# pansanity666/TransHuman

Measured on AMD Instinct MI355X. Metric: rays/sec (512x512, 64 samples/ray), higher is better.
Workload: dtype f32 (fp16 hi/lo x3 MFMA emulation)

## Files before the change

include/transhuman_hip.h:

```cpp
#ifndef TRANSHUMAN_HIP_H
#define TRANSHUMAN_HIP_H

#include <stddef.h>
#include <stdint.h>

#ifdef __cplusplus
extern "C" {
#endif

#define TH_ABI_VERSION 12

typedef struct th_ctx th_ctx;
typedef void* th_stream;

int         th_abi_version(void);
const char* th_last_error(void);
int         th_ctx_create(int device, th_ctx** out);
void        th_ctx_destroy(th_ctx* ctx);
size_t      th_sizeof(const char* type_name);

enum { TH_PROF_HULL = 0, TH_PROF_DPARF = 1, TH_PROF_GATHER = 2, TH_PROF_MLP = 3, TH_PROF_COMPOSITE = 4,
       TH_PROF_VIT = 5, TH_PROF_FOLD = 6 , TH_PROF_PHASES = 8 };
int th_profile_enable(th_ctx* ctx, int on);
int th_profile_read(th_ctx* ctx, double* ms_out, int64_t* count_out);
// ... 17 lines not shown
    th_linear upsample_color;
} th_mlp_weights;

typedef struct {
    const float *ln1_w, *ln1_b, *ln2_w, *ln2_b;
    th_linear qkv, proj, fc1, fc2;
} th_vit_block;

int th_set_mlp_weights(th_ctx* ctx, const th_mlp_weights* w, th_stream stream);
int th_set_mlp_mode(th_ctx* ctx, int mode);
int th_set_fused_waves(th_ctx* ctx, int waves);
int th_set_tok_gather(th_ctx* ctx, int on);
int th_set_tex_rows(th_ctx* ctx, int on);

#define TH_RANGE_SLOTS 8
#define TH_RANGE_FP16_LIMIT 0x7B53u
#define TH_RANGE_FP16_FLOOR 0x2400u
int th_set_vit_mode(th_ctx* ctx, int mode);
int th_range_snapshot(th_ctx* ctx, th_stream stream);
int th_range_read(th_ctx* ctx, int slot, uint32_t* out );
int th_range_last_slot(th_ctx* ctx);
int th_set_chunk_samples(int n);
int th_set_vit_weights(th_ctx* ctx, int depth, int dim, int heads, const th_vit_block* blocks,
                       const float* norm_w, const float* norm_b, th_stream stream);

size_t th_linear_workspace_bytes(int out_f, int in_f);
int th_linear_forward(th_ctx* ctx, const float* A, int lda, int M, const th_linear* lin, int act,
                      float* C, int ldc, void* workspace, size_t workspace_bytes, th_stream stream);

typedef struct {
    const float* pts;
    const float* ray_o;
    const float* ray_d;
    const float* near;
    const float* far;
    const float* t_vals;
    const float* one_minus_t;
    int R, S;
    const float* z_vals;
    const float* sigma_noise;
} th_points;

size_t th_hull_workspace_bytes(int n_verts);
int th_hull_mask(th_ctx* ctx, const th_points* p, const float* verts_world, int n_verts, float thresh,
                 uint8_t* mask_out, int32_t* ray_hit_out, void* workspace, size_t workspace_bytes,
                 th_stream stream);

int th_paint_group(th_ctx* ctx, const float* holder_map_nchw, int V, int C, int H, int W,
                   const float* verts_world, int n_verts, const float* cams, const float* scale_xy,
                   const uint8_t* vizmap, const int32_t* csr_offsets, const int32_t* csr_members,
                   int n_clusters, float* painted_out , float* tokens_out,
                   th_stream stream);
int th_segment_mean_f32(th_ctx* ctx, const float* src, int width, const int32_t* csr_offsets,
                        const int32_t* csr_members, int n_clusters, float* out, th_stream stream);
int th_segment_mean_rot_f64(th_ctx* ctx, const double* blend, const int32_t* csr_offsets,
                            const int32_t* csr_members, int n_clusters, float* rot_out,
                            th_stream stream);

#define TH_MAP_FULL    384
#define TH_MAP_COMPACT 260
#define TH_MAP_SPLIT   256

int th_upsample_concat_nhwc(th_ctx* ctx, const float* img, const float* lat0, const float* lat1,
                            const float* lat2, const int32_t* dims_host, int V, int H, int W,
                            const float* color_w, const float* color_b, float* out_nhwc, th_stream stream);
int th_upsample_concat_split(th_ctx* ctx, const float* img, const float* lat0, const float* lat1, const float* lat2,
                             const int32_t* dims_host, int V, int H, int W, float* out, th_stream stream);
int th_map_box(th_ctx* ctx, const float* verts_a, int na, const float* verts_b, int nb, const float* cams, int V,
               const float* scale_xy, int H, int W, float reach, int32_t* box_out, th_stream stream);
int th_upsample_concat_split_box(th_ctx* ctx, const float* img, const float* lat0, const float* lat1, const float* lat2,
                                 const int32_t* dims_host, int V, int H, int W, float* out, const int32_t* box,
                                 th_stream stream);
size_t th_map_demand_bytes(int V, int H, int W);
int th_upsample_concat_split_demand(th_ctx* ctx, const float* img, const float* lat0, const float* lat1, const float* lat2,
                                    const int32_t* dims_host, int V, int H, int W, float* out, const int32_t* box,
                                    const void* demand, th_stream stream);
size_t th_paint_group_nhwc_workspace_bytes(int V, int n_verts, int C, int out_f);
int th_paint_group_nhwc(th_ctx* ctx, const float* map_nhwc, int V, int H, int W, int C,
                        const float* verts_world, int n_verts, const float* cams, const float* scale_xy,
                        const uint8_t* vizmap, const th_linear* reduction, const th_linear* color_lift,
                        const int32_t* csr_offsets,
                        const int32_t* csr_members, int n_clusters, float* tokens_out, void* workspace,
                        size_t workspace_bytes, th_stream stream);

size_t th_conv_pack_bytes(int cout, int cin, int ks);
int th_conv_pack(th_ctx* ctx, const float* w, int cout, int cin, int ks, void* packed, size_t packed_bytes,
                 float* inv_scale_out, th_stream stream);
int th_conv2d_supported(int cin, int cout, int ks, int stride);
int th_conv2d(th_ctx* ctx, const float* x, int N, int cin, int H, int W, const void* packed, float inv_scale, int cout,
              int ks, int stride, float* y, th_stream stream);

int th_maxpool3x3s2(th_ctx* ctx, const float* x, int planes, int H, int W, float* y, th_stream stream);

size_t th_bn_workspace_bytes(int N, int C, int HW);
int th_bn_act(th_ctx* ctx, const float* x, const float* residual, int N, int C, int HW, const float* gamma,
              const float* beta, float eps, float momentum, float* running_mean, float* running_var, int relu,
              float* y, void* workspace, size_t workspace_bytes, th_stream stream);
int th_bn_act_eval(th_ctx* ctx, const float* x, const float* residual, int N, int C, int HW, const float* gamma,
                   const float* beta, float eps, const float* running_mean, const float* running_var, int relu,
                   float* y, th_stream stream);
int th_conv2d_stats_partials(int N, int cin, int H, int W, int cout, int ks, int stride);
int th_conv2d_stats(th_ctx* ctx, const float* x, int N, int cin, int H, int W, const void* packed, float inv_scale,
                    int cout, int ks, int stride, float* y, void* stats, size_t stats_bytes, th_stream stream);
int th_bn_act_stats(th_ctx* ctx, const float* x, const float* residual, int N, int C, int HW, const void* stats,
                    int n_partials, const float* gamma, const float* beta, float eps, float momentum,
                    float* running_mean, float* running_var, int relu, float* y, th_stream stream);

size_t th_vit_workspace_bytes(int V, int N, int dim, int heads);
int th_vit_forward(th_ctx* ctx, const float* x, const float* pe, int V, int N, float* out,
                   void* workspace, size_t workspace_bytes, th_stream stream);

int th_dparf_encode(th_ctx* ctx, const float* pts_smpl, const int32_t* sel, int P, const float* centres,
                    const float* rot, const float* tokens, int V, int n_clusters, float* out,
                    th_stream stream);

int th_nchw_to_nhwc(th_ctx* ctx, const float* src, int V, int C, int H, int W, float* dst, th_stream stream);
int th_pixel_gather(th_ctx* ctx, const float* pixel_map_nhwc, int V, int C, int H, int W,
                    const float* pts_world, const int32_t* sel, int P, const float* cams,
                    const float* scale_xy, float* out, int ldo, th_stream stream);
int th_pixel_gather_split(th_ctx* ctx, const float* map_split, int V, int H, int W, const float* pts_world,
                          const int32_t* sel, int P, const float* cams, const float* scale_xy, void* out_rows,
                          int ldo, th_stream stream);

int th_map_fold(th_ctx* ctx, const float* map_split, int V, int H, int W, const int32_t* box, float* fold, th_stream stream);
int th_map_fold_demand(th_ctx* ctx, const float* map_split, int V, int H, int W, const void* demand, float* fold, th_stream stream);

size_t th_pixel_texlist_bytes(int V, int P);
int th_pixel_texlist(th_ctx* ctx, const float* map_split, int V, int H, int W, const float* pts_world, const int32_t* sel,
                     int P, const float* cams, const float* scale_xy, void* out, size_t out_bytes, th_stream stream);

size_t th_network_workspace_bytes(int V, int P);
int th_network_forward(th_ctx* ctx, const float* pixel_feat, const float* viewdir, const float* pts_smpl,
                       const uint8_t* mask, int P, const float* centres, const float* rot,
                       const float* tokens, int V, int n_clusters, float* raw_out, void* workspace,
                       size_t workspace_bytes, th_stream stream);

int th_composite(th_ctx* ctx, const float* raw, const float* z, const th_points* rays, int white_bkgd,
                 float* rgb, float* acc, float* depth, float* weights_out, th_stream stream);

int th_gen_rays(th_ctx* ctx, const float* K_host, const float* R_host, const float* T_host,
                const float* bounds_host, int H, int W, float* ray_o, float* ray_d, float* near_out,
                float* far_out, uint8_t* mask_at_box, th_stream stream);

int th_bound_mask(th_ctx* ctx, const int32_t* corners_xy_host , int H, int W, uint8_t* mask,
                  th_stream stream);

size_t th_marching_cubes_workspace_bytes(int X, int Y, int Z);
int th_marching_cubes_count(th_ctx* ctx, const float* cube, int X, int Y, int Z, float iso, void* workspace,
                            size_t workspace_bytes, int64_t* counts_host , th_stream stream);
int th_marching_cubes_range(th_ctx* ctx, const void* workspace, int X, int Y, int Z, int x,
                            int64_t* prefix_host , th_stream stream);
int th_marching_cubes_emit(th_ctx* ctx, const float* cube, int X, int Y, int Z, float iso, const void* workspace,
                           int x0, int x1, const double* scale_host , const double* origin_host ,
                           double* verts, int32_t* tris, th_stream stream);

size_t th_ssim_workspace_bytes(int h, int w, int c);
int th_ssim(th_ctx* ctx, const float* a, const float* b, int h, int w, int c, int pitch, double* out, void* workspace,
            size_t workspace_bytes, th_stream stream);

size_t th_lpips_pack_bytes(void);
int th_lpips_pack(th_ctx* ctx, const float* const* conv_w , const float* const* conv_b ,
                  const float* const* lin_w , void* packed, size_t bytes, th_stream stream);
size_t th_lpips_workspace_bytes(int n, int h, int w);
int th_lpips(th_ctx* ctx, const float* in0, const float* in1, int n, int h, int w, const void* packed, double* out,
             void* workspace, size_t workspace_bytes, th_stream stream);

typedef struct {
    const double* v_template;
    const double* shapedirs;
    const double* posedirs;
    const double* J_regressor;
    const double* weights;
    const int32_t* parent;
    int n_verts;
} th_smpl_model;
size_t th_smpl_workspace_bytes(int n_verts);
int th_smpl_lbs(th_ctx* ctx, const th_smpl_model* model, const float* pose_aa, const float* rot, const double* beta,
                double* verts, double* joints, double* T, void* workspace, size_t workspace_bytes,
                th_stream stream);

int th_view_embed(th_ctx* ctx, const float* ray_d, int R, int view_res, float* out, th_stream stream);

typedef struct {
    const int32_t* box;
    float          reach;
    const float*   img;
    const float*   lat0;
    const float*   lat1;
    const float*   lat2;
    int32_t        dims[6];
    const void*    demand;
} th_map_source;

typedef struct {
    const float* verts_world;
    int          n_verts;
    const float* Rh;
    const float* Th;
    const float* cams;
    const float* scale_xy;
    const float* pixel_map_nhwc;
    int          V, H, W;
    int          map_channels;
    const float* tokens;
    const float* centres;
    const float* rot;
    int          n_clusters;
    float        hull_thresh;
// ... 35 lines not shown
```

transhuman_amd/csrc/k_encoder.hip:

```cpp
#include "th_internal.h"

struct UpsSrc {
    const float* p;
    int C, h, w;
    int c0;
};

__device__ __forceinline__ void ups_coord(int dst, int in, int out, int& i0, int& i1, float& l0, float& l1) {
    float scale = (out > 1) ? (float)(in - 1) / (float)(out - 1) : 0.f;
    float src = scale * (float)dst;
    i0 = (int)src;
    i1 = i0 + ((i0 < in - 1) ? 1 : 0);
    l1 = src - (float)i0;
    l0 = 1.0f - l1;
}

__global__ __launch_bounds__(256) void upsample_concat_nhwc_kernel(UpsSrc s0, UpsSrc s1, UpsSrc s2,
                                                                   const float* __restrict__ img,
                                                                   const float* __restrict__ wc,
                                                                   const float* __restrict__ bc, int H, int W,
                                                                   int NG, int CO, float* __restrict__ out,
                                                                   float* __restrict__ rgb4,
                                                                   const int32_t* __restrict__ box,
                                                                   const unsigned* __restrict__ need) {
    __shared__ float tile[64][65];
    const int lane = threadIdx.x & 63, wave = threadIdx.x >> 6;
    const int x = blockIdx.x * 64 + lane, y = blockIdx.y;
    const int v = blockIdx.z / NG, grp = blockIdx.z % NG;
    unsigned long long want = ~0ull;
    if (need != nullptr) {
        const unsigned* nw = need + ((((long long)v * H + y) * W + (long long)blockIdx.x * 64) >> 5);
        want = (unsigned long long)nw[0] | ((unsigned long long)nw[1] << 32);
        if (want == 0ull) return;
    }
    if (box != nullptr) {
        const int by0 = box[4 * v + 1], by1 = box[4 * v + 3];
        if (y < by0 || y > by1) return;
        const int32_t* sp = box + 4 * (gridDim.z / NG) + ((long long)v * H + y) * 2;
        if ((int)blockIdx.x * 64 + 63 < sp[0] || (int)blockIdx.x * 64 > sp[1]) return;
    }
    int cout0;
    if (grp == 4 && NG == 5) {
        if (wave == 0 && x < W && ((want >> lane) & 1ull)) {
            long long hw = (long long)H * W;
            const float* ip = img + (long long)v * 3 * hw + (long long)y * W + x;
            float* dst = rgb4 ? rgb4 + (((long long)v * H + y) * W + x) * 4 : out + (((long long)v * H + y) * W + x) * CO + 256;
            *reinterpret_cast<float4*>(dst) = make_float4(ip[0], ip[hw], ip[2 * hw], 0.f);
        }
        return;
    }
    if (grp < 4) {
        UpsSrc s = grp == 0 ? s0 : (grp == 1 ? s1 : s2);
        int cin0 = grp == 3 ? 64 : 0;
        cout0 = s.c0 + cin0;
        int y0, y1, x0, x1;
        float ly0, ly1, lx0, lx1;
        ups_coord(y, s.h, H, y0, y1, ly0, ly1);
        ups_coord(x < W ? x : W - 1, s.w, W, x0, x1, lx0, lx1);
        const float* base = s.p + ((long long)v * s.C + cin0) * s.h * s.w;
        for (int c = wave; c < 64; c += 4) {
            const float* pl = base + (long long)c * s.h * s.w;
            float v00 = pl[y0 * s.w + x0], v01 = pl[y0 * s.w + x1], v10 = pl[y1 * s.w + x0], v11 = pl[y1 * s.w + x1];
            tile[lane][c] = ly0 * (lx0 * v00 + lx1 * v01) + ly1 * (lx0 * v10 + lx1 * v11);
        }
    } else {
        int cin0 = (grp - 4) * 64;
        cout0 = 256 + cin0;
        int xx = x < W ? x : W - 1;
        long long hw = (long long)H * W;
        const float* ip = img + (long long)v * 3 * hw + (long long)y * W + xx;
        float r = ip[0], g = ip[hw], b = ip[2 * hw];
        for (int c = wave; c < 64; c += 4) {
            const float* w = wc + (cin0 + c) * 3;
            tile[lane][c] = fmaf(b, w[2], fmaf(g, w[1], r * w[0])) + bc[cin0 + c];
        }
    }
    __syncthreads();
    float* orow = out + (((long long)v * H + y) * W + (long long)blockIdx.x * 64) * CO + cout0;
    for (int px = wave; px < 64; px += 4)
        if (blockIdx.x * 64 + px < W && ((want >> px) & 1ull)) orow[(long long)px * CO + lane] = tile[px][lane];
}

int th_upsample_concat_launch(const float* img, const float* lat0, const float* lat1, const float* lat2,
                              const int* dims , int V, int H, int W, const float* wc,
                              const float* bc, float* out, hipStream_t s, int split, const int32_t* box, const unsigned* need) {
    UpsSrc s0{lat0, 64, dims[0], dims[1], 0};
    UpsSrc s1{lat1, 64, dims[2], dims[3], 64};
    UpsSrc s2{lat2, 128, dims[4], dims[5], 128};
    const int NG = wc ? 6 : 5, CO = wc ? 384 : (split ? 256 : 260);
    float* rgb4 = (!wc && split) ? out + (long long)V * H * W * 256 : nullptr;
    hipLaunchKernelGGL(upsample_concat_nhwc_kernel, dim3(th_cdiv(W, 64), H, V * NG), dim3(256), 0, s, s0, s1, s2, img, wc,
                       bc, H, W, NG, CO, out, rgb4, box, need);
    TH_LAUNCH_CHECK();
    return 0;
}

#define MAPBOX_NB 8
__global__ void map_box_init_kernel(int V, int H, int W, int32_t* __restrict__ box) {
    const int v = blockIdx.x;
    int32_t* sp = box + 4 * V + (long long)v * H * 2;
    for (int i = threadIdx.x; i < H; i += blockDim.x) { sp[2 * i] = W; sp[2 * i + 1] = -1; }
    if (threadIdx.x == 0) {
        box[4 * v] = 0x7fffffff; box[4 * v + 1] = 0x7fffffff; box[4 * v + 2] = -1; box[4 * v + 3] = -1;
        box[4 * V + (long long)V * H * 2 + v] = 0;
    }
}
__global__ __launch_bounds__(1024) void map_box_kernel(const float* __restrict__ va, int na, const float* __restrict__ vb,
                                                       int nb, const float* __restrict__ cams,
                                                       const float* __restrict__ scale, int H, int W, float reach,
                                                       int32_t* __restrict__ box) {
    const int v = blockIdx.x, V = gridDim.x, tid = threadIdx.x;
    const float* cam = cams + 21 * v;
    bool bad = false;
    extern __shared__ int span_l[];
    __shared__ int bx[4];
    for (int i = tid; i < H; i += 1024) { span_l[2 * i] = W; span_l[2 * i + 1] = -1; }
    if (tid == 0) { bx[0] = 0x7fffffff; bx[1] = 0x7fffffff; bx[2] = -1; bx[3] = -1; }
    __syncthreads();
    for (int i = blockIdx.y * 1024 + tid; i < na + nb; i += 1024 * gridDim.y) {
        const float* p = i < na ? va + 3 * i : vb + 3 * (i - na);
        const float x = p[0], y = p[1], z = p[2];
        float vx0 = 3.0e38f, vx1 = -3.0e38f, vy0 = 3.0e38f, vy1 = -3.0e38f;
        bool vbad = false;
        for (int k = 0; k < 8; ++k) {
            const float qx = x + ((k & 1) ? reach : -reach), qy = y + ((k & 2) ? reach : -reach),
                        qz = z + ((k & 4) ? reach : -reach);
            const float cx = fmaf(cam[2], qz, fmaf(cam[1], qy, cam[0] * qx)) + cam[9];
            const float cy = fmaf(cam[5], qz, fmaf(cam[4], qy, cam[3] * qx)) + cam[10];
            const float cz = fmaf(cam[8], qz, fmaf(cam[7], qy, cam[6] * qx)) + cam[11];
            const float* K = cam + 12;
            const float pz = fmaf(K[8], cz, fmaf(K[7], cy, K[6] * cx));
            float u, w;
            th_project(cam, qx, qy, qz, u, w);
            const float ix = ((u * scale[0] - 1.0f + 1.0f) / 2.0f) * (float)(W - 1);
            const float iy = ((w * scale[1] - 1.0f + 1.0f) / 2.0f) * (float)(H - 1);
            if (!(pz > 1e-6f) || !(fabsf(ix) < 1.0e9f) || !(fabsf(iy) < 1.0e9f)) vbad = true;
            vx0 = fminf(vx0, ix); vx1 = fmaxf(vx1, ix);
            vy0 = fminf(vy0, iy); vy1 = fmaxf(vy1, iy);
        }
        bad = bad || vbad;
        if (!vbad) {
            const int ax0 = (int)fminf(fmaxf(floorf(vx0) - 2.0f, 0.0f), (float)(W - 1));
            const int ax1 = (int)fminf(fmaxf(floorf(vx1) + 3.0f, 0.0f), (float)(W - 1));
            const int ay0 = (int)fminf(fmaxf(floorf(vy0) - 2.0f, 0.0f), (float)(H - 1));
            const int ay1 = (int)fminf(fmaxf(floorf(vy1) + 3.0f, 0.0f), (float)(H - 1));
            atomicMin(&bx[0], ax0); atomicMin(&bx[1], ay0); atomicMax(&bx[2], ax1); atomicMax(&bx[3], ay1);
            for (int yy = ay0; yy <= ay1; ++yy) {
                atomicMin(&span_l[2 * yy], ax0);
                atomicMax(&span_l[2 * yy + 1], ax1);
            }
        }
    }
    if (bad) atomicOr(&box[4 * V + (long long)V * H * 2 + v], 1);
    __syncthreads();
    int32_t* sp = box + 4 * V + (long long)v * H * 2;
    for (int i = tid; i < H; i += 1024)
        if (span_l[2 * i + 1] >= span_l[2 * i]) {
            atomicMin(&sp[2 * i], span_l[2 * i]);
            atomicMax(&sp[2 * i + 1], span_l[2 * i + 1]);
        }
    if (tid == 0 && bx[2] >= 0) {
        atomicMin(&box[4 * v], bx[0]); atomicMin(&box[4 * v + 1], bx[1]);
        atomicMax(&box[4 * v + 2], bx[2]); atomicMax(&box[4 * v + 3], bx[3]);
    }
}
__global__ void map_box_final_kernel(int V, int H, int W, int nverts, int32_t* __restrict__ box) {
    const int v = blockIdx.x;
    const bool full = box[4 * V + (long long)V * H * 2 + v] != 0 || nverts <= 0 || box[4 * v + 2] < 0;
    if (!full) return;
    int32_t* sp = box + 4 * V + (long long)v * H * 2;
    for (int i = threadIdx.x; i < H; i += blockDim.x) { sp[2 * i] = 0; sp[2 * i + 1] = W - 1; }
    if (threadIdx.x == 0) { box[4 * v] = 0; box[4 * v + 1] = 0; box[4 * v + 2] = W - 1; box[4 * v + 3] = H - 1; }
}
int th_map_box_launch(const float* va, int na, const float* vb, int nb, const float* cams, int V, const float* scale, int H,
                      int W, float reach, int32_t* box, hipStream_t s) {
// ... 192 lines not shown
```

transhuman_amd/csrc/k_mlp_fused_host.hip:

```cpp
#include <stdio.h>
#include <stdlib.h>
#include <string.h>

#include "k_mlp_fused_kernel.h"
#include "k_mlp_fused8_kernel.h"

__global__ void pack_fused_kernel(const float* __restrict__ W, int N, int K, int KB, int CT, const int* __restrict__ cols,
                                  float scale, uint4* __restrict__ out) {
    long long total = 4LL * KB * CT * 2 * 64;
    for (long long o = blockIdx.x * (long long)blockDim.x + threadIdx.x; o < total;
         o += (long long)gridDim.x * blockDim.x) {
        int lane = (int)(o & 63);
        long long q = o >> 6;
        int plane = (int)(q & 1); q >>= 1;
        int ct = (int)(q % CT); q /= CT;
        int kb = (int)(q % KB);
        int wave = (int)(q / KB);
        int col = cols[wave * CT + ct] + (lane & 31);
        int k0 = 16 * kb + 8 * (lane >> 5);
        h8 v;
#pragma unroll
        for (int j = 0; j < 8; ++j) {
            int k = k0 + j;
            float x = (col < N && k < K) ? W[(long long)col * K + k] * scale : 0.f;
// ... 73 lines not shown
};

static int pack_layer(const float* w, const float* b, int N, int K, int CT, const int* cols_host, int sl2,
                      PackCursor& cur, FusedLayer* out, hipStream_t s) {
    const int KB = (K + 15) / 16;
    if (b) TH_HIP(hipMemcpyAsync(cur.bias, b, (size_t)N * 4, hipMemcpyDeviceToDevice, s));
    else TH_HIP(hipMemsetAsync(cur.bias, 0, (size_t)N * 4, s));
    TH_HIP(hipMemcpyAsync(cur.cols, cols_host, 4 * CT * sizeof(int), hipMemcpyHostToDevice, s));
    uint4* dst = (uint4*)cur.w;
    long long total = 4LL * KB * CT * 2 * 64;
    hipLaunchKernelGGL(pack_fused_kernel, dim3(256), dim3(256), 0, s, w, N, K, KB, CT, cur.cols, ldexpf(1.f, sl2), dst);
    TH_HIP(hipStreamSynchronize(s));
    out->w = dst;
    out->bias = cur.bias;
    out->inv_scale = ldexpf(1.f, -sl2);
    out->CT = CT;
    out->KB = KB;
    cur.w += th_align((size_t)total * 16);
    cur.bias += (N + 3) & ~3;
    cur.cols += 16;
    return 0;
}

static int pack_layer16(const float* w, int N, int K, int CT, const int* cols_host, const FusedLayer& base, int sl2, PackCursor& cur,
                        FusedLayer* out, hipStream_t s) {
    const int T = (K + 31) / 32;
    Cols24 cols{};
    for (int i = 0; i < 8 * CT; ++i) cols.c[i] = cols_host[i];
    uint4* dst = (uint4*)cur.w;
    const long long total = 8LL * T * CT * 2 * 64;
    hipLaunchKernelGGL(pack_fused16_kernel, dim3(256), dim3(256), 0, s, w, N, K, T, CT, cols, ldexpf(1.f, sl2), K == 256 ? 1 : 0, dst);
    TH_LAUNCH_CHECK();
    *out = base;
    out->w = dst;
    out->CT = CT;
    out->KB = T;
    cur.w += th_align((size_t)total * 16);
    return 0;
}

__global__ void fold_matmul_kernel(const float* __restrict__ F, const float* __restrict__ Vw, float* __restrict__ out) {
    int o = blockIdx.x, k = threadIdx.x;
    double acc = 0.0;
    for (int m = 0; m < 256; ++m) acc += (double)F[o * 256 + m] * (double)Vw[m * 256 + k];
    out[o * 256 + k] = (float)acc;
}
__global__ void fold_bias_kernel(const float* __restrict__ F, const float* __restrict__ bF, const float* __restrict__ b1,
                                 const float* __restrict__ b0, float* __restrict__ out) {
    int o = threadIdx.x;
    double acc = bF ? (double)bF[o] : 0.0;
    for (int m = 0; m < 256; ++m) {
        double bm = (b1 ? (double)b1[m] : 0.0) + (b0 ? (double)b0[m] : 0.0);
        acc += (double)F[o * 256 + m] * bm;
    }
    out[o] = (float)acc;
}

__global__ void fold_mm_kernel(const float* __restrict__ A, int lda, const float* __restrict__ B, int ldb, int K, int N,
                               float* __restrict__ out, int ldo) {
    const int m = blockIdx.x;
    for (int n = threadIdx.x; n < N; n += blockDim.x) {
        double acc = 0.0;
        for (int k = 0; k < K; ++k) acc += (double)A[(long long)m * lda + k] * (double)B[(long long)k * ldb + n];
        out[(long long)m * ldo + n] = (float)acc;
    }
}
__global__ void fold_mv_kernel(const float* __restrict__ A, int lda, int K, const float* __restrict__ b0,
                               const float* __restrict__ b1, const float* __restrict__ b2, float* __restrict__ out) {
    const int m = blockIdx.x * blockDim.x + threadIdx.x;
    double acc = b0 ? (double)b0[m] : 0.0;
    for (int k = 0; k < K; ++k)
        acc += (double)A[(long long)m * lda + k] * ((b1 ? (double)b1[k] : 0.0) + (b2 ? (double)b2[k] : 0.0));
    out[m] = (float)acc;
}
__global__ void scale_rows_kernel(const float* __restrict__ src, int lds_, int rows, int cols, float scale,
                                  float* __restrict__ dst, int ldd) {
    long long n = (long long)rows * cols;
    for (long long i = blockIdx.x * (long long)blockDim.x + threadIdx.x; i < n; i += (long long)gridDim.x * blockDim.x) {
        int r = (int)(i / cols), c = (int)(i % cols);
        dst[(long long)r * ldd + c] = src[(long long)r * lds_ + c] * scale;
    }
}

int th_fused_pack(const th_mlp_weights* w, const th_linear* folded, void* store, FusedParams* out, hipStream_t s) {
    char* tail = (char*)store + th_fused_pack_bytes() - 64 * 1024;
    PackCursor cur{(char*)store, (float*)tail, (int*)(tail + 40 * 1024)};
    unsigned int* amax = (unsigned int*)(tail + 60 * 1024);
    int c256[8], c128[4], ckv[12], cst[8];
    int c256_16[16], c128_16[8], ckv16[24];
    for (int wv = 0; wv < 8; ++wv) {
        c256_16[wv * 2] = wv * 32; c256_16[wv * 2 + 1] = wv * 32 + 16;
        c128_16[wv] = wv * 16;
        ckv16[wv * 3] = wv * 16; ckv16[wv * 3 + 1] = 128 + wv * 32; ckv16[wv * 3 + 2] = 128 + wv * 32 + 16;
    }
    for (int wv = 0; wv < 4; ++wv) {
        c256[wv * 2] = wv * 64; c256[wv * 2 + 1] = wv * 64 + 32;
        c128[wv] = wv * 32;
        ckv[wv * 3] = wv * 32; ckv[wv * 3 + 1] = 128 + wv * 64; ckv[wv * 3 + 2] = 128 + wv * 64 + 32;
        cst[wv * 2] = wv * 32; cst[wv * 2 + 1] = 128 + wv * 32;
    }
    int sl2, sl2b;
#define PACK_SIMPLE(LAYER, L, N_, K_, CT_, COLS)                                       \
    TH_TRY(layer_scale_log2((L).w, (long long)(N_) * (K_), amax, &sl2, s));            \
    TH_TRY(pack_layer((L).w, (L).b, N_, K_, CT_, COLS, sl2, cur, &out->LAYER, s))
    float* scratch = nullptr;
    const size_t n_scratch = 256 * 63 + 128 * 256 + 128 * 384 + 128 * 260 + 256 * 384 + 256 + (384 * 256 + 384);
    TH_HIP(hipMalloc((void**)&scratch, n_scratch * 4));
    struct Free { float* p; ~Free() { (void)hipFree(p); } } free_scratch{scratch};
    float* wpe = scratch;
    float* XF = wpe + 256 * 63;
    float* XR = XF + 128 * 256;
    float* XRc = XR + 128 * 384;
    float* st = XRc + 128 * 260;
    float* stb = st + 256 * 384;
    float* tw = stb + 256;
    {
        TH_HIP(hipMemcpy2DAsync(wpe, 63 * 4, w->fc_0.w + 192, 255 * 4, 63 * 4, 256, hipMemcpyDeviceToDevice, s));
        TH_TRY(layer_scale_log2(wpe, 256LL * 63, amax, &sl2, s));
        TH_TRY(pack_layer(wpe, w->fc_0.b, 256, 63, 2, c256, sl2, cur, &out->fc_0pe, s));
        TH_TRY(pack_layer16(wpe, 256, 63, 2, c256_16, out->fc_0pe, sl2, cur, &out->w16.fc_0pe, s));
    }
    PACK_SIMPLE(ar0, w->alpha_res_0, 256, 384, 2, c256);
    PACK_SIMPLE(fc_2, w->fc_2, 256, 256, 2, c256);
    TH_TRY(pack_layer16(w->fc_2.w, 256, 256, 2, c256_16, out->fc_2, sl2, cur, &out->w16.fc_2, s));
    PACK_SIMPLE(fc_3, w->fc_3, 256, 256, 2, c256);
    TH_TRY(pack_layer16(w->fc_3.w, 256, 256, 2, c256_16, out->fc_3, sl2, cur, &out->w16.fc_3, s));
    PACK_SIMPLE(fc_4, w->fc_4, 128, 128, 1, c128);
    TH_TRY(pack_layer16(w->fc_4.w, 128, 128, 1, c128_16, out->fc_4, sl2, cur, &out->w16.fc_4, s));
#undef PACK_SIMPLE
    out->compact_ready = false;
    if (folded) {
        TH_TRY(layer_scale_log2(folded[0].w, 256LL * 260, amax, &sl2, s));
        TH_TRY(pack_layer(folded[0].w, folded[0].b, 256, 260, 2, c256, sl2, cur, &out->ar0c, s));
    }
    {
        const float* Wvf = w->view_fc.w;
        hipLaunchKernelGGL(fold_mm_kernel, dim3(128), dim3(256), 0, s, Wvf, 283, w->feature_fc.w, 256, 256, 256, XF, 256);
        hipLaunchKernelGGL(fold_mm_kernel, dim3(128), dim3(256), 0, s, Wvf, 283, w->rgb_res_0.w, 384, 256, 384, XR, 384);
        if (folded)
            hipLaunchKernelGGL(fold_mm_kernel, dim3(128), dim3(256), 0, s, Wvf, 283, folded[1].w, 260, 256, 260, XRc, 260);
        TH_LAUNCH_CHECK();
        TH_TRY(layer_scale_log2(XF, 128LL * 256, amax, &sl2, s));
        TH_TRY(layer_scale_log2(XR, 128LL * 384, amax, &sl2b, s));
        if (sl2b < sl2) sl2 = sl2b;
        if (folded) {
            TH_TRY(layer_scale_log2(XRc, 128LL * 260, amax, &sl2b, s));
            if (sl2b < sl2) sl2 = sl2b;
        }
        {
            TH_HIP(hipMemcpy2DAsync(st, 27 * 4, Wvf + 256, 283 * 4, 27 * 4, 128, hipMemcpyDeviceToDevice, s));
            TH_TRY(layer_scale_log2(st, 128LL * 27, amax, &sl2b, s));
            if (sl2b < sl2) sl2 = sl2b;
            TH_TRY(pack_layer(st, nullptr, 128, 27, 1, c128, sl2, cur, &out->vfD, s));
            TH_TRY(pack_layer16(st, 128, 27, 1, c128_16, out->vfD, sl2, cur, &out->w16.vfD, s));
        }
        const int s_vf = sl2;
        TH_TRY(pack_layer(XF, nullptr, 128, 256, 1, c128, s_vf, cur, &out->vfA, s));
        TH_TRY(pack_layer16(XF, 128, 256, 1, c128_16, out->vfA, s_vf, cur, &out->w16.vfA, s));
        for (int variant = 0; variant < (folded ? 2 : 1); ++variant) {
            const int K = variant ? 260 : 384;
            const float* xr = variant ? XRc : XR;
            const th_linear& r0 = variant ? folded[1] : w->rgb_res_0;
            const th_linear& r1 = variant ? folded[2] : w->rgb_res_1;
            int s_r1;
            TH_TRY(layer_scale_log2(r1.w, 128LL * K, amax, &s_r1, s));
            hipLaunchKernelGGL(scale_rows_kernel, dim3(128), dim3(256), 0, s, xr, K, 128, K, ldexpf(1.f, s_vf), st, K);
            hipLaunchKernelGGL(scale_rows_kernel, dim3(128), dim3(256), 0, s, r1.w, K, 128, K, ldexpf(1.f, s_r1),
                               st + 128 * K, K);
            hipLaunchKernelGGL(fold_mv_kernel, dim3(1), dim3(128), 0, s, Wvf, 283, 256, w->view_fc.b, w->feature_fc.b,
                               r0.b, stb);
            if (r1.b) TH_HIP(hipMemcpyAsync(stb + 128, r1.b, 128 * 4, hipMemcpyDeviceToDevice, s));
            else TH_HIP(hipMemsetAsync(stb + 128, 0, 128 * 4, s));
            TH_LAUNCH_CHECK();
            FusedLayer* dst = variant ? &out->rstc : &out->rst;
            TH_TRY(pack_layer(st, stb, 256, K, 2, cst, 0, cur, dst, s));
            dst->inv_scale = ldexpf(1.f, -s_vf);
            dst->inv_scale2 = ldexpf(1.f, -s_r1);
        }
        out->vfA.inv_scale = out->vfD.inv_scale = ldexpf(1.f, -s_vf);
        out->compact_ready = folded != nullptr;
    }
    float* tb = tw + 384 * 256;
    for (int which = 0; which < 2; ++which) {
        const th_linear& k = which == 0 ? w->key1 : w->key0;
        const th_linear& v = which == 0 ? w->val1 : w->val0;
        TH_HIP(hipMemcpyAsync(tw, k.w, 128 * 256 * 4, hipMemcpyDeviceToDevice, s));
        hipLaunchKernelGGL(fold_matmul_kernel, dim3(256), dim3(256), 0, s, w->fc_1.w, v.w, tw + 128 * 256);
        if (k.b) TH_HIP(hipMemcpyAsync(tb, k.b, 128 * 4, hipMemcpyDeviceToDevice, s));
        else TH_HIP(hipMemsetAsync(tb, 0, 128 * 4, s));
        TH_HIP(hipMemsetAsync(tb + 128, 0, 256 * 4, s));
        TH_TRY(layer_scale_log2(tw, 384LL * 256, amax, &sl2, s));
        TH_TRY(pack_layer(tw, tb, 384, 256, 3, ckv, sl2, cur, which == 0 ? &out->kv1 : &out->kv0, s));
        TH_TRY(pack_layer16(tw, 384, 256, 3, ckv16, which == 0 ? out->kv1 : out->kv0, sl2, cur, which == 0 ? &out->w16.kv1 : &out->w16.kv0, s));
    }
    hipLaunchKernelGGL(fold_bias_kernel, dim3(1), dim3(256), 0, s, w->fc_1.w, w->fc_1.b, w->val1.b, w->val0.b, cur.bias);
    out->fc_1 = FusedLayer{};
    out->fc_1.bias = cur.bias;
    cur.bias += 256;
    TH_HIP(hipStreamSynchronize(s));
    TH_REQUIRE(cur.w <= tail, "fused pack overflow");
    TH_REQUIRE((char*)cur.bias <= tail + 40 * 1024 && (char*)cur.cols <= tail + 60 * 1024, "fused pack tail overflow");
    return 0;
}

__global__ __launch_bounds__(256) void tok_split_kernel(float* __restrict__ t, int rows, float* __restrict__ sc,
                                                        unsigned int* __restrict__ range) {
    const unsigned bits = reinterpret_cast<const unsigned*>(sc)[1];
    const int E = (int)((bits >> 23) & 255u);
    int sl2 = 0;
    if (E == 255) { if (range != nullptr && blockIdx.x == 0 && threadIdx.x == 0) atomicMax(range + TH_RANGE_VIT, 0x7c00u); }
    else if (bits != 0u) sl2 = min(139 - E, 100);
    const float scale = __builtin_bit_cast(float, (unsigned)(sl2 + 127) << 23);
    if (blockIdx.x == 0 && threadIdx.x == 0) sc[0] = __builtin_bit_cast(float, (unsigned)(127 - sl2) << 23);
    const int lane = threadIdx.x & 63;
    for (int r = blockIdx.x * 4 + (threadIdx.x >> 6); r < rows; r += gridDim.x * 4) {
        float* row = t + (long long)r * 256;
        const float4 x = reinterpret_cast<const float4*>(row)[lane];
        const float v[4] = {x.x * scale, x.y * scale, x.z * scale, x.w * scale};
        h4 hv, lv;
#pragma unroll
        for (int e = 0; e < 4; ++e) {
            _Float16 hi, lo;
            split_h(v[e], hi, lo);
            hv[e] = hi;
            lv[e] = lo;
        }
        __builtin_amdgcn_s_waitcnt(0);
        _Float16* rh = reinterpret_cast<_Float16*>(row);
        *reinterpret_cast<h4*>(rh + 4 * lane) = hv;
        *reinterpret_cast<h4*>(rh + 256 + 4 * lane) = lv;
    }
}

int th_tok_split(float* tprime, int rows, float* sc, unsigned int* range, hipStream_t s) {
    if (rows <= 0) return 0;
    unsigned int* amax = reinterpret_cast<unsigned int*>(sc) + 1;
    TH_HIP(hipMemsetAsync(amax, 0, 4, s));
    hipLaunchKernelGGL(absmax_kernel, dim3(64), dim3(256), 0, s, tprime, (long long)rows * 256, amax);
    hipLaunchKernelGGL(tok_split_kernel, dim3(th_cdiv(rows, 4) < 1024 ? th_cdiv(rows, 4) : 1024), dim3(256), 0, s, tprime, rows, sc,
                       range);
    TH_LAUNCH_CHECK();
    return 0;
}

int th_map_fold_launch(const FusedParams& base, const float* map_split, int V, int H, int W, const int32_t* box, float* fold,
                       unsigned int* range, hipStream_t s, const unsigned* demand) {
    TH_REQUIRE(base.compact_ready, "the map fold needs the colour-folded layers (th_mlp_weights.upsample_color)");
    TH_REQUIRE(V >= 1 && H >= 1 && W >= 1 && map_split && fold, "bad argument");
    MapFoldParams p;
    p.ar0 = base.ar0c; p.rst = base.rstc;
    p.lat = map_split; p.rgb = map_split + (size_t)V * H * W * 256;
    p.box = box; p.V = V; p.H = H; p.W = W;
    p.out0 = fold; p.out12 = fold + (size_t)V * H * W * 256;
    p.range = range;
    p.list = nullptr; p.count = nullptr;
    static unsigned long long attr_done = 0ull;
    if (th_lds_attr_needed(&attr_done)) {
        TH_HIP(hipFuncSetAttribute((const void*)map_fold_kernel<false>, hipFuncAttributeMaxDynamicSharedMemorySize, 2 * MF_TEX * STR272));
        TH_HIP(hipFuncSetAttribute((const void*)map_fold_kernel<true>, hipFuncAttributeMaxDynamicSharedMemorySize, 2 * MF_TEX * STR272));
    }
    if (demand != nullptr) {
        const size_t NW = (size_t)V * H * W / 32;
        p.count = demand + 2 * NW;
        p.list = reinterpret_cast<const int32_t*>(demand + 2 * NW + 16);
        hipLaunchKernelGGL(map_fold_kernel<true>, dim3(512), dim3(256), 2 * MF_TEX * STR272, s, p);
        TH_LAUNCH_CHECK();
        return 0;
    }
    const int tpr = (W + MF_TEX - 1) / MF_TEX;
    hipLaunchKernelGGL(map_fold_kernel<false>, dim3((unsigned)(V * H * tpr)), dim3(256), 2 * MF_TEX * STR272, s, p);
    TH_LAUNCH_CHECK();
    return 0;
}

int th_mlp_fused_forward(const FusedParams& base, const ThMlpPacked& heads, int V, int P, const float* stok,
                         const void* pe, const void* f, int f_ld, const float* vd, const int32_t* vd_sel, int vd_div, int rgb_all, float* raw_c,
                         unsigned int* range, hipStream_t s, const void* tsplit, const float* t_inv, int t_nc, const float* tex_map,
                         size_t tex_stride) {
    if (P <= 0) return 0;
    TH_REQUIRE(V >= 1 && V <= 3, "fused MLP supports 1..3 reference views");
    TH_REQUIRE(f_ld == 384 || (f_ld == 272 && base.compact_ready),
               "pixel-feature rows must be 384 wide, or 272 wide with upsample_color weights uploaded");
    const bool cf = f_ld == 272;
    FusedParams p = base;
    if (cf) { p.ar0 = base.ar0c; p.rst = base.rstc; }
    p.alpha_w = heads.alpha_w; p.alpha_b = heads.alpha_b; p.rgb_w = heads.rgb_w; p.rgb_b = heads.rgb_b;
    TH_REQUIRE(tsplit == nullptr || (t_inv != nullptr && t_nc >= 7 && t_nc <= 4096), "split token table: scale word and 7 <= N_c <= 4096");
    p.tsplit = (const _Float16*)tsplit; p.t_inv = t_inv; p.t_nc = t_nc;
    const bool tex = tex_map != nullptr;
    TH_REQUIRE(!tex || (cf && f != nullptr), "texel hand-over: compact (272-wide) operand planes only");
    p.tex_hdr = nullptr; p.tex_rec = nullptr; p.tex_map = nullptr; p.tex_map2 = nullptr;
    if (tex) {
        p.tex_hdr = (const unsigned*)f;
        p.tex_rec = p.tex_hdr + (size_t)th_cdiv(P, FM_PTS) * 512;
        p.tex_map = tex_map;
        p.tex_map2 = tex_map + tex_stride;
        f = nullptr;
    }
    p.stok = stok; p.pe = (const _Float16*)pe; p.f = (const _Float16*)f; p.vd = vd; p.vd_sel = vd_sel; p.vd_div = vd_div > 0 ? vd_div : 1; p.raw_c = raw_c; p.P = P; p.rgb_all = rgb_all; p.range = range;
    static unsigned long long attr_done = 0ull;
    if (th_lds_attr_needed(&attr_done)) {
#define FM_ATTR(V_, F_)                                                                                       \
    TH_HIP(hipFuncSetAttribute((const void*)mlp_fused_kernel<V_, F_>, hipFuncAttributeMaxDynamicSharedMemorySize, \
                               FUSED_LDS_BYTES))
        FM_ATTR(1, 0); FM_ATTR(2, 0); FM_ATTR(3, 0); FM_ATTR(1, 1); FM_ATTR(2, 1); FM_ATTR(3, 1);
#undef FM_ATTR
#define FM_ATTR_T(V_)                                                                                              \
    TH_HIP(hipFuncSetAttribute((const void*)mlp_fused_kernel<V_, 1, true>, hipFuncAttributeMaxDynamicSharedMemorySize, \
                               FUSED_LDS_BYTES))
        FM_ATTR_T(1); FM_ATTR_T(2); FM_ATTR_T(3);
#undef FM_ATTR_T
    }
    dim3 grid(tex ? 8 * th_cdiv(th_cdiv(P, FM_PTS), 8) : th_cdiv(P, FM_PTS));
    const bool eight = base.waves == 8 && tex && tsplit != nullptr;
    static unsigned long long attr8_done = 0ull;
    if (eight && th_lds_attr_needed(&attr8_done)) {
        TH_HIP(hipFuncSetAttribute((const void*)mlp_fused8_kernel<1>, hipFuncAttributeMaxDynamicSharedMemorySize, F8_LDS_BYTES));
        TH_HIP(hipFuncSetAttribute((const void*)mlp_fused8_kernel<2>, hipFuncAttributeMaxDynamicSharedMemorySize, F8_LDS_BYTES));
        TH_HIP(hipFuncSetAttribute((const void*)mlp_fused8_kernel<3>, hipFuncAttributeMaxDynamicSharedMemorySize, F8_LDS_BYTES));
    }
    static int dbg_state = getenv("TH_FUSED_DBG") ? 1 : 0;
    static long long* dbg_dev = nullptr;
    p.dbg = base.cycles_buf;
    const bool dbg_now = dbg_state == 1 && P >= 4096 && base.cycles_buf == nullptr;
    hipEvent_t dbg_e0 = nullptr, dbg_e1 = nullptr;
    if (dbg_now) {
        if (!dbg_dev) TH_HIP(hipMalloc((void**)&dbg_dev, 64 * sizeof(long long)));
        TH_HIP(hipMemsetAsync(dbg_dev, 0, 64 * sizeof(long long), s));
        p.dbg = dbg_dev;
        TH_HIP(hipEventCreate(&dbg_e0));
        TH_HIP(hipEventCreate(&dbg_e1));
        TH_HIP(hipStreamSynchronize(s));
        TH_HIP(hipEventRecord(dbg_e0, s));
    }
#define FM_LAUNCH(V_, F_) hipLaunchKernelGGL((mlp_fused_kernel<V_, F_>), grid, dim3(256), FUSED_LDS_BYTES, s, p)
#define FM_LAUNCH_T(V_) hipLaunchKernelGGL((mlp_fused_kernel<V_, 1, true>), grid, dim3(256), FUSED_LDS_BYTES, s, p)
#define FM_LAUNCH_8(V_) hipLaunchKernelGGL((mlp_fused8_kernel<V_>), grid, dim3(F8_THREADS), F8_LDS_BYTES, s, p)
    if (eight) {
        if (V == 1) FM_LAUNCH_8(1); else if (V == 2) FM_LAUNCH_8(2); else FM_LAUNCH_8(3);
    } else if (tex) {
        if (V == 1) FM_LAUNCH_T(1); else if (V == 2) FM_LAUNCH_T(2); else FM_LAUNCH_T(3);
    } else
    switch (V * 2 + (cf ? 1 : 0)) {
        case 2: FM_LAUNCH(1, 0); break;
        case 3: FM_LAUNCH(1, 1); break;
        case 4: FM_LAUNCH(2, 0); break;
        case 5: FM_LAUNCH(2, 1); break;
        case 6: FM_LAUNCH(3, 0); break;
        default: FM_LAUNCH(3, 1); break;
    }
#undef FM_LAUNCH
#undef FM_LAUNCH_T
#undef FM_LAUNCH_8
    TH_LAUNCH_CHECK();
    if (dbg_now) {
// ... 23 lines not shown
```

transhuman_amd/csrc/k_mlp_fused_kernel.h:

```cpp
#pragma once
#include <hip/hip_fp16.h>

#include <utility>

#include "th_internal.h"

typedef float f32x16 __attribute__((ext_vector_type(16)));
typedef _Float16 h8 __attribute__((ext_vector_type(8)));
typedef _Float16 h4 __attribute__((ext_vector_type(4)));
typedef float f32x4v __attribute__((ext_vector_type(4)));
typedef unsigned fm_u4 __attribute__((ext_vector_type(4)));

#define FM_PTS 32
#define STR272 560
#define STR256 528
#define STR192 400
#define STR128 272
#define STR64 144
#define STRVD 80
#define KSTR 132

#define ABUF_BYTES (2 * 96 * STR272)
#define MBUF_BYTES (96 * KSTR * 4)
#define MISC_FLOATS (9 * 32 + 128 + 4 * 32 * 4 + 8)
// ... 1294 lines not shown
    auto texel = [&](int x) __attribute__((always_inline)) -> long long {
        if constexpr (LIST) return (long long)P.list[x];
        else return trow + x;
    };
    for (;;) {
    unsigned rmax = 0u;
    const unsigned seen_f = P.range ? P.range[TH_RANGE_F] : 0u;
    {
        const int wv = __builtin_amdgcn_readfirstlane(wave);
#pragma unroll 4
        for (int k = 0; k < MF_TEX / 4; ++k) {
            const int r = wv + 4 * k;
            const long long t = texel(min(xs + r, x1));
            const float4 q = *reinterpret_cast<const float4*>(P.lat + t * 256 + 4 * lane);
            uint2 h, l;
            split_pair(q.x, q.y, h.x, l.x);
            split_pair(q.z, q.w, h.y, l.y);
            range_acc<false>(rmax, h.x);
            range_acc<false>(rmax, h.y);
            *reinterpret_cast<uint2*>(hi_pl + r * STR272 + lane * 8) = h;
            *reinterpret_cast<uint2*>(lo_pl + r * STR272 + lane * 8) = l;
        }
        if (tid < MF_TEX) {
            const long long t = texel(min(xs + tid, x1));
            const float4 c = *reinterpret_cast<const float4*>(P.rgb + t * 4);
            uint4 th = make_uint4(0u, 0u, 0u, 0u), tl = make_uint4(0u, 0u, 0u, 0u);
            split_pair(c.x, c.y, th.x, tl.x);
            split_pair(c.z, 0.f, th.y, tl.y);
            range_acc<false>(rmax, th.x);
            range_acc<false>(rmax, th.y);
            const uint4 z4 = make_uint4(0u, 0u, 0u, 0u);
            *reinterpret_cast<uint4*>(hi_pl + tid * STR272 + 512) = th;
            *reinterpret_cast<uint4*>(hi_pl + tid * STR272 + 528) = z4;
            *reinterpret_cast<uint4*>(lo_pl + tid * STR272 + 512) = tl;
            *reinterpret_cast<uint4*>(lo_pl + tid * STR272 + 528) = z4;
        }
        range_commit(P.range, TH_RANGE_F, seen_f, rmax);
    }
    __syncthreads();
    const int myrow = lane & 31;
    uint4 wk2[FM_RING_D2][2][2];
    f32x16 acc[2][MF_RT];
    gemm_phase_core<MF_RT, 2, STR272, 32 * STR272, FM_RING_D2, true, 3, false>(hi_pl, lo_pl, wslice(P.ar0, wave, 2, 0), MF_KB, lane, acc, wk2);
    {
        const float sc = P.ar0.inv_scale;
#pragma unroll
        for (int r = 0; r < MF_RT; ++r) {
            const int x = xs + r * 32 + myrow;
            if (MF_STORE(x <= x1)) {
                float* o = P.out0 + texel(x) * 256 + wave * 64 + 4 * (lane >> 5);
#pragma unroll
                for (int c = 0; c < 2; ++c)
#pragma unroll
                    for (int g = 0; g < 4; ++g)
                        *reinterpret_cast<float4*>(o + c * 32 + 8 * g) =
                            make_float4(acc[c][r][4 * g] * sc, acc[c][r][4 * g + 1] * sc, acc[c][r][4 * g + 2] * sc, acc[c][r][4 * g + 3] * sc);
            }
        }
    }
    gemm_phase_core<MF_RT, 2, STR272, 32 * STR272, FM_RING_D2, true, 3, false>(hi_pl, lo_pl, wslice(P.rst, wave, 2, 0), MF_KB, lane, acc, wk2);
    {
        const float s0 = P.rst.inv_scale, s1 = P.rst.inv_scale2;
#pragma unroll
        for (int r = 0; r < MF_RT; ++r) {
            const int x = xs + r * 32 + myrow;
            if (MF_STORE(x <= x1)) {
                float* o = P.out12 + texel(x) * 256 + wave * 32 + 4 * (lane >> 5);
#pragma unroll
                for (int g = 0; g < 4; ++g) {
                    *reinterpret_cast<float4*>(o + 8 * g) =
                        make_float4(acc[0][r][4 * g] * s0, acc[0][r][4 * g + 1] * s0, acc[0][r][4 * g + 2] * s0, acc[0][r][4 * g + 3] * s0);
                    *reinterpret_cast<float4*>(o + 128 + 8 * g) =
                        make_float4(acc[1][r][4 * g] * s1, acc[1][r][4 * g + 1] * s1, acc[1][r][4 * g + 2] * s1, acc[1][r][4 * g + 3] * s1);
                }
            }
        }
    }
    if (!LIST) break;
    xs += (int)gridDim.x * MF_TEX;
    if (xs > x1) break;
    __syncthreads();
    }
}
```

transhuman_amd/csrc/th_api.hip:

```cpp
#include <stdlib.h>
#include <string.h>

#include <vector>

#include "th_internal.h"

static thread_local std::string g_err;
void th_set_error(const std::string& msg) { g_err = msg; }

struct ThProf {
    bool on = false;
    std::vector<hipEvent_t> pool;
    size_t used = 0;
    struct Span { int phase; hipEvent_t a, b; };
    std::vector<Span> spans;
    hipEvent_t get() {
        if (used == pool.size()) {
            hipEvent_t e;
            if (hipEventCreate(&e) != hipSuccess) return nullptr;
            pool.push_back(e);
        }
        return pool[used++];
    }
};
struct ProfScope {
    ThProf* p; int phase; hipStream_t s; hipEvent_t a = nullptr;
    ProfScope(ThProf* p_, int phase_, hipStream_t s_) : p(p_), phase(phase_), s(s_) {
        if (p && p->on) {
            hipStreamCaptureStatus st = hipStreamCaptureStatusNone;
            if (hipStreamIsCapturing(s, &st) != hipSuccess || st != hipStreamCaptureStatusNone) return;
            a = p->get();
            if (a) (void)hipEventRecord(a, s);
        }
    }
    void close() {
        if (a) { hipEvent_t b = p->get(); if (b) { (void)hipEventRecord(b, s); p->spans.push_back({phase, a, b}); } }
        a = nullptr;
    }
    ~ProfScope() { close(); }
};
static ThProf* prof_of(th_ctx* c);
__global__ void clock_probe_kernel(long long* __restrict__ out, int iters) {
    float x = 1.0f + threadIdx.x * 1e-3f;
    const long long t0 = clock64(), w0 = wall_clock64();
    for (int i = 0; i < iters; ++i) x = fmaf(x, 0.999f, 1e-3f);
    const long long t1 = clock64(), w1 = wall_clock64();
    if (threadIdx.x == 0) { out[0] = t1 - t0; out[1] = w1 - w0; }
    if (x == 12345.678f) out[2] = 1;
}


extern "C" {

int th_abi_version(void) { return TH_ABI_VERSION; }
const char* th_last_error(void) { return g_err.c_str(); }
size_t th_sizeof(const char* type_name) {
    if (type_name == nullptr) return 0;
#define TH_SZ(T) if (strcmp(type_name, #T) == 0) return sizeof(T)
    TH_SZ(th_points); TH_SZ(th_frame); TH_SZ(th_map_source); TH_SZ(th_linear); TH_SZ(th_mlp_weights); TH_SZ(th_vit_block); TH_SZ(th_smpl_model);
#undef TH_SZ
    return 0;
}

int th_ctx_create(int device, th_ctx** out) {
    TH_REQUIRE(out != nullptr, "null out");
    int count = 0;
    TH_HIP(hipGetDeviceCount(&count));
    TH_REQUIRE(device >= 0 && device < count, "no such device");
    TH_HIP(hipSetDevice(device));
    hipDeviceProp_t prop;
    TH_HIP(hipGetDeviceProperties(&prop, device));
    TH_REQUIRE(std::string(prop.gcnArchName).rfind("gfx950", 0) == 0,
               std::string("libtranshuman_hip is built for gfx950 only, device is ") + prop.gcnArchName);
    th_ctx* c = new th_ctx();
    c->device = device;
    c->n_cu = prop.multiProcessorCount;
    if (const char* e = getenv("TH_TOK_GATHER")) c->tok_gather = e[0] == '0' ? 0 : 1;
    if (const char* e = getenv("TH_ROWS_TEX")) c->tex_rows = e[0] == '0' ? 0 : 1;
    c->fused.waves = 8;
    if (const char* e = getenv("TH_FUSED_WAVES")) c->fused.waves = e[0] == '4' ? 4 : 8;
    TH_HIP(hipHostMalloc((void**)&c->host_pinned, 64 * sizeof(int32_t), hipHostMallocDefault));
    TH_HIP(hipMalloc((void**)&c->range_dev, TH_RANGE_SLOTS * sizeof(unsigned int)));
    TH_HIP(hipMemset(c->range_dev, 0, TH_RANGE_SLOTS * sizeof(unsigned int)));
    TH_HIP(hipHostMalloc((void**)&c->range_host, th_ctx::kRangeSnaps * TH_RANGE_SLOTS * sizeof(unsigned int),
                         hipHostMallocDefault));
    memset(c->range_host, 0, th_ctx::kRangeSnaps * TH_RANGE_SLOTS * sizeof(unsigned int));
    *out = c;
    return 0;
}

void th_ctx_destroy(th_ctx* c) {
    if (!c) return;
    if (c->mlp_store) (void)hipFree(c->mlp_store);
    if (c->vit_store) (void)hipFree(c->vit_store);
    if (c->fused_store) (void)hipFree(c->fused_store);
    if (c->host_pinned) (void)hipHostFree(c->host_pinned);
    if (c->range_dev) (void)hipFree(c->range_dev);
    if (c->range_host) (void)hipHostFree(c->range_host);
    if (c->aux) (void)hipStreamDestroy(c->aux);
    if (c->aux2) (void)hipStreamDestroy(c->aux2);
    if (c->aux2_join) (void)hipEventDestroy(c->aux2_join);
    if (c->aux_fork) (void)hipEventDestroy(c->aux_fork);
    if (c->aux_join) (void)hipEventDestroy(c->aux_join);
    if (c->after_shade) (void)hipEventDestroy(c->after_shade);
    for (auto& e : c->range_ev)
        if (e) (void)hipEventDestroy(e);
    for (auto& t : c->prepass)
        if (t.ev) (void)hipEventDestroy(t.ev);
    delete[] c->vit.blocks;
    if (c->prof) {
        ThProf* p = (ThProf*)c->prof;
        for (auto e : p->pool) (void)hipEventDestroy(e);
        delete p;
    }
    delete c;
}

int th_profile_enable(th_ctx* c, int on) {
    TH_REQUIRE(c, "null ctx");
    ThProf* p = prof_of(c);
    p->on = on != 0;
    p->used = 0;
    p->spans.clear();
    return 0;
}

int th_clock_probe(th_ctx* c, int64_t* out_dev, th_stream stream) {
    TH_REQUIRE(c && out_dev, "null argument");
    hipLaunchKernelGGL(clock_probe_kernel, dim3(1), dim3(64), 0, (hipStream_t)stream, (long long*)out_dev, 4096);
    TH_LAUNCH_CHECK();
    return 0;
}

int th_fused_cycles(th_ctx* c, int64_t* counters_dev) {
    TH_REQUIRE(c, "null ctx");
    c->fused.cycles_buf = (long long*)counters_dev;
    return 0;
}

int th_host_wait_read(th_ctx* c, double* ms_out) {
    TH_REQUIRE(c && ms_out, "null argument");
    *ms_out = c->host_wait_ms;
    c->host_wait_ms = 0.0;
    return 0;
}

int th_profile_read(th_ctx* c, double* ms_out, int64_t* count_out) {
    TH_REQUIRE(c && ms_out && count_out, "null argument");
    ThProf* p = prof_of(c);
    for (int i = 0; i < TH_PROF_PHASES; ++i) { ms_out[i] = 0.0; count_out[i] = 0; }
    for (auto& sp : p->spans) {
        TH_HIP(hipEventSynchronize(sp.b));
        float ms = 0.f;
        TH_HIP(hipEventElapsedTime(&ms, sp.a, sp.b));
        if (sp.phase >= 0 && sp.phase < TH_PROF_PHASES) { ms_out[sp.phase] += ms; count_out[sp.phase] += 1; }
    }
    p->used = 0;
    p->spans.clear();
    return 0;
}

static bool lin_ok(const th_linear& l, int out_f, int in_f) {
    return l.w != nullptr && l.out_f == out_f && l.in_f == in_f;
}

int th_set_mlp_weights(th_ctx* c, const th_mlp_weights* w, th_stream stream) {
    TH_REQUIRE(c && w, "null argument");
    hipStream_t s = (hipStream_t)stream;
    TH_REQUIRE(lin_ok(w->fc_0, 256, 255) && lin_ok(w->alpha_res_0, 256, 384) && lin_ok(w->key0, 128, 256) &&
                   lin_ok(w->val0, 256, 256) && lin_ok(w->key1, 128, 256) && lin_ok(w->val1, 256, 256) &&
                   lin_ok(w->fc_1, 256, 256) && lin_ok(w->fc_2, 256, 256) && lin_ok(w->fc_3, 256, 256) &&
                   lin_ok(w->alpha_fc, 1, 256) && lin_ok(w->feature_fc, 256, 256) &&
                   lin_ok(w->rgb_res_0, 256, 384) && lin_ok(w->view_fc, 128, 283) &&
                   lin_ok(w->rgb_res_1, 128, 384) && lin_ok(w->fc_4, 128, 128) && lin_ok(w->rgb_fc, 3, 128),
               "unexpected layer shape (expects the reference Network of cross_transformer.py:96-126)");
    struct Item { const th_linear* l; ThPacked* dst; int out_f, in_f; };
    ThMlpPacked& M = c->mlp;
    size_t total = 0;
// ... 214 lines not shown

int th_hull_mask(th_ctx* c, const th_points* p, const float* verts, int nv, float thresh, uint8_t* mask,
                 int32_t* ray_hit, void* ws, size_t ws_bytes, th_stream stream) {
    TH_REQUIRE(c && p && verts && mask && ws, "null argument");
    TH_REQUIRE(p->pts || (p->ray_o && p->ray_d && p->near && p->far && p->t_vals && p->one_minus_t),
               "need explicit pts or a complete ray description");
    ThPointSrc ps = th_src(p);
    long long P = (long long)p->R * p->S;
    return th_hull_mask_launch(ps, P, verts, nv, thresh, mask, ray_hit, ws, ws_bytes, (hipStream_t)stream);
}

int th_paint_group(th_ctx* c, const float* map, int V, int C, int H, int W, const float* verts, int nv,
                   const float* cams, const float* scale, const uint8_t* viz, const int32_t* off, const int32_t* mem,
                   int nc, float* painted, float* tokens, th_stream stream) {
    TH_REQUIRE(c && map && verts && cams && scale && off && mem && tokens, "null argument");
    TH_REQUIRE(painted != nullptr, "painted_out scratch [V,n_verts,C] is required");
    hipStream_t s = (hipStream_t)stream;
    TH_TRY(th_paint_launch(map, V, C, H, W, verts, nv, cams, scale, viz, painted, s));
    return th_segmean_launch(painted, V, (long long)nv * C, C, off, mem, nc, tokens, s);
}

int th_segment_mean_f32(th_ctx* c, const float* src, int width, const int32_t* off, const int32_t* mem, int nc,
                        float* out, th_stream stream) {
    TH_REQUIRE(c && src && off && mem && out, "null argument");
    return th_segmean_launch(src, 1, 0, width, off, mem, nc, out, (hipStream_t)stream);
}

int th_segment_mean_rot_f64(th_ctx* c, const double* blend, const int32_t* off, const int32_t* mem, int nc,
                            float* rot, th_stream stream) {
    TH_REQUIRE(c && blend && off && mem && rot, "null argument");
    return th_segmean_rot_launch(blend, off, mem, nc, rot, (hipStream_t)stream);
}

int th_upsample_concat_split(th_ctx* c, const float* img, const float* lat0, const float* lat1, const float* lat2,
                             const int32_t* dims_host, int V, int H, int W, float* out, th_stream stream) {
    TH_REQUIRE(c && img && lat0 && lat1 && lat2 && dims_host && out, "null argument");
    return th_upsample_concat_launch(img, lat0, lat1, lat2, dims_host, V, H, W, nullptr, nullptr, out, (hipStream_t)stream, 1,
                                     nullptr);
}

int th_upsample_concat_split_box(th_ctx* c, const float* img, const float* lat0, const float* lat1, const float* lat2,
                                 const int32_t* dims_host, int V, int H, int W, float* out, const int32_t* box,
                                 th_stream stream) {
    TH_REQUIRE(c && img && lat0 && lat1 && lat2 && dims_host && out, "null argument");
    return th_upsample_concat_launch(img, lat0, lat1, lat2, dims_host, V, H, W, nullptr, nullptr, out, (hipStream_t)stream, 1,
                                     box);
}

size_t th_map_demand_bytes(int V, int H, int W) { return th_demand_bytes(V, H, W); }

int th_upsample_concat_split_demand(th_ctx* c, const float* img, const float* lat0, const float* lat1, const float* lat2,
                                    const int32_t* dims_host, int V, int H, int W, float* out, const int32_t* box,
                                    const void* demand, th_stream stream) {
    TH_REQUIRE(c && img && lat0 && lat1 && lat2 && dims_host && out && demand, "null argument");
    TH_REQUIRE((W % 64) == 0, "demand-driven map: image width must be a multiple of 64");
    const unsigned* need_map = reinterpret_cast<const unsigned*>(demand) + (size_t)V * H * W / 32;
    return th_upsample_concat_launch(img, lat0, lat1, lat2, dims_host, V, H, W, nullptr, nullptr, out, (hipStream_t)stream, 1,
                                     box, need_map);
}

int th_map_box(th_ctx* c, const float* verts_a, int na, const float* verts_b, int nb, const float* cams, int V,
               const float* scale_xy, int H, int W, float reach, int32_t* box_out, th_stream stream) {
    TH_REQUIRE(c && cams && scale_xy && box_out && (verts_a || na == 0) && (verts_b || nb == 0), "null argument");
    TH_REQUIRE(V > 0 && H > 0 && W > 0 && na >= 0 && nb >= 0 && reach >= 0.f, "bad sizes");
    return th_map_box_launch(verts_a, na, verts_b, nb, cams, V, scale_xy, H, W, reach, box_out, (hipStream_t)stream);
}

int th_upsample_concat_nhwc(th_ctx* c, const float* img, const float* lat0, const float* lat1, const float* lat2,
                            const int32_t* dims_host, int V, int H, int W, const float* color_w, const float* color_b,
                            float* out_nhwc, th_stream stream) {
    TH_REQUIRE(c && img && lat0 && lat1 && lat2 && dims_host && out_nhwc, "null argument");
    TH_REQUIRE(color_w == nullptr || color_b != nullptr, "color_b is required with color_w");
    return th_upsample_concat_launch(img, lat0, lat1, lat2, dims_host, V, H, W, color_w, color_b, out_nhwc,
                                     (hipStream_t)stream, 0, nullptr);
}

size_t th_paint_group_nhwc_workspace_bytes(int V, int n_verts, int C, int out_f) {
    if (C == TH_MAP_SPLIT) C = TH_MAP_COMPACT;
    size_t rows = (size_t)V * n_verts;
    return th_align(rows * C * 4) + th_align(rows * out_f * 4) + ThPacked::bytes(out_f, C) +
           th_align((size_t)(out_f * 260 + out_f) * 4);
}

int th_paint_group_nhwc(th_ctx* c, const float* map_nhwc, int V, int H, int W, int C, const float* verts, int nv,
                        const float* cams, const float* scale, const uint8_t* viz, const th_linear* reduction,
                        const th_linear* color_lift, const int32_t* off, const int32_t* mem, int nc, float* tokens,
                        void* ws, size_t ws_bytes, th_stream stream) {
    TH_REQUIRE(c && map_nhwc && verts && cams && scale && reduction && off && mem && tokens && ws, "null argument");
    const bool compact = C == TH_MAP_COMPACT || C == TH_MAP_SPLIT;
    TH_REQUIRE(reduction->in_f == (compact ? TH_MAP_FULL : C), "reduction layer must take the (full) map's channel count");
    TH_REQUIRE(!compact || (color_lift && color_lift->w && lin_ok(*color_lift, 128, 3)),
               "a compact map needs the upsample_color layer (3 -> 128) to fold into the reduction layer");
    const int out_f = reduction->out_f;
    TH_REQUIRE(ws_bytes >= th_paint_group_nhwc_workspace_bytes(V, nv, C, out_f), "workspace too small");
    hipStream_t s = (hipStream_t)stream;
    ThArena ar(ws, ws_bytes);
    const size_t rows = (size_t)V * nv;
    const int CR = C == TH_MAP_SPLIT ? TH_MAP_COMPACT : C;
    float* g = ar.take<float>(rows * CR);
    float* r = ar.take<float>(rows * out_f);
    void* pk = ar.take<char>(ThPacked::bytes(out_f, CR));
    float* fold = ar.take<float>((size_t)out_f * 260 + out_f);
    TH_REQUIRE(fold != nullptr, "workspace carve failed");
    TH_TRY(th_pixgather_launch(map_nhwc, V, C, H, W, verts, nullptr, nullptr, nv, cams, scale, g, CR, TH_ROWS_F32, s));
    ThPacked P;
    th_linear red = *reduction;
    if (compact) {
        TH_TRY(th_fold_color_launch(reduction->w, reduction->b, color_lift->w, color_lift->b, out_f, fold,
                                    fold + (size_t)out_f * 260, s));
        red.w = fold; red.b = fold + (size_t)out_f * 260; red.in_f = 260;
    }
    TH_TRY(th_pack_linear(red, pk, &P, s));
    TH_TRY(th_gemm(g, CR, (int)rows, P, TH_ACT_NONE, r, out_f, s));
    return th_segmean_masked_launch(r, V, out_f, viz, nv, off, mem, nc, tokens, s);
}

int th_bn_act_eval(th_ctx* c, const float* x, const float* residual, int N, int C, int HW, const float* gamma, const float* beta,
                   float eps, const float* running_mean, const float* running_var, int relu, float* y, th_stream stream) {
    TH_REQUIRE(c && x && y && running_mean && running_var, "null argument");
    return th_bn_act_launch(x, residual, N, C, HW, gamma, beta, eps, 0.f, const_cast<float*>(running_mean),
                            const_cast<float*>(running_var), relu, y, nullptr, 0, (hipStream_t)stream, 1);
}

size_t th_vit_workspace_bytes(int V, int N, int dim, int heads) { return th_vit_ws(V, N, dim, heads); }

size_t th_conv_pack_bytes(int cout, int cin, int ks) { return th_conv_pack_size(cout, cin, ks); }

int th_conv_pack(th_ctx* c, const float* w, int cout, int cin, int ks, void* packed, size_t packed_bytes,
                 float* inv_scale_out, th_stream stream) {
    TH_REQUIRE(c && w && packed && inv_scale_out, "null argument");
    return th_conv_pack_launch(w, cout, cin, ks, packed, packed_bytes, inv_scale_out, (hipStream_t)stream);
}

int th_conv2d_supported(int cin, int cout, int ks, int stride) { return th_conv2d_built(cin, cout, ks, stride) ? 1 : 0; }

int th_conv2d(th_ctx* c, const float* x, int N, int cin, int H, int W, const void* packed, float inv_scale, int cout, int ks,
              int stride, float* y, th_stream stream) {
    TH_REQUIRE(c && x && packed && y, "null argument");
    TH_REQUIRE(N > 0 && H > 0 && W > 0, "empty tensor");
    return th_conv2d_launch(x, N, cin, H, W, packed, inv_scale, cout, ks, stride, y, (hipStream_t)stream, c->range_dev);
}

int th_conv2d_stats_partials(int N, int cin, int H, int W, int cout, int ks, int stride) {
    int np = 0;
    if (!th_conv2d_built(cin, cout, ks, stride) || N <= 0 || H <= 0 || W <= 0) return 0;
    if (th_conv2d_launch(nullptr, N, cin, H, W, nullptr, 0.f, cout, ks, stride, nullptr, nullptr, nullptr, nullptr, &np)) return 0;
    return np;
}

int th_conv2d_stats(th_ctx* c, const float* x, int N, int cin, int H, int W, const void* packed, float inv_scale, int cout,
                    int ks, int stride, float* y, void* stats, size_t stats_bytes, th_stream stream) {
    TH_REQUIRE(c && x && packed && y && stats, "null argument");
    TH_REQUIRE(N > 0 && H > 0 && W > 0, "empty tensor");
    const int np = th_conv2d_stats_partials(N, cin, H, W, cout, ks, stride);
    TH_REQUIRE(np > 0, "th_conv2d_stats: shape not built");
    TH_REQUIRE(stats_bytes >= (size_t)cout * np * sizeof(float2), "statistics buffer too small");
    TH_REQUIRE(((uintptr_t)stats & 7) == 0, "statistics buffer must be 8-byte aligned");
    return th_conv2d_launch(x, N, cin, H, W, packed, inv_scale, cout, ks, stride, y, (hipStream_t)stream, c->range_dev,
                            (float2*)stats, nullptr);
}

int th_bn_act_stats(th_ctx* c, const float* x, const float* residual, int N, int C, int HW, const void* stats, int n_partials,
                    const float* gamma, const float* beta, float eps, float momentum, float* running_mean,
                    float* running_var, int relu, float* y, th_stream stream) {
    TH_REQUIRE(c && x && y && stats && n_partials > 0, "null argument");
    TH_REQUIRE((running_mean == nullptr) == (running_var == nullptr), "running_mean / running_var go together");
    return th_bn_act_launch(x, residual, N, C, HW, gamma, beta, eps, momentum, running_mean, running_var, relu, y, nullptr, 0,
                            (hipStream_t)stream, 0, stats, n_partials);
}

int th_maxpool3x3s2(th_ctx* c, const float* x, int planes, int H, int W, float* y, th_stream stream) {
    TH_REQUIRE(c && x && y && planes > 0 && H > 0 && W > 0, "bad argument");
    return th_maxpool3x3s2_launch(x, planes, H, W, y, (hipStream_t)stream);
}

size_t th_bn_workspace_bytes(int N, int C, int HW) { return th_bn_ws(N, C, HW); }

int th_bn_act(th_ctx* c, const float* x, const float* residual, int N, int C, int HW, const float* gamma, const float* beta,
              float eps, float momentum, float* running_mean, float* running_var, int relu, float* y, void* ws,
              size_t ws_bytes, th_stream stream) {
    TH_REQUIRE(c && x && y && ws, "null argument");
    TH_REQUIRE((running_mean == nullptr) == (running_var == nullptr), "running_mean / running_var go together");
    return th_bn_act_launch(x, residual, N, C, HW, gamma, beta, eps, momentum, running_mean, running_var, relu, y, ws,
                            ws_bytes, (hipStream_t)stream);
}

int th_vit_forward(th_ctx* c, const float* x, const float* pe, int V, int N, float* out, void* ws, size_t ws_bytes,
                   th_stream stream) {
    TH_REQUIRE(c && x && pe && out && ws, "null argument");
    ProfScope sc(prof_of(c), TH_PROF_VIT, (hipStream_t)stream);
    return th_vit_launch(c->vit, x, pe, V, N, out, ws, ws_bytes, (hipStream_t)stream, c->vit_mode >= 1 ? c->range_dev : nullptr,
                         c->vit_mode >= 1);
}

int th_dparf_encode(th_ctx* c, const float* pts, const int32_t* sel, int P, const float* centres, const float* rot,
                    const float* tokens, int V, int nc, float* out, th_stream stream) {
    TH_REQUIRE(c && pts && centres && rot && tokens && out, "null argument");
    return th_dparf_launch(pts, nullptr, nullptr, nullptr, sel, P, centres, rot, tokens, V, nc, 0.5f, out, nullptr,
                           TH_ROWS_F32, nullptr, (hipStream_t)stream);
}

int th_nchw_to_nhwc(th_ctx* c, const float* src, int V, int C, int H, int W, float* dst, th_stream stream) {
    TH_REQUIRE(c && src && dst, "null argument");
    return th_nchw_to_nhwc_launch(src, V, C, H, W, dst, (hipStream_t)stream);
}

int th_pixel_gather(th_ctx* c, const float* map, int V, int C, int H, int W, const float* pts, const int32_t* sel,
                    int P, const float* cams, const float* scale, float* out, int ldo, th_stream stream) {
    TH_REQUIRE(c && map && pts && cams && scale && out, "null argument");
    return th_pixgather_launch(map, V, C, H, W, pts, nullptr, sel, P, cams, scale, out, ldo, TH_ROWS_F32,
                               (hipStream_t)stream);
}

int th_pixel_gather_split(th_ctx* c, const float* map_split, int V, int H, int W, const float* pts, const int32_t* sel, int P,
                          const float* cams, const float* scale, void* out_rows, int ldo, th_stream stream) {
    TH_REQUIRE(c && map_split && pts && cams && scale && out_rows, "null argument");
    TH_REQUIRE(ldo == 272, "split rows of the compact map are 272 wide (256 latents | r g b 0 | zeros)");
    return th_pixgather_launch(map_split, V, TH_MAP_SPLIT, H, W, pts, nullptr, sel, P, cams, scale, (float*)out_rows, ldo,
                               TH_ROWS_SPLIT, (hipStream_t)stream, nullptr);
}

int th_map_fold(th_ctx* c, const float* map_split, int V, int H, int W, const int32_t* box, float* fold, th_stream stream) {
    TH_REQUIRE(c && map_split && fold, "null argument");
    TH_REQUIRE(c->fused_ready && c->fused.compact_ready, "th_map_fold needs the MLP weights incl. upsample_color (th_set_mlp_weights)");
    ProfScope sc(prof_of(c), TH_PROF_FOLD, (hipStream_t)stream);
    return th_map_fold_launch(c->fused, map_split, V, H, W, box, fold, c->range_dev, (hipStream_t)stream);
}

int th_map_fold_demand(th_ctx* c, const float* map_split, int V, int H, int W, const void* demand, float* fold, th_stream stream) {
    TH_REQUIRE(c && map_split && fold && demand, "null argument");
    TH_REQUIRE(c->fused_ready && c->fused.compact_ready, "th_map_fold needs the MLP weights incl. upsample_color (th_set_mlp_weights)");
    ProfScope sc(prof_of(c), TH_PROF_FOLD, (hipStream_t)stream);
    return th_map_fold_launch(c->fused, map_split, V, H, W, nullptr, fold, c->range_dev, (hipStream_t)stream,
                              reinterpret_cast<const unsigned*>(demand));
}

size_t th_pixel_texlist_bytes(int V, int P) { return th_pixtex_bytes(V, P); }

int th_pixel_texlist(th_ctx* c, const float* map_split, int V, int H, int W, const float* pts, const int32_t* sel, int P,
                     const float* cams, const float* scale, void* out, size_t out_bytes, th_stream stream) {
    TH_REQUIRE(c && pts && cams && scale && out, "null argument");
    (void)map_split;
    TH_REQUIRE(out_bytes >= th_pixtex_bytes(V, P), "output too small (th_pixel_texlist_bytes)");
    ThPointSrc ps{};
    ps.pts = pts;
    return th_pixtex_launch(V, H, W, &ps, sel, P, cams, scale, out, (hipStream_t)stream);
}

int th_composite(th_ctx* c, const float* raw, const float* z, const th_points* rays, int white, float* rgb,
                 float* acc, float* depth, float* wout, th_stream stream) {
    TH_REQUIRE(c && raw && rays && rgb && acc && depth, "null argument");
    TH_REQUIRE(rays->ray_d != nullptr, "ray_d required");
    TH_REQUIRE(z || (rays->near && rays->far && rays->t_vals && rays->one_minus_t), "need z or near/far/t_vals");
    return th_composite_launch(raw, z, th_src(rays), white, rgb, acc, depth, wout, nullptr, (hipStream_t)stream);
}

int th_gen_rays(th_ctx* c, const float* K_host, const float* R_host, const float* T_host, const float* bounds_host, int H,
                int W, float* ray_o, float* ray_d, float* near_out, float* far_out, uint8_t* mask_at_box,
                th_stream stream) {
    TH_REQUIRE(c && K_host && R_host && T_host && bounds_host && ray_o && ray_d && near_out && far_out && mask_at_box,
               "null argument");
    return th_gen_rays_launch(K_host, R_host, T_host, bounds_host, H, W, ray_o, ray_d, near_out, far_out, mask_at_box,
                              (hipStream_t)stream);
}

int th_bound_mask(th_ctx* c, const int32_t* corners_xy_host, int H, int W, uint8_t* mask, th_stream stream) {
    TH_REQUIRE(c && corners_xy_host && mask && H > 0 && W > 0, "bad argument");
    return th_bound_mask_launch(corners_xy_host, H, W, mask, (hipStream_t)stream);
}

size_t th_ssim_workspace_bytes(int h, int w, int c) { return th_ssim_ws(h, w, c); }

int th_ssim(th_ctx* c, const float* a, const float* b, int h, int w, int ch, int pitch, double* out, void* ws, size_t ws_bytes,
            th_stream stream) {
    TH_REQUIRE(c && a && b && out && ws, "null argument");
    TH_REQUIRE(h >= 7 && w >= 7, "image is " + std::to_string(h) + " x " + std::to_string(w) +
                                     ": SSIM needs at least 7 x 7 pixels (skimage raises ValueError)");
    return th_ssim_launch(a, b, h, w, ch, pitch, out, ws, ws_bytes, (hipStream_t)stream);
}

size_t th_lpips_pack_bytes(void) { return th_lpips_pack_bytes_internal(); }

int th_lpips_pack(th_ctx* c, const float* const* conv_w, const float* const* conv_b, const float* const* lin_w,
                  void* packed, size_t bytes, th_stream stream) {
    TH_REQUIRE(c && conv_w && conv_b && lin_w && packed, "null argument");
    return th_lpips_pack_launch(conv_w, conv_b, lin_w, packed, bytes, (hipStream_t)stream);
}

size_t th_lpips_workspace_bytes(int n, int h, int w) { return th_lpips_ws(n, h, w); }

int th_lpips(th_ctx* c, const float* in0, const float* in1, int n, int h, int w, const void* packed, double* out,
             void* ws, size_t ws_bytes, th_stream stream) {
    TH_REQUIRE(h >= 16 && w >= 16, "image is " + std::to_string(h) + " x " + std::to_string(w) +
                                       ": LPIPS (VGG16) needs at least 16 x 16 pixels (the fifth tap would be empty)");
    TH_REQUIRE(c && in0 && in1 && packed && out && ws, "null argument");
    return th_lpips_launch(in0, in1, n, h, w, packed, out, ws, ws_bytes, (hipStream_t)stream);
}

size_t th_marching_cubes_workspace_bytes(int X, int Y, int Z) { return th_mc_ws(X, Y, Z) + 256; }

int th_marching_cubes_count(th_ctx* c, const float* cube, int X, int Y, int Z, float iso, void* ws, size_t ws_bytes,
                            int64_t* counts_host, th_stream stream) {
    TH_REQUIRE(c && cube && ws && counts_host, "null argument");
    TH_REQUIRE(ws_bytes >= th_marching_cubes_workspace_bytes(X, Y, Z), "workspace too small");
    hipStream_t s = (hipStream_t)stream;
    long long* cnt = (long long*)((char*)ws + th_mc_ws(X, Y, Z));
    TH_TRY(th_mc_count_launch(cube, X, Y, Z, iso, ws, th_mc_ws(X, Y, Z), cnt, s));
    long long h[2];
    TH_HIP(hipMemcpyAsync(h, cnt, sizeof(h), hipMemcpyDeviceToHost, s));
    TH_HIP(hipStreamSynchronize(s));
    counts_host[0] = h[0]; counts_host[1] = h[1];
    return 0;
}
// ... 241 lines not shown
    w.idx = ar.take<int32_t>((size_t)P);
    w.info = ar.take<int32_t>(16);
    w.vd_all = ar.take<float>((size_t)R * 27);
    w.raw = ar.take<float>((size_t)P * 4);
    w.tprime = ar.take<float>(TPRIME_FLOATS(f->V));
    w.gws_b = th_dparf_grid_ws(f->n_clusters > 0 ? f->n_clusters : 1);
    w.gws = ar.take<char>(w.gws_b);
    return w;
}
static int frame_f_ld(const th_frame* f) {
    return (f->map_channels == TH_MAP_COMPACT || f->map_channels == TH_MAP_SPLIT) ? 272 : 384;
}

static int shade_points(th_ctx* c, const th_frame* f, const ThPointSrc& ps, long long P, bool ray_mode, ThArena& ar,
                        void* pool, size_t pool_bytes, float** raw_out, const uint8_t** mask_out, int64_t* stats_host,
                        hipStream_t s, int prepass = 0, int slot = 0, const int32_t** ray_hit_out = nullptr) {
    const int R = ps.R, S = ps.S, V = f->V;
    const bool compact = f->map_channels == TH_MAP_COMPACT || f->map_channels == TH_MAP_SPLIT;
    const int f_ld = frame_f_ld(f);
    const int fmt = mlp_row_format(c, V);
    const bool tex = tex_rows(c, f);
    const float* tex_map = tex ? f->map_fold : nullptr;
    const size_t tex_stride = (size_t)f->V * f->H * f->W * 256;
    TH_REQUIRE(prepass == 1 || !compact || c->mlp.compact_ready,
               "compact pixel map needs th_mlp_weights.upsample_color (colour-folded layers) to be uploaded");
    const ShadeWs w = carve_shade_ws(f, P, R, ar);
    uint8_t* mask = w.mask;
    int32_t* ray_hit = w.ray_hit;
    const size_t hws_b = w.hws_b, cws_b = w.cws_b, gws_b = w.gws_b;
    void *hws = w.hws, *cws = w.cws, *gws = w.gws;
    int32_t *idx = w.idx, *info = w.info;
    float *vd_all = w.vd_all, *raw = w.raw, *tprime = w.tprime;
    TH_REQUIRE(raw != nullptr && tprime != nullptr && gws != nullptr, "workspace too small");

    ThProf* pf = prof_of(c);
    int32_t* hp = c->host_pinned;
    if ((prepass == 0 || prepass == 2) && pool != nullptr) c->after_shade_valid = false;
    if (prepass == 2 || prepass == 3) {
        hp = c->host_pinned + 16 + 4 * slot;
        TH_HIP(hipStreamWaitEvent(s, c->prepass[slot].ev, 0));
        ThWaitClock wc(c);
        TH_HIP(hipEventSynchronize(c->prepass[slot].ev));
    } else {
    ProfScope sc_hull(pf, TH_PROF_HULL, s);
    const bool no_hull = f->hull_thresh < 0.f;
    if (no_hull) {
        TH_HIP(hipMemsetAsync(info, 0, 16 * 4, s));
        TH_HIP(hipMemsetAsync(mask, 1, (size_t)P, s));
        if (ray_mode) TH_HIP(hipMemsetAsync(ray_hit, 1, (size_t)R * 4, s));
    } else {
        TH_TRY(th_hull_mask_launch(ps, P, f->verts_world, f->n_verts, f->hull_thresh, mask,
                                   ray_mode ? ray_hit : nullptr, hws, hws_b, s, info));
    }
    if (ray_mode) {
        TH_TRY(th_view_embed_launch(ps.ray_d, R, 4, vd_all, s, ray_hit));
        TH_TRY(th_compact_mask_rule(mask, P, ray_hit, R, S, no_hull ? R : f->small_frame_rays, info, idx, info + 2, cws,
                                    cws_b, s));
    } else {
        TH_TRY(th_compact_mask(mask, P, idx, info + 2, cws, cws_b, s));
    }
    sc_hull.close();
    if (prepass == 1) {
        TH_HIP(hipMemcpyAsync(c->host_pinned + 16 + 4 * slot, info, 4 * 4, hipMemcpyDeviceToHost, s));
        if (!c->prepass[slot].ev) TH_HIP(hipEventCreateWithFlags(&c->prepass[slot].ev, hipEventDisableTiming));
        TH_HIP(hipEventRecord(c->prepass[slot].ev, s));
        return 0;
    }
    TH_HIP(hipMemcpyAsync(c->host_pinned, info, 4 * 4, hipMemcpyDeviceToHost, s));
    ThWaitClock wc(c);
    TH_HIP(hipStreamSynchronize(s));
    }
    const int hit_rays = hp[0], unmasked = hp[1], n = hp[2];
    if (stats_host) { stats_host[0] = hit_rays; stats_host[1] = n; stats_host[2] = -1; stats_host[3] = unmasked; }
    th_ctx::Prepass* tk = (prepass == 2 || prepass == 3) ? &c->prepass[slot] : nullptr;
    const bool demand_miss = f->map_source != nullptr && f->map_source->demand != nullptr &&
                             !(tk && tk->demand == f->map_source->demand);
    if (f->map_source != nullptr && n > 0 && !(tk && tk->map_done == f->pixel_map_nhwc) &&
        !(f->map_source->demand != nullptr && c->map_completed != nullptr && c->map_completed == f->pixel_map_nhwc &&
          c->map_completed_demand == (const void*)f->map_source->demand) &&
        (f->map_source->demand != nullptr ? demand_miss
                                          : (unmasked || f->hull_thresh < 0.f || f->hull_thresh > f->map_source->reach))) {
        const th_map_source* ms = f->map_source;
        TH_REQUIRE(f->map_channels == TH_MAP_SPLIT && ms->img && ms->lat0 && ms->lat1 && ms->lat2, "map_source: split map only");
        TH_TRY(th_upsample_concat_launch(ms->img, ms->lat0, ms->lat1, ms->lat2, ms->dims, V, f->H, f->W, nullptr, nullptr,
                                         const_cast<float*>(f->pixel_map_nhwc), s, 1, nullptr));
        if (tex) TH_TRY(th_map_fold_launch(c->fused, f->pixel_map_nhwc, V, f->H, f->W, nullptr, const_cast<float*>(f->map_fold),
                                           c->range_dev, s));
        if (tk) tk->map_done = f->pixel_map_nhwc;
        if (f->map_source->demand != nullptr) {
            c->map_completed = f->pixel_map_nhwc;
            c->map_completed_demand = (const void*)f->map_source->demand;
        }
    }
    const bool can_pre = ray_mode && tok_gather(c, V) && fmt == TH_ROWS_SPLIT;
    char* pb = (char*)pool;
    if (prepass == 3) {
        th_ctx::Prepass& t = c->prepass[slot];
        t.npre = 0;
        if (!can_pre || n <= 0) return 0;
        const PoolPlan pl = pool_plan(c, V, f_ld, n, true, tex);
        TH_REQUIRE(pool != nullptr && pool_bytes >= pl.total, "shading pool too small (th_shade_pool_bytes)");
        const int m = (int)pl.pre_n;
        float* a_f = (float*)(pb + pl.a_f);
        float* a_h = (float*)(pb + pl.a_h);
        float* a_pe = (float*)(pb + pl.a_pe);
        const bool grid = getenv("TH_DPARF_NOGRID") == nullptr && th_dparf_grid_ok(f->n_clusters);
        if (!c->aux) {
            TH_HIP(hipStreamCreateWithFlags(&c->aux, hipStreamNonBlocking));
            TH_HIP(hipEventCreateWithFlags(&c->aux_fork, hipEventDisableTiming));
            TH_HIP(hipEventCreateWithFlags(&c->aux_join, hipEventDisableTiming));
            TH_HIP(hipStreamCreateWithFlags(&c->aux2, hipStreamNonBlocking));
            TH_HIP(hipEventCreateWithFlags(&c->aux2_join, hipEventDisableTiming));
        }
        const bool early = c->pregather_early && c->after_shade_valid && c->after_shade_stream == s &&
                           c->after_shade_pool == pool;
        c->after_shade_valid = false;
        if (early) {
            TH_HIP(hipStreamWaitEvent(c->aux, c->after_shade, 0));
            if (tex) TH_HIP(hipStreamWaitEvent(c->aux2, c->after_shade, 0));
        } else {
            TH_HIP(hipEventRecord(c->aux_fork, s));
            TH_HIP(hipStreamWaitEvent(c->aux, c->aux_fork, 0));
            if (tex) TH_HIP(hipStreamWaitEvent(c->aux2, c->aux_fork, 0));
        }
        hipStream_t s4 = c->aux, s5 = tex ? c->aux2 : s;
        int rc = 0;
        {
            if (grid && t.grid_centres != f->centres) rc = th_dparf_grid_build(f->centres, f->n_clusters, gws, gws_b, s4);
            t.grid_centres = nullptr;
            if (rc == 0) {
                ProfScope ps1(pf, TH_PROF_DPARF, s4);
                rc = th_dparf_launch(nullptr, &ps, f->Rh, f->Th, idx, m, f->centres, f->rot, nullptr, V, f->n_clusters, 0.5f, a_h,
                                     a_pe, TH_ROWS_NBR, grid ? gws : nullptr, s4);
            }
            if (rc == 0) {
                ProfScope ps2(pf, TH_PROF_GATHER, s5);
                rc = tex ? th_pixtex_launch(V, f->H, f->W, &ps, idx, m, f->cams, f->scale_xy, a_f, s5)
                         : th_pixgather_launch(f->pixel_map_nhwc, V, f->map_channels, f->H, f->W, nullptr, &ps, idx, m, f->cams,
                                               f->scale_xy, a_f, f_ld, fmt, s, c->range_dev);
            }
        }
        t.pre_tokens = nullptr;
        if (rc == 0 && c->pregather_early && f->tokens != nullptr) {
            const float* table = nullptr;
            rc = token_table(c, f->tokens, V, f->n_clusters, tprime, &table, s);
            if (rc == 0) t.pre_tokens = f->tokens;
        }
        const hipError_t e1 = hipEventRecord(c->aux_join, c->aux);
        const hipError_t e2 = e1 == hipSuccess ? hipStreamWaitEvent(s, c->aux_join, 0) : e1;
        if (e2 != hipSuccess) (void)hipStreamSynchronize(c->aux);
        if (s5 != s) {
            const hipError_t e3 = hipEventRecord(c->aux2_join, c->aux2);
            const hipError_t e4 = e3 == hipSuccess ? hipStreamWaitEvent(s, c->aux2_join, 0) : e3;
            if (e4 != hipSuccess) (void)hipStreamSynchronize(c->aux2);
        }
        if (rc != 0) return rc;
        if (!t.ev2) TH_HIP(hipEventCreateWithFlags(&t.ev2, hipEventDisableTiming));
        TH_HIP(hipEventRecord(t.ev2, s));
        t.npre = m;
        t.pre_map = f->pixel_map_nhwc;
        t.pre_centres = f->centres;
        t.pre_pool = pool;
        return 0;
    }
    int npre = 0;
    if (prepass == 2) {
        th_ctx::Prepass& t = c->prepass[slot];
        if (t.npre > 0 && can_pre && t.pre_map == f->pixel_map_nhwc && t.pre_centres == f->centres && t.pre_pool == pool) {
// ... 301 lines not shown
```

transhuman_amd/csrc/th_internal.h:

```cpp
#pragma once
#include <hip/hip_runtime.h>
#include <stdint.h>
#include <stddef.h>
#include <time.h>
#include <string>

#include "transhuman_hip.h"

#define TH_WAVE 64

void th_set_error(const std::string& msg);
#define TH_FAIL(msg)                                                                \
    do {                                                                            \
        th_set_error(std::string(__func__) + ": " + (msg));                         \
        return -1;                                                                  \
    } while (0)
#define TH_REQUIRE(cond, msg)                                                       \
    do {                                                                            \
        if (!(cond)) TH_FAIL(msg);                                                  \
    } while (0)
#define TH_HIP(call)                                                                \
    do {                                                                            \
        hipError_t e__ = (call);                                                    \
        if (e__ != hipSuccess) {                                                    \
// ... 136 lines not shown
    b.w11 = (ix - x0) * (iy - y0);
    int xi0 = (int)x0, yi0 = (int)y0, xi1 = xi0 + 1, yi1 = yi0 + 1;
    bool bx1 = xi1 <= W - 1, by1 = yi1 <= H - 1;
    if (!bx1) { b.w01 = 0.f; b.w11 = 0.f; xi1 = W - 1; }
    if (!by1) { b.w10 = 0.f; b.w11 = 0.f; yi1 = H - 1; }
    b.i00 = yi0 * W + xi0; b.i01 = yi0 * W + xi1; b.i10 = yi1 * W + xi0; b.i11 = yi1 * W + xi1;
    b.x0 = xi0; b.y0 = yi0; b.x1 = xi1; b.y1 = yi1;
    return b;
}

__device__ __forceinline__ void th_project(const float* __restrict__ cam, float x, float y, float z, float& u,
                                           float& v) {
    float cx = fmaf(cam[2], z, fmaf(cam[1], y, cam[0] * x)) + cam[9];
    float cy = fmaf(cam[5], z, fmaf(cam[4], y, cam[3] * x)) + cam[10];
    float cz = fmaf(cam[8], z, fmaf(cam[7], y, cam[6] * x)) + cam[11];
    const float* K = cam + 12;
    float px = fmaf(K[2], cz, fmaf(K[1], cy, K[0] * cx));
    float py = fmaf(K[5], cz, fmaf(K[4], cy, K[3] * cx));
    float pz = fmaf(K[8], cz, fmaf(K[7], cy, K[6] * cx));
    u = px / pz;
    v = py / pz;
}

#endif

struct ThMlpPacked {
    ThPacked fc_0, alpha_res_0, kv0, kv1, fc_1, fc_2, fc_3, feature_fc, rgb_res_0, view_fc, rgb_res_1, fc_4;
    ThPacked fc_0tok;
    ThPacked alpha_res_0c, rgb_res_0c, rgb_res_1c;
    bool compact_ready = false;
    float *alpha_w = nullptr, *alpha_b = nullptr;
    float *rgb_w = nullptr, *rgb_b = nullptr;
    bool ready = false;
};
struct ThVitBlockPacked {
    float *ln1_w, *ln1_b, *ln2_w, *ln2_b;
    ThPacked qkv, proj, fc1, fc2;
};
struct ThVitPacked {
    int depth = 0, dim = 0, heads = 0;
    ThVitBlockPacked* blocks = nullptr;
    float *norm_w = nullptr, *norm_b = nullptr;
    bool ready = false;
};

struct FusedLayer {
    const uint4* w;
    const float* bias;
    float inv_scale;
    int CT, KB;
    float inv_scale2;
};
struct Fused16 {
    FusedLayer fc_0pe, kv1, kv0, fc_2, fc_3, fc_4, vfA, vfD;
};
struct FusedParams {
    Fused16 w16;
    int waves;
    FusedLayer fc_0pe;
    FusedLayer kv1, ar0, kv0, fc_1, fc_2, fc_3, fc_4;
    FusedLayer vfA, vfD, rst;
    FusedLayer ar0c, rstc;
    bool compact_ready;
    const float *alpha_w, *alpha_b, *rgb_w, *rgb_b;
    const float* stok;
    const _Float16* tsplit;
    const float* t_inv;
    int t_nc;
    const _Float16* pe;
    const _Float16* f;
    const unsigned* tex_hdr;
    const unsigned* tex_rec;
    const float* tex_map;
    const float* tex_map2;
    const float* vd;
    const int32_t* vd_sel;
    int vd_div;
    float* raw_c;
    int P;
    int rgb_all;
    unsigned int* range;
    long long* dbg;
    long long* cycles_buf;
};
enum { TH_RANGE_F = 0, TH_RANGE_S = 1, TH_RANGE_P = 2, TH_RANGE_N = 3, TH_RANGE_INTER = 4, TH_RANGE_F4 = 5, TH_RANGE_CONV = 6,
       TH_RANGE_VIT = 7 };
size_t th_fused_pack_bytes();
int th_fused_pack(const th_mlp_weights* w, const th_linear* folded, void* store, FusedParams* out, hipStream_t s);
int th_mlp_fused_forward(const FusedParams& base, const ThMlpPacked& heads, int V, int P, const float* stok,
                         const void* pe, const void* f, int f_ld, const float* vd, const int32_t* vd_sel, int vd_div, int rgb_all,
                         float* raw_c, unsigned int* range, hipStream_t s, const void* tsplit = nullptr,
                         const float* t_inv = nullptr, int t_nc = 0, const float* tex_map = nullptr, size_t tex_stride = 0);
static inline bool th_lds_attr_needed(unsigned long long* done) {
    int dev = 0;
    if (hipGetDevice(&dev) != hipSuccess || dev < 0 || dev > 63) return true;
    if ((*done >> dev) & 1ull) return false;
    *done |= 1ull << dev;
    return true;
}
int th_map_fold_launch(const FusedParams& base, const float* map_split, int V, int H, int W, const int32_t* box, float* fold,
                       unsigned int* range, hipStream_t s, const unsigned* demand = nullptr );
size_t th_pixtex_bytes(int V, long long P);
int th_pixtex_launch(int V, int H, int W, const ThPointSrc* ps, const int32_t* sel, int P, const float* cams,
                     const float* scale, void* out, hipStream_t s);
int th_tok_split(float* tprime, int rows, float* sc, unsigned int* range, hipStream_t s);

struct th_ctx {
    void* fused_store = nullptr;
    FusedParams fused{};
    bool fused_ready = false;
    int mlp_mode = 1;
    int vit_mode = 1;
    int tok_gather = 1;
    int tex_rows = 1;
    int device = 0;
    void* mlp_store = nullptr;
    void* vit_store = nullptr;
    ThMlpPacked mlp;
    ThVitPacked vit;
    int32_t* host_pinned = nullptr;
    struct Prepass {
        hipEvent_t ev = nullptr;
        const void* ws = nullptr;
        const void* rays = nullptr;
        int R = 0, S = 0;
        bool valid = false;
        hipEvent_t ev2 = nullptr;
        int npre = 0;
        const void* pre_map = nullptr;
        const void* pre_centres = nullptr;
        const void* pre_pool = nullptr;
        const void* grid_centres = nullptr;
        const void* pre_tokens = nullptr;
        const void* demand = nullptr;
        const void* map_done = nullptr;
    };
    static constexpr int kPrepassSlots = 4;
    Prepass prepass[kPrepassSlots];
    int prepass_rr = 0;
    int n_cu = 256;
    const void* map_completed = nullptr;
    const void* map_completed_demand = nullptr;
    hipStream_t aux = nullptr, aux2 = nullptr;
    hipEvent_t aux_fork = nullptr, aux_join = nullptr, aux2_join = nullptr;
    hipEvent_t after_shade = nullptr;
    hipStream_t after_shade_stream = nullptr;
    const void* after_shade_pool = nullptr;
    bool after_shade_valid = false, pregather_early = false;
    void* prof = nullptr;
    unsigned int* range_dev = nullptr;
    unsigned int* range_host = nullptr;
    static constexpr int kRangeSnaps = 8;
    hipEvent_t range_ev[kRangeSnaps] = {};
    int range_gen[kRangeSnaps] = {-1, -1, -1, -1, -1, -1, -1, -1};
    int range_gen_next = 0, range_last = -1;
    double host_wait_ms = 0.0;
};
struct ThWaitClock {
    th_ctx* c;
    timespec t0;
    explicit ThWaitClock(th_ctx* c_) : c(c_) { clock_gettime(CLOCK_MONOTONIC, &t0); }
    ~ThWaitClock() {
        timespec t1;
        clock_gettime(CLOCK_MONOTONIC, &t1);
        c->host_wait_ms += (t1.tv_sec - t0.tv_sec) * 1e3 + (t1.tv_nsec - t0.tv_nsec) * 1e-6;
    }
};

size_t th_hull_ws(int n_verts);
int th_hull_mask_launch(const ThPointSrc& ps, long long P, const float* verts, int nv, float thresh,
                        uint8_t* mask, int32_t* ray_hit, void* ws, size_t ws_bytes, hipStream_t s,
                        int32_t* info_zero = nullptr);
int th_compact_mask_rule(uint8_t* mask, long long P, const int32_t* ray_hit, int R, int S, int thr, int32_t* dev_info,
                         int32_t* idx_out, int32_t* dev_count, void* ws, size_t ws_bytes, hipStream_t s);
size_t th_compact_ws(long long P);
int th_compact_mask(const uint8_t* mask, long long P, int32_t* idx_out, int32_t* dev_count, void* ws,
                    size_t ws_bytes, hipStream_t s);
int th_small_frame_rule(uint8_t* mask, const int32_t* ray_hit, int R, int S, int thr, int32_t* dev_info,
                        hipStream_t s);

int th_paint_launch(const float* map, int V, int C, int H, int W, const float* verts, int nv, const float* cams,
                    const float* scale, const uint8_t* viz, float* painted, hipStream_t s);
int th_segmean_launch(const float* src, int batch, long long batch_stride, int width, const int32_t* off,
                      const int32_t* mem, int nc, float* out, hipStream_t s);
int th_segmean_rot_launch(const double* blend, const int32_t* off, const int32_t* mem, int nc, float* rot,
                          hipStream_t s);
int th_nchw_to_nhwc_launch(const float* src, int V, int C, int H, int W, float* dst, hipStream_t s);

enum { TH_ROWS_F32 = 0, TH_ROWS_SPLIT = 1, TH_ROWS_FOLDED = 2, TH_ROWS_NBR = 3 };
int th_dparf_launch(const float* pts_smpl, const ThPointSrc* ps, const float* Rh, const float* Th,
                    const int32_t* sel, int P, const float* centres, const float* rot, const float* tokens,
                    int V, int nc, float alpha, float* out, float* pe_out, int fmt, const void* grid_ws,
                    hipStream_t s);
static inline bool th_dparf_grid_ok(int nc) { return nc >= 7 && (size_t)nc * 16 <= 64 * 1024; }
size_t th_dparf_grid_ws(int nc);
int th_dparf_grid_build(const float* centres, int nc, void* ws, size_t ws_bytes, hipStream_t s);
int th_pixgather_launch(const float* map, int V, int C, int H, int W, const float* pts_world,
// ... 63 lines not shown
```

transhuman_amd/hip.py:

```python
import ctypes as C
import os

import torch

_HERE = os.path.dirname(os.path.abspath(__file__))
LIB_PATH = os.environ.get("TH_LIB_PATH") or os.path.join(_HERE, "libtranshuman_hip.so")

c_float_p = C.POINTER(C.c_float)


class ThLinear(C.Structure):
    _fields_ = [("w", C.c_void_p), ("b", C.c_void_p), ("out_f", C.c_int), ("in_f", C.c_int)]


class ThMlpWeights(C.Structure):
    _names = ["fc_0", "alpha_res_0", "key0", "val0", "key1", "val1", "fc_1", "fc_2", "fc_3", "alpha_fc",
              "feature_fc", "rgb_res_0", "view_fc", "rgb_res_1", "fc_4", "rgb_fc", "upsample_color"]
    _fields_ = [(n, ThLinear) for n in _names]


class ThSmplModel(C.Structure):
    _fields_ = [("v_template", C.c_void_p), ("shapedirs", C.c_void_p), ("posedirs", C.c_void_p),
                ("J_regressor", C.c_void_p), ("weights", C.c_void_p), ("parent", C.c_void_p), ("n_verts", C.c_int)]


class ThVitBlock(C.Structure):
    _fields_ = [("ln1_w", C.c_void_p), ("ln1_b", C.c_void_p), ("ln2_w", C.c_void_p), ("ln2_b", C.c_void_p),
                ("qkv", ThLinear), ("proj", ThLinear), ("fc1", ThLinear), ("fc2", ThLinear)]


class ThPoints(C.Structure):
    _fields_ = [("pts", C.c_void_p), ("ray_o", C.c_void_p), ("ray_d", C.c_void_p), ("near", C.c_void_p),
                ("far", C.c_void_p), ("t_vals", C.c_void_p), ("one_minus_t", C.c_void_p), ("R", C.c_int),
                ("S", C.c_int), ("z_vals", C.c_void_p), ("sigma_noise", C.c_void_p)]


class ThFrame(C.Structure):
    _fields_ = [("verts_world", C.c_void_p), ("n_verts", C.c_int), ("Rh", C.c_void_p), ("Th", C.c_void_p),
                ("cams", C.c_void_p), ("scale_xy", C.c_void_p), ("pixel_map_nhwc", C.c_void_p), ("V", C.c_int),
                ("H", C.c_int), ("W", C.c_int), ("map_channels", C.c_int), ("tokens", C.c_void_p), ("centres", C.c_void_p),
                ("rot", C.c_void_p), ("n_clusters", C.c_int), ("hull_thresh", C.c_float),
                ("small_frame_rays", C.c_int), ("map_source", C.c_void_p), ("map_fold", C.c_void_p)]


class ThMapSource(C.Structure):
    _fields_ = [("box", C.c_void_p), ("reach", C.c_float), ("img", C.c_void_p), ("lat0", C.c_void_p),
                ("lat1", C.c_void_p), ("lat2", C.c_void_p), ("dims", C.c_int32 * 6), ("demand", C.c_void_p)]


SYMBOLS = {
    "th_abi_version": (C.c_int, []),
    "th_last_error": (C.c_char_p, []),
    "th_sizeof": (C.c_size_t, [C.c_char_p]),
    "th_ctx_create": (C.c_int, [C.c_int, C.POINTER(C.c_void_p)]),
    "th_ctx_destroy": (None, [C.c_void_p]),
    "th_profile_enable": (C.c_int, [C.c_void_p, C.c_int]),
    "th_profile_read": (C.c_int, [C.c_void_p, C.POINTER(C.c_double), C.POINTER(C.c_int64)]),
    "th_fused_cycles": (C.c_int, [C.c_void_p, C.c_void_p]),
    "th_host_wait_read": (C.c_int, [C.c_void_p, C.POINTER(C.c_double)]),
    "th_clock_probe": (C.c_int, [C.c_void_p, C.c_void_p, C.c_void_p]),
    "th_set_mlp_weights": (C.c_int, [C.c_void_p, C.POINTER(ThMlpWeights), C.c_void_p]),
    "th_set_mlp_mode": (C.c_int, [C.c_void_p, C.c_int]),
    "th_set_fused_waves": (C.c_int, [C.c_void_p, C.c_int]),
    "th_set_vit_mode": (C.c_int, [C.c_void_p, C.c_int]),
    "th_set_tok_gather": (C.c_int, [C.c_void_p, C.c_int]),
    "th_set_tex_rows": (C.c_int, [C.c_void_p, C.c_int]),
    "th_map_fold": (C.c_int, [C.c_void_p, C.c_void_p, C.c_int, C.c_int, C.c_int, C.c_void_p, C.c_void_p, C.c_void_p]),
    "th_pixel_texlist_bytes": (C.c_size_t, [C.c_int, C.c_int]),
    "th_pixel_texlist": (C.c_int, [C.c_void_p, C.c_void_p, C.c_int, C.c_int, C.c_int, C.c_void_p, C.c_void_p, C.c_int,
                                   C.c_void_p, C.c_void_p, C.c_void_p, C.c_size_t, C.c_void_p]),
    "th_range_snapshot": (C.c_int, [C.c_void_p, C.c_void_p]),
    "th_range_read": (C.c_int, [C.c_void_p, C.c_int, C.POINTER(C.c_uint32)]),
    "th_range_last_slot": (C.c_int, [C.c_void_p]),
    "th_set_chunk_samples": (C.c_int, [C.c_int]),
    "th_set_vit_weights": (C.c_int, [C.c_void_p, C.c_int, C.c_int, C.c_int, C.POINTER(ThVitBlock), C.c_void_p,
                                     C.c_void_p, C.c_void_p]),
    "th_linear_workspace_bytes": (C.c_size_t, [C.c_int, C.c_int]),
    "th_linear_forward": (C.c_int, [C.c_void_p, C.c_void_p, C.c_int, C.c_int, C.POINTER(ThLinear), C.c_int,
                                    C.c_void_p, C.c_int, C.c_void_p, C.c_size_t, C.c_void_p]),
    "th_hull_workspace_bytes": (C.c_size_t, [C.c_int]),
    "th_hull_mask": (C.c_int, [C.c_void_p, C.POINTER(ThPoints), C.c_void_p, C.c_int, C.c_float, C.c_void_p,
                               C.c_void_p, C.c_void_p, C.c_size_t, C.c_void_p]),
    "th_paint_group": (C.c_int, [C.c_void_p, C.c_void_p, C.c_int, C.c_int, C.c_int, C.c_int, C.c_void_p, C.c_int,
                                 C.c_void_p, C.c_void_p, C.c_void_p, C.c_void_p, C.c_void_p, C.c_int, C.c_void_p,
                                 C.c_void_p, C.c_void_p]),
    "th_segment_mean_f32": (C.c_int, [C.c_void_p, C.c_void_p, C.c_int, C.c_void_p, C.c_void_p, C.c_int, C.c_void_p,
                                      C.c_void_p]),
    "th_segment_mean_rot_f64": (C.c_int, [C.c_void_p, C.c_void_p, C.c_void_p, C.c_void_p, C.c_int, C.c_void_p,
                                          C.c_void_p]),
    "th_upsample_concat_nhwc": (C.c_int, [C.c_void_p, C.c_void_p, C.c_void_p, C.c_void_p, C.c_void_p,
                                          C.POINTER(C.c_int32), C.c_int, C.c_int, C.c_int, C.c_void_p, C.c_void_p,
                                          C.c_void_p, C.c_void_p]),
    "th_upsample_concat_split": (C.c_int, [C.c_void_p, C.c_void_p, C.c_void_p, C.c_void_p, C.c_void_p,
                                           C.POINTER(C.c_int32), C.c_int, C.c_int, C.c_int, C.c_void_p, C.c_void_p]),
    "th_upsample_concat_split_box": (C.c_int, [C.c_void_p, C.c_void_p, C.c_void_p, C.c_void_p, C.c_void_p,
                                               C.POINTER(C.c_int32), C.c_int, C.c_int, C.c_int, C.c_void_p, C.c_void_p,
                                               C.c_void_p]),
    "th_map_demand_bytes": (C.c_size_t, [C.c_int, C.c_int, C.c_int]),
    "th_upsample_concat_split_demand": (C.c_int, [C.c_void_p, C.c_void_p, C.c_void_p, C.c_void_p, C.c_void_p,
                                                  C.POINTER(C.c_int32), C.c_int, C.c_int, C.c_int, C.c_void_p, C.c_void_p,
                                                  C.c_void_p, C.c_void_p]),
    "th_map_fold_demand": (C.c_int, [C.c_void_p, C.c_void_p, C.c_int, C.c_int, C.c_int, C.c_void_p, C.c_void_p, C.c_void_p]),
    "th_render_predemand": (C.c_int, [C.c_void_p, C.POINTER(ThFrame), C.POINTER(ThPoints), C.c_void_p, C.c_size_t, C.c_void_p,
                                      C.c_int, C.c_void_p, C.c_size_t, C.c_void_p]),
    "th_map_box": (C.c_int, [C.c_void_p, C.c_void_p, C.c_int, C.c_void_p, C.c_int, C.c_void_p, C.c_int, C.c_void_p,
                             C.c_int, C.c_int, C.c_float, C.c_void_p, C.c_void_p]),
    "th_paint_group_nhwc_workspace_bytes": (C.c_size_t, [C.c_int, C.c_int, C.c_int, C.c_int]),
    "th_paint_group_nhwc": (C.c_int, [C.c_void_p, C.c_void_p, C.c_int, C.c_int, C.c_int, C.c_int, C.c_void_p, C.c_int,
                                      C.c_void_p, C.c_void_p, C.c_void_p, C.POINTER(ThLinear), C.POINTER(ThLinear),
                                      C.c_void_p, C.c_void_p, C.c_int, C.c_void_p, C.c_void_p, C.c_size_t, C.c_void_p]),
    "th_vit_workspace_bytes": (C.c_size_t, [C.c_int, C.c_int, C.c_int, C.c_int]),
    "th_vit_forward": (C.c_int, [C.c_void_p, C.c_void_p, C.c_void_p, C.c_int, C.c_int, C.c_void_p, C.c_void_p,
                                 C.c_size_t, C.c_void_p]),
    "th_dparf_encode": (C.c_int, [C.c_void_p, C.c_void_p, C.c_void_p, C.c_int, C.c_void_p, C.c_void_p, C.c_void_p,
                                  C.c_int, C.c_int, C.c_void_p, C.c_void_p]),
    "th_nchw_to_nhwc": (C.c_int, [C.c_void_p, C.c_void_p, C.c_int, C.c_int, C.c_int, C.c_int, C.c_void_p,
                                  C.c_void_p]),
    "th_pixel_gather": (C.c_int, [C.c_void_p, C.c_void_p, C.c_int, C.c_int, C.c_int, C.c_int, C.c_void_p,
                                  C.c_void_p, C.c_int, C.c_void_p, C.c_void_p, C.c_void_p, C.c_int, C.c_void_p]),
    "th_pixel_gather_split": (C.c_int, [C.c_void_p, C.c_void_p, C.c_int, C.c_int, C.c_int, C.c_void_p, C.c_void_p, C.c_int,
                                        C.c_void_p, C.c_void_p, C.c_void_p, C.c_int, C.c_void_p]),
    "th_network_workspace_bytes": (C.c_size_t, [C.c_int, C.c_int]),
    "th_network_forward": (C.c_int, [C.c_void_p, C.c_void_p, C.c_void_p, C.c_void_p, C.c_void_p, C.c_int, C.c_void_p,
                                     C.c_void_p, C.c_void_p, C.c_int, C.c_int, C.c_void_p, C.c_void_p, C.c_size_t,
                                     C.c_void_p]),
    "th_composite": (C.c_int, [C.c_void_p, C.c_void_p, C.c_void_p, C.POINTER(ThPoints), C.c_int, C.c_void_p,
                               C.c_void_p, C.c_void_p, C.c_void_p, C.c_void_p]),
    "th_gen_rays": (C.c_int, [C.c_void_p, c_float_p, c_float_p, c_float_p, c_float_p, C.c_int, C.c_int, C.c_void_p,
                              C.c_void_p, C.c_void_p, C.c_void_p, C.c_void_p, C.c_void_p]),
    "th_bound_mask": (C.c_int, [C.c_void_p, C.POINTER(C.c_int32), C.c_int, C.c_int, C.c_void_p, C.c_void_p]),
    "th_ssim_workspace_bytes": (C.c_size_t, [C.c_int, C.c_int, C.c_int]),
    "th_ssim": (C.c_int, [C.c_void_p, C.c_void_p, C.c_void_p, C.c_int, C.c_int, C.c_int, C.c_int, C.c_void_p, C.c_void_p,
                          C.c_size_t, C.c_void_p]),
    "th_lpips_pack_bytes": (C.c_size_t, []),
    "th_lpips_pack": (C.c_int, [C.c_void_p, C.c_void_p, C.c_void_p, C.c_void_p, C.c_void_p, C.c_size_t, C.c_void_p]),
    "th_lpips_workspace_bytes": (C.c_size_t, [C.c_int, C.c_int, C.c_int]),
    "th_lpips": (C.c_int, [C.c_void_p, C.c_void_p, C.c_void_p, C.c_int, C.c_int, C.c_int, C.c_void_p, C.c_void_p,
                           C.c_void_p, C.c_size_t, C.c_void_p]),
    "th_marching_cubes_workspace_bytes": (C.c_size_t, [C.c_int, C.c_int, C.c_int]),
    "th_marching_cubes_count": (C.c_int, [C.c_void_p, C.c_void_p, C.c_int, C.c_int, C.c_int, C.c_float, C.c_void_p,
                                          C.c_size_t, C.POINTER(C.c_int64), C.c_void_p]),
    "th_marching_cubes_range": (C.c_int, [C.c_void_p, C.c_void_p, C.c_int, C.c_int, C.c_int, C.c_int,
                                          C.POINTER(C.c_int64), C.c_void_p]),
    "th_marching_cubes_emit": (C.c_int, [C.c_void_p, C.c_void_p, C.c_int, C.c_int, C.c_int, C.c_float, C.c_void_p,
                                         C.c_int, C.c_int, C.POINTER(C.c_double), C.POINTER(C.c_double), C.c_void_p,
                                         C.c_void_p, C.c_void_p]),
    "th_smpl_workspace_bytes": (C.c_size_t, [C.c_int]),
    "th_smpl_lbs": (C.c_int, [C.c_void_p, C.POINTER(ThSmplModel), C.c_void_p, C.c_void_p, C.c_void_p, C.c_void_p,
                              C.c_void_p, C.c_void_p, C.c_void_p, C.c_size_t, C.c_void_p]),
    "th_view_embed": (C.c_int, [C.c_void_p, C.c_void_p, C.c_int, C.c_int, C.c_void_p, C.c_void_p]),
    "th_render_workspace_bytes": (C.c_size_t, [C.POINTER(ThFrame), C.c_int, C.c_int]),
    "th_shade_pool_bytes": (C.c_size_t, [C.c_void_p, C.POINTER(ThFrame), C.c_longlong, C.c_int]),
    "th_render_prepass_wait": (C.c_int, [C.c_void_p, C.c_void_p, C.POINTER(C.c_int64)]),
    "th_render_rays": (C.c_int, [C.c_void_p, C.POINTER(ThFrame), C.POINTER(ThPoints), C.c_void_p, C.c_void_p,
                                 C.c_void_p, C.c_int, C.c_void_p, C.c_size_t, C.c_void_p, C.c_size_t,
                                 C.POINTER(C.c_int64), C.c_void_p]),
    "th_render_prepass": (C.c_int, [C.c_void_p, C.POINTER(ThFrame), C.POINTER(ThPoints), C.c_void_p, C.c_size_t,
                                    C.c_void_p]),
    "th_render_pregrid": (C.c_int, [C.c_void_p, C.POINTER(ThFrame), C.POINTER(ThPoints), C.c_void_p, C.c_size_t,
                                    C.c_void_p]),
    "th_render_pregather": (C.c_int, [C.c_void_p, C.POINTER(ThFrame), C.POINTER(ThPoints), C.c_void_p, C.c_size_t,
                                      C.c_void_p, C.c_size_t, C.c_void_p]),
    "th_render_pregather_early": (C.c_int, [C.c_void_p, C.POINTER(ThFrame), C.POINTER(ThPoints), C.c_void_p, C.c_size_t,
                                      C.c_void_p, C.c_size_t, C.c_void_p]),
    "th_conv_pack_bytes": (C.c_size_t, [C.c_int, C.c_int, C.c_int]),
    "th_conv_pack": (C.c_int, [C.c_void_p, C.c_void_p, C.c_int, C.c_int, C.c_int, C.c_void_p, C.c_size_t,
                               C.POINTER(C.c_float), C.c_void_p]),
    "th_conv2d_supported": (C.c_int, [C.c_int, C.c_int, C.c_int, C.c_int]),
    "th_conv2d": (C.c_int, [C.c_void_p, C.c_void_p, C.c_int, C.c_int, C.c_int, C.c_int, C.c_void_p, C.c_float, C.c_int,
                            C.c_int, C.c_int, C.c_void_p, C.c_void_p]),
    "th_maxpool3x3s2": (C.c_int, [C.c_void_p, C.c_void_p, C.c_int, C.c_int, C.c_int, C.c_void_p, C.c_void_p]),
    "th_bn_workspace_bytes": (C.c_size_t, [C.c_int, C.c_int, C.c_int]),
    "th_bn_act": (C.c_int, [C.c_void_p, C.c_void_p, C.c_void_p, C.c_int, C.c_int, C.c_int, C.c_void_p, C.c_void_p,
                            C.c_float, C.c_float, C.c_void_p, C.c_void_p, C.c_int, C.c_void_p, C.c_void_p, C.c_size_t,
                            C.c_void_p]),
    "th_bn_act_eval": (C.c_int, [C.c_void_p, C.c_void_p, C.c_void_p, C.c_int, C.c_int, C.c_int, C.c_void_p, C.c_void_p,
                                 C.c_float, C.c_void_p, C.c_void_p, C.c_int, C.c_void_p, C.c_void_p]),
    "th_conv2d_stats_partials": (C.c_int, [C.c_int] * 7),
    "th_conv2d_stats": (C.c_int, [C.c_void_p, C.c_void_p, C.c_int, C.c_int, C.c_int, C.c_int, C.c_void_p, C.c_float, C.c_int,
                                  C.c_int, C.c_int, C.c_void_p, C.c_void_p, C.c_size_t, C.c_void_p]),
    "th_bn_act_stats": (C.c_int, [C.c_void_p, C.c_void_p, C.c_void_p, C.c_int, C.c_int, C.c_int, C.c_void_p, C.c_int,
                                  C.c_void_p, C.c_void_p, C.c_float, C.c_float, C.c_void_p, C.c_void_p, C.c_int, C.c_void_p,
                                  C.c_void_p]),
    "th_render_prepass_cancel": (C.c_int, [C.c_void_p]),
    "th_render_prepass_drop": (C.c_int, [C.c_void_p, C.c_void_p]),
# ... 296 lines not shown
            self.pts = _f32(pts).reshape(-1, 3)
            self.R, self.S = self.pts.shape[0], 1
            self.keep = (self.pts,)
            self.c = ThPoints(_p(self.pts), None, None, None, None, None, None, self.R, 1)
            return
        self.ray_o, self.ray_d = _f32(ray_o).reshape(-1, 3), _f32(ray_d).reshape(-1, 3)
        self.near, self.far = _f32(near).reshape(-1), _f32(far).reshape(-1)
        dev = self.ray_o.device
        self.t, self.omt = _t_vals(n_samples, dev)
        self.R, self.S = self.ray_o.shape[0], n_samples
        self.z_vals = None if z_vals is None else _f32(z_vals).reshape(self.R, self.S)
        self.sigma_noise = None if sigma_noise is None else _f32(sigma_noise).reshape(self.R, self.S)
        self.c = ThPoints(None, _p(self.ray_o), _p(self.ray_d), _p(self.near), _p(self.far), _p(self.t), _p(self.omt),
                          self.R, self.S, _p(self.z_vals), _p(self.sigma_noise))


_t_cache = {}


def _t_vals(n_samples, dev):
    key = (int(n_samples), str(dev))
    if key not in _t_cache:
        t = torch.linspace(0.0, 1.0, steps=n_samples)
        _t_cache[key] = (t.to(dev), (1.0 - t).to(dev))
    return _t_cache[key]


def hull_mask(points, verts_world, thresh=0.1):
    lib = load_library()
    v = _f32(verts_world).reshape(-1, 3)
    P = points.R * points.S
    mask = torch.empty(P, dtype=torch.uint8, device=v.device)
    hit = torch.empty(points.R, dtype=torch.int32, device=v.device)
    ws = _ws(lib.th_hull_workspace_bytes(v.shape[0]), v.device)
    _check(lib.th_hull_mask(ctx(v.device), C.byref(points.c), _p(v), v.shape[0], thresh, _p(mask), _p(hit), _p(ws),
                            ws.numel(), _stream()))
    return mask.view(points.R, points.S).bool(), hit.bool()


def pack_cams(R, T, K):
    V = R.shape[0]
    return torch.cat([_f32(R).reshape(V, 9), _f32(T).reshape(V, 3), _f32(K).reshape(V, 9)], dim=1).contiguous()


def feat_scale(scale_np, image_shape, device):
    import numpy as np
    s = np.asarray(scale_np, dtype=np.float64) / np.asarray(image_shape, dtype=np.float64)
    key = (float(s[0]), float(s[1]), str(device))
    if key not in _scale_cache:
        _scale_cache[key] = torch.tensor(s).to(dtype=torch.float32, device=device)
    return _scale_cache[key]


_scale_cache = {}


def csr_to_device(offsets, members, device):
    return (torch.as_tensor(offsets, dtype=torch.int32, device=device).contiguous(),
            torch.as_tensor(members, dtype=torch.int32, device=device).contiguous())


def paint_group(holder_map, verts_world, cams, scale_xy, vizmap, off, mem, return_painted=False):
    lib = load_library()
    m = _f32(holder_map)
    V, Cc, H, W = m.shape
    v = _f32(verts_world).reshape(-1, 3)
    nc = off.numel() - 1
    viz = vizmap.to(torch.uint8).contiguous() if vizmap is not None else None
    painted = torch.empty((V, v.shape[0], Cc), dtype=torch.float32, device=m.device)
    tokens = torch.empty((V, nc, Cc), dtype=torch.float32, device=m.device)
    _check(lib.th_paint_group(ctx(m.device), _p(m), V, Cc, H, W, _p(v), v.shape[0], _p(cams), _p(scale_xy), _p(viz),
                              _p(off), _p(mem), nc, _p(painted), _p(tokens), _stream()))
    return (tokens, painted) if return_painted else tokens


class SplitMap:

    def __init__(self, buf, V, H, W, source=None):
        self.buf, self.V, self.H, self.W = buf, V, H, W
        self.shape = (V, H, W, 256)
        self.device = buf.device
        self.source = source
        self.fold = None

    @property
    def box(self):
        return self.source[1][0] if self.source is not None else None

    @property
    def demand(self):
        return self.source[1][5] if self.source is not None and len(self.source[1]) > 5 else None

    def data_ptr(self):
        return self.buf.data_ptr()

    @property
    def latents(self):
        return self.buf[: self.V * self.H * self.W * 256].view(self.V, self.H, self.W, 256)

    @property
    def rgb0(self):
        return self.buf[self.V * self.H * self.W * 256:].view(self.V, self.H, self.W, 4)

    def interleaved(self):
        return torch.cat([self.latents, self.rgb0], dim=-1).contiguous()


def map_fold(net, split_map):
    assert isinstance(split_map, SplitMap)
    _sync_weights(net, "mlp")
    V, H, W = split_map.V, split_map.H, split_map.W
    fold = torch.empty((2, V, H, W, 256), dtype=torch.float32, device=split_map.device)
    if split_map.demand is not None:
        _check(load_library().th_map_fold_demand(ctx(split_map.device), _p(split_map), V, H, W, _p(split_map.demand), _p(fold), _stream()))
        split_map.fold = fold
        return fold
    if split_map.box is not None:
        _box_checked(split_map.box, H)
    _check(load_library().th_map_fold(ctx(split_map.device), _p(split_map), V, H, W, _p(split_map.box), _p(fold), _stream()))
    split_map.fold = fold
    return fold


def map_box(verts_a, verts_b, cams, scale_xy, H, W, reach):
    lib = load_library()
    a = _f32(verts_a).reshape(-1, 3)
    b = _f32(verts_b).reshape(-1, 3) if verts_b is not None else None
    V = cams.shape[0]
    buf = torch.empty(V * 4 + V * int(H) * 2 + V, dtype=torch.int32, device=a.device)
    box = buf[: V * 4].view(V, 4)
    box._th_map_box = (buf, int(H))
    _check(lib.th_map_box(ctx(a.device), _p(a), a.shape[0], _p(b), b.shape[0] if b is not None else 0, _p(cams), V,
                          _p(scale_xy), int(H), int(W), float(reach), _p(box), _stream()))
    return box


def _box_checked(box, H):
    tag = getattr(box, "_th_map_box", None)
    if tag is None or tag[0].data_ptr() != box.data_ptr() or tag[1] != int(H):
        raise HipError("box must be the tensor hip.map_box returned for this image height (its row spans follow it in memory)")
    return box


def map_spans(box, H):
    _box_checked(box, H)
    V = box.shape[0]
    return torch.as_strided(box, (V, int(H), 2), (int(H) * 2, 2, 1), storage_offset=box.storage_offset() + V * 4)


def upsample_concat_split(images, lat0, lat1, lat2, box=None, reach=0.0, demand=None):
    lib = load_library()
    img, l0, l1, l2 = _f32(images), _f32(lat0), _f32(lat1), _f32(lat2)
    V, _, H, W = img.shape
    assert l0.shape[1] == 64 and l1.shape[1] == 64 and l2.shape[1] == 128
    dims = (C.c_int32 * 6)(l0.shape[2], l0.shape[3], l1.shape[2], l1.shape[3], l2.shape[2], l2.shape[3])
    buf = torch.empty(V * H * W * 260, dtype=torch.float32, device=img.device)
    if demand is not None:
        _check(lib.th_upsample_concat_split_demand(ctx(img.device), _p(img), _p(l0), _p(l1), _p(l2), dims, V, H, W, _p(buf), None,
                                                   _p(demand), _stream()))
        src = ThMapSource(None, float(reach), _p(img), _p(l0), _p(l1), _p(l2), dims, _p(demand))
        return SplitMap(buf, V, H, W, source=(src, (None, img, l0, l1, l2, demand)))
    if box is None:
        _check(lib.th_upsample_concat_split(ctx(img.device), _p(img), _p(l0), _p(l1), _p(l2), dims, V, H, W, _p(buf), _stream()))
        return SplitMap(buf, V, H, W)
    assert box.dtype == torch.int32 and tuple(box.shape) == (V, 4) and box.is_contiguous()
    _box_checked(box, H)
    _check(lib.th_upsample_concat_split_box(ctx(img.device), _p(img), _p(l0), _p(l1), _p(l2), dims, V, H, W, _p(buf),
                                            _p(box), _stream()))
    src = ThMapSource(_p(box), float(reach), _p(img), _p(l0), _p(l1), _p(l2), dims, None)
    return SplitMap(buf, V, H, W, source=(src, (box, img, l0, l1, l2)))


def upsample_concat_nhwc(images, lat0, lat1, lat2, color_w=None, color_b=None):
    lib = load_library()
    img, l0, l1, l2 = _f32(images), _f32(lat0), _f32(lat1), _f32(lat2)
    V, _, H, W = img.shape
    assert l0.shape[1] == 64 and l1.shape[1] == 64 and l2.shape[1] == 128
    dims = (C.c_int32 * 6)(l0.shape[2], l0.shape[3], l1.shape[2], l1.shape[3], l2.shape[2], l2.shape[3])
    cw = _f32(color_w).reshape(128, 3) if color_w is not None else None
    cb = _f32(color_b) if color_w is not None else None
    out = torch.empty((V, H, W, 384 if color_w is not None else 260), dtype=torch.float32, device=img.device)
    _check(lib.th_upsample_concat_nhwc(ctx(img.device), _p(img), _p(l0), _p(l1), _p(l2), dims, V, H, W, _p(cw), _p(cb),
                                       _p(out), _stream()))
    return out


def paint_group_nhwc(map_nhwc, verts_world, cams, scale_xy, vizmap, red_w, red_b, off, mem, color_w=None,
                     color_b=None):
    lib = load_library()
    V, H, W, Cc = map_nhwc.shape
    v = _f32(verts_world).reshape(-1, 3)
    nc = off.numel() - 1
    viz = vizmap.to(torch.uint8).contiguous() if vizmap is not None else None
    lin, keep = _linear(red_w, red_b)
    lift, keep2 = _linear(color_w, color_b) if color_w is not None else (None, None)
    tokens = torch.empty((V, nc, lin.out_f), dtype=torch.float32, device=v.device)
    ws = _ws(lib.th_paint_group_nhwc_workspace_bytes(V, v.shape[0], Cc, lin.out_f), v.device)
    _check(lib.th_paint_group_nhwc(ctx(v.device), _p(map_nhwc), V, H, W, Cc, _p(v), v.shape[0], _p(cams), _p(scale_xy),
                                   _p(viz), C.byref(lin), C.byref(lift) if lift is not None else None, _p(off), _p(mem),
                                   nc, _p(tokens), _p(ws), ws.numel(), _stream()))
    return tokens


_conv_cache = {}


def conv2d_supported(conv):
    ks, st, pd = conv.kernel_size, conv.stride, conv.padding
    return (not conv_fallback(conv.weight.device) and conv.bias is None and ks[0] == ks[1] and st[0] == st[1] and pd[0] == pd[1] == ks[0] // 2 and
            conv.groups == 1 and conv.dilation == (1, 1) and
            bool(load_library().th_conv2d_supported(conv.in_channels, conv.out_channels, ks[0], st[0])))


def conv2d(x, conv, stats=False):
    lib = load_library()
    assert x.dim() == 4 and x.dtype == torch.float32 and x.is_contiguous()
    w = conv.weight
    key = id(conv)
    ent = _conv_cache.get(key)
    if ent is None or ent[0] is not w or ent[1] != w._version or ent[2].device != x.device:
        co, ci, ks, _ = w.shape
        buf = torch.empty(lib.th_conv_pack_bytes(co, ci, ks), dtype=torch.uint8, device=x.device)
        inv = C.c_float()
        _check(lib.th_conv_pack(ctx(x.device), _p(_f32(w)), co, ci, ks, _p(buf), buf.numel(), C.byref(inv), _stream()))
        ent = (w, w._version, buf, float(inv.value))
        _conv_cache[key] = ent
    N, ci, H, W = x.shape
    co, ks, st = conv.out_channels, conv.kernel_size[0], conv.stride[0]
    pd = ks // 2
    Ho, Wo = (H + 2 * pd - ks) // st + 1, (W + 2 * pd - ks) // st + 1
    y = torch.empty((N, co, Ho, Wo), dtype=torch.float32, device=x.device)
    if stats:
        npart = int(lib.th_conv2d_stats_partials(N, ci, H, W, co, ks, st))
        sbuf = torch.empty((co, npart, 2), dtype=torch.float32, device=x.device)
        _check(lib.th_conv2d_stats(ctx(x.device), _p(x), N, ci, H, W, _p(ent[2]), ent[3], co, ks, st, _p(y), _p(sbuf),
                                   sbuf.numel() * 4, _stream()))
        return y, (sbuf, npart)
    _check(lib.th_conv2d(ctx(x.device), _p(x), N, ci, H, W, _p(ent[2]), ent[3], co, ks, st, _p(y), _stream()))
    return y


def maxpool3x3s2(x):
    assert x.dim() == 4 and x.dtype == torch.float32 and x.is_contiguous()
    N, Cc, H, W = x.shape
    y = torch.empty((N, Cc, (H - 1) // 2 + 1, (W - 1) // 2 + 1), dtype=torch.float32, device=x.device)
    _check(load_library().th_maxpool3x3s2(ctx(x.device), _p(x), N * Cc, H, W, _p(y), _stream()))
    return y


def bn_act(x, bn, residual=None, relu=True, conv_stats=None):
    lib = load_library()
    assert x.dim() == 4 and x.is_contiguous() and x.dtype == torch.float32
    N, Cc, H, W = x.shape
    r = None if residual is None else residual.contiguous()
    if not bn.training:
        assert bn.track_running_stats and bn.running_mean is not None, "eval-mode BatchNorm without running statistics"
        y = torch.empty_like(x)
        _check(lib.th_bn_act_eval(ctx(x.device), _p(x), None if r is None else _p(r), N, Cc, H * W,
                                  None if bn.weight is None else _p(bn.weight), None if bn.bias is None else _p(bn.bias),
                                  float(bn.eps), _p(bn.running_mean), _p(bn.running_var), int(relu), _p(y), _stream()))
        return y
    y = torch.empty_like(x)
    track = bn.track_running_stats and bn.running_mean is not None
    assert bn.momentum is not None, "cumulative-average BatchNorm (momentum=None) is not handled here"
    mom = float(bn.momentum)
    r = None if residual is None else residual.contiguous()
    if conv_stats is not None:
        sbuf, npart = conv_stats
        assert sbuf.shape == (Cc, npart, 2) and sbuf.dtype == torch.float32 and sbuf.device == x.device
        _check(lib.th_bn_act_stats(ctx(x.device), _p(x), None if r is None else _p(r), N, Cc, H * W, _p(sbuf), npart,
                                   None if bn.weight is None else _p(bn.weight), None if bn.bias is None else _p(bn.bias),
                                   float(bn.eps), mom, _p(bn.running_mean) if track else None,
                                   _p(bn.running_var) if track else None, int(relu), _p(y), _stream()))
        return y
    ws = _ws(lib.th_bn_workspace_bytes(N, Cc, H * W), x.device)
    _check(lib.th_bn_act(ctx(x.device), _p(x), None if r is None else _p(r), N, Cc, H * W,
                         None if bn.weight is None else _p(bn.weight), None if bn.bias is None else _p(bn.bias),
                         float(bn.eps), mom, _p(bn.running_mean) if track else None,
                         _p(bn.running_var) if track else None, int(relu), _p(y), _p(ws), ws.numel(), _stream()))
    return y
# ... 312 lines not shown
    _check(lib.th_lpips(ctx(a.device), _p(a), _p(b), N, H, W, _p(packed), _p(out), _p(ws), ws.numel(), _stream()))
    return out


def marching_cubes(cube, iso, scale=(1.0, 1.0, 1.0), origin=(0.0, 0.0, 0.0), x_range=None):
    lib = load_library()
    c = _f32(cube)
    assert c.dim() == 3
    X, Y, Z = c.shape
    dev = c.device
    ws = _ws(lib.th_marching_cubes_workspace_bytes(X, Y, Z), dev)
    counts = (C.c_int64 * 2)()
    _check(lib.th_marching_cubes_count(ctx(dev), _p(c), X, Y, Z, float(iso), _p(ws), ws.numel(), counts, _stream()))
    nv, nt = int(counts[0]), int(counts[1])
    verts = torch.zeros((nv, 3), dtype=torch.float64, device=dev)
    tris = torch.zeros((nt, 3), dtype=torch.int32, device=dev)
    sc = (C.c_double * 3)(*[float(v) for v in scale])
    og = (C.c_double * 3)(*[float(v) for v in origin])
    x0, x1 = (0, X) if x_range is None else (int(x_range[0]), int(x_range[1]))
    if nv > 0:
        _check(lib.th_marching_cubes_emit(ctx(dev), _p(c), X, Y, Z, float(iso), _p(ws), x0, x1, sc, og,
                                          _p(verts), _p(tris) if nt > 0 else _p(verts), _stream()))
    if x_range is None:
        return verts, tris
    a, b = (C.c_int64 * 2)(), (C.c_int64 * 2)()
    _check(lib.th_marching_cubes_range(ctx(dev), _p(ws), X, Y, Z, max(x0, 0), a, _stream()))
    _check(lib.th_marching_cubes_range(ctx(dev), _p(ws), X, Y, Z, min(x1, X), b, _stream()))
    return verts, tris, (int(a[0]), int(b[0])), (int(a[1]), int(b[1]))


class SmplModel:

    def __init__(self, arrays, device=None):
        dev = torch.device("cuda", torch.cuda.current_device()) if device is None else torch.device(device)
        f64 = lambda k: torch.as_tensor(arrays[k], dtype=torch.float64).contiguous().to(dev)
        self.v_template, self.shapedirs, self.posedirs = f64("v_template"), f64("shapedirs"), f64("posedirs")
        self.J_regressor, self.weights = f64("J_regressor"), f64("weights")
        self.parent = torch.as_tensor(arrays["parent"], dtype=torch.int32).contiguous().to(dev)
        self.nv = self.v_template.shape[0]
        assert self.shapedirs.shape == (self.nv, 3, 10) and self.posedirs.shape == (self.nv, 3, 207)
        assert self.J_regressor.shape == (24, self.nv) and self.weights.shape == (self.nv, 24)
        self.c = ThSmplModel(_p(self.v_template), _p(self.shapedirs), _p(self.posedirs), _p(self.J_regressor),
                             _p(self.weights), _p(self.parent), self.nv)

    def __call__(self, pose, beta):
        lib = load_library()
        dev = self.v_template.device
        p = torch.as_tensor(pose, dtype=torch.float32).contiguous().to(dev)
        b = torch.as_tensor(beta, dtype=torch.float64).reshape(10).contiguous().to(dev)
        is_rot = tuple(p.shape) == (24, 3, 3)
        assert is_rot or p.numel() == 72, "Unsupported Pose Inputs"
        v = torch.empty((self.nv, 3), dtype=torch.float64, device=dev)
        j = torch.empty((24, 3), dtype=torch.float64, device=dev)
        T = torch.empty((self.nv, 4, 4), dtype=torch.float64, device=dev)
        ws = _ws(lib.th_smpl_workspace_bytes(self.nv), dev)
        _check(lib.th_smpl_lbs(ctx(dev), C.byref(self.c), None if is_rot else _p(p), _p(p) if is_rot else None, _p(b),
                               _p(v), _p(j), _p(T), _p(ws), ws.numel(), _stream()))
        return v, j, T


def view_embed(ray_d, view_res=4):
    lib = load_library()
    d = _f32(ray_d).reshape(-1, 3)
    out = torch.empty((d.shape[0], 3 + 6 * view_res), dtype=torch.float32, device=d.device)
    _check(lib.th_view_embed(ctx(d.device), _p(d), d.shape[0], view_res, _p(out), _stream()))
    return out


class Frame:

    def __init__(self, verts_world, Rh, Th, cams, scale_xy, pixel_map_nhwc, tokens, centres, rot,
                 hull_thresh=0.1, small_frame_rays=2400):
        self.verts = _f32(verts_world).reshape(-1, 3)
        self.Rh, self.Th = _f32(Rh).reshape(9), _f32(Th).reshape(3)
        self.cams, self.scale = cams, scale_xy
        self.map = pixel_map_nhwc
        self.centres, self.rot = _f32(centres).reshape(-1, 3), _f32(rot).reshape(-1, 9)
        self.tokens = _f32(tokens) if tokens is not None else None
        V, H, W, Cc = pixel_map_nhwc.shape
        assert Cc in (384, 260) or isinstance(pixel_map_nhwc, SplitMap), \
            "pixel map must be the full (384) or the compact (260 interleaved / SplitMap) channels-last map"
        src = getattr(pixel_map_nhwc, "source", None)
        self.c = ThFrame(_p(self.verts), self.verts.shape[0], _p(self.Rh), _p(self.Th), _p(self.cams), _p(self.scale),
                         _p(self.map), V, H, W, Cc, _p(self.tokens), _p(self.centres), _p(self.rot),
                         self.centres.shape[0], hull_thresh, small_frame_rays,
                         C.cast(C.pointer(src[0]), C.c_void_p).value if src is not None else None,
                         _p(getattr(pixel_map_nhwc, "fold", None)))

    def set_tokens(self, tokens):
        self.tokens = _f32(tokens)
        assert self.tokens.shape[1] == self.centres.shape[0]
        self.c.tokens = self.tokens.data_ptr()


_ws_cache = {}


def _cached_ws(nbytes, device, slot=0):
    key = (str(device), slot)
    cur = _ws_cache.get(key)
    if cur is None or cur.numel() < nbytes:
        _ws_cache[key] = None
        cur = torch.empty(int(nbytes), dtype=torch.uint8, device=device)
        _ws_cache[key] = cur
    return cur


_pool_cache = {}


def _shade_pool(frame_c, n_valid, with_pregather, device, slot=None):
    need = int(load_library().th_shade_pool_bytes(ctx(device), C.byref(frame_c), int(n_valid), int(with_pregather)))
    key = str(device) if slot is None else (str(device), int(slot))
    cur = _pool_cache.get(key)
    if cur is None or cur.numel() < need:
        _pool_cache[key] = None
        cur = torch.empty(int(need * 1.0625) + 4096, dtype=torch.uint8, device=device)
        _pool_cache[key] = cur
    cur.record_stream(torch.cuda.current_stream(device))
    return cur


def _prepass_counts(ws, device):
    out = (C.c_int64 * 3)()
    rc = load_library().th_render_prepass_wait(ctx(device), _p(ws), out)
    if rc == 1:
        return None
    _check(rc)
    return int(out[0]), int(out[1]), int(out[2])


def drop_workspaces(device=None):
    lib = load_library()
    for key in list(_pool_cache.keys()):
        dev = key if isinstance(key, str) else key[0]
        if device is None or str(device) == dev:
            _pool_cache.pop(key, None)
    for (dev, _slot) in list(_ws_cache.keys()):
        if device is None or str(device) == dev:
            _ws_cache.pop((dev, _slot), None)
    try:
        _check(lib.th_render_prepass_cancel(ctx(device)))
    except HipError:
        pass


def render_prepass(points, verts_world, V, hull_thresh=0.1, small_frame_rays=2400, n_clusters=0, slot=0):
    lib = load_library()
    v = _f32(verts_world).reshape(-1, 3)
    dev = v.device
    f = ThFrame()
    f.verts_world, f.n_verts, f.V = v.data_ptr(), v.shape[0], V
    f.hull_thresh, f.small_frame_rays, f.map_channels = hull_thresh, small_frame_rays, 384
    f.n_clusters = n_clusters
    ws = _cached_ws(lib.th_render_workspace_bytes(C.byref(f), points.R, points.S), dev, slot)
    points._prepass_keep = (v, ws)
    points._prepass_nc = int(n_clusters)
    _check(lib.th_render_prepass(ctx(dev), C.byref(f), C.byref(points.c), _p(ws), ws.numel(), _stream()))
    points._prepass_pending = True


def render_predemand(points, cams, scale_xy, V, H, W, verts_paint=None):
    if not getattr(points, "_prepass_pending", False) or int(W) % 64 != 0 or V > 3:
        return None
    lib = load_library()
    v, ws = points._prepass_keep
    dev = v.device
    f = ThFrame()
    f.verts_world, f.n_verts, f.V, f.H, f.W = v.data_ptr(), v.shape[0], int(V), int(H), int(W)
    f.cams, f.scale_xy = cams.data_ptr(), scale_xy.data_ptr()
    f.n_clusters, f.map_channels = points._prepass_nc, 384
    vp = _f32(verts_paint).reshape(-1, 3) if verts_paint is not None else None
    nb = int(lib.th_map_demand_bytes(int(V), int(H), int(W)))
    demand = torch.empty(nb, dtype=torch.uint8, device=dev)
    rc = lib.th_render_predemand(ctx(dev), C.byref(f), C.byref(points.c), _p(ws), ws.numel(), _p(vp), vp.shape[0] if vp is not None else 0,
                                 _p(demand), nb, _stream())
    if rc == 1:
        return None
    _check(rc)
    demand._keep = (vp, cams, scale_xy)
    return demand


def render_pregrid(frame, points):
    if not getattr(points, "_prepass_pending", False):
        return
    _, ws = points._prepass_keep
    _check(load_library().th_render_pregrid(ctx(frame.verts.device), C.byref(frame.c), C.byref(points.c), _p(ws), ws.numel(),
                                            _stream()))


def render_pregather(net, frame, points, slot=0, early=False, pool_slot=None):
    if not getattr(points, "_prepass_pending", False):
        return
    lib = load_library()
    _sync_weights(net, "mlp")
    dev = frame.verts.device
    _, ws = points._prepass_keep
    cnt = _prepass_counts(ws, dev)
    if cnt is None:
        return
    pool = _shade_pool(frame.c, cnt[2], True, dev, pool_slot)
    points._pregathered = True
    fn = lib.th_render_pregather_early if early else lib.th_render_pregather
    _check(fn(ctx(dev), C.byref(frame.c), C.byref(points.c), _p(ws), ws.numel(), _p(pool), pool.numel(), _stream()))


def render_rays(net, frame, points, white_bkgd=False, defer_guard=False, small_frame_rays=None, pool_slot=None):
    lib = load_library()
    _sync_weights(net, "mlp")
    dev = frame.verts.device
    R = points.R
    rgb = torch.empty((R, 3), dtype=torch.float32, device=dev)
    acc = torch.empty(R, dtype=torch.float32, device=dev)
    dep = torch.empty(R, dtype=torch.float32, device=dev)
    if R == 0:
        st0 = dict(hit_rays=0, valid_samples=0, unmasked=0)
        return (rgb, acc, dep, st0, lambda: True) if defer_guard else (rgb, acc, dep, st0)
    fc = frame.c
    if small_frame_rays is not None and int(small_frame_rays) != fc.small_frame_rays:
        fc = ThFrame.from_buffer_copy(frame.c)
        fc.small_frame_rays = int(small_frame_rays)
    need = lib.th_render_workspace_bytes(C.byref(fc), R, points.S)
    n_bound, pre = R * points.S, False
    if getattr(points, "_prepass_pending", False) and points._prepass_keep[1].numel() >= need:
        points._prepass_pending = False
        ws = points._prepass_keep[1]
        cnt = _prepass_counts(ws, dev)
        if cnt is not None:
            n_bound, pre = cnt[2], bool(getattr(points, "_pregathered", False))
    else:
        ws = _cached_ws(need, dev)
        _check(lib.th_render_prepass_drop(ctx(dev), _p(ws)))
    points._pregathered = False
    pool = _shade_pool(fc, n_bound, pre, dev, pool_slot)
    stats = (C.c_int64 * 4)()
    _check(lib.th_render_rays(ctx(dev), C.byref(fc), C.byref(points.c), _p(rgb), _p(acc), _p(dep), int(white_bkgd),
                              _p(ws), ws.numel(), _p(pool), pool.numel(), stats, _stream()))
    st = dict(hit_rays=stats[0], valid_samples=stats[1], unmasked=stats[3])
    slot = int(stats[2])
    if defer_guard:
        return rgb, acc, dep, st, (lambda: _guard(dev, slot))
    for _ in range(3):
        if _guard(dev, slot):
            break
        if (conv_fallback(dev) or vit_fallback(dev)) and getattr(frame, "rebuild", None) is not None:
            frame = frame.rebuild()
            keep_sfr = fc.small_frame_rays
            fc = ThFrame.from_buffer_copy(frame.c)
            fc.small_frame_rays = keep_sfr
        _check(lib.th_render_prepass_drop(ctx(dev), _p(ws)))
        pool = _shade_pool(fc, st["valid_samples"], False, dev, pool_slot)
        _check(lib.th_render_rays(ctx(dev), C.byref(fc), C.byref(points.c), _p(rgb), _p(acc), _p(dep),
                                  int(white_bkgd), _p(ws), ws.numel(), _p(pool), pool.numel(), stats, _stream()))
        st = dict(hit_rays=stats[0], valid_samples=stats[1], unmasked=stats[3])
        slot = int(stats[2])
    return rgb, acc, dep, st


def eval_sigma_grid(net, frame, pts):
    lib = load_library()
    _sync_weights(net, "mlp")
    p = _f32(pts).reshape(-1, 3)
    P = p.shape[0]
    out = torch.empty(P, dtype=torch.float32, device=p.device)
    if P == 0:
        return out, dict(valid_samples=0)
    ws = _cached_ws(lib.th_sigma_grid_workspace_bytes(C.byref(frame.c), P), p.device)
    stats = (C.c_int64 * 4)()
    for _ in range(3):
        pool = _shade_pool(frame.c, P, False, p.device)
        _check(lib.th_eval_sigma_grid(ctx(p.device), C.byref(frame.c), _p(p), P, _p(out), _p(ws), ws.numel(), _p(pool),
                                      pool.numel(), stats, _stream()))
        if _guard(p.device, int(stats[2])):
            break
        if (conv_fallback(p.device) or vit_fallback(p.device)) and getattr(frame, "rebuild", None) is not None:
            frame = frame.rebuild()
    return out, dict(valid_samples=stats[1])


def set_tok_gather(on, device=None):
    _check(load_library().th_set_tok_gather(ctx(device), 1 if on else 0))


_tex_rows = {}


def tex_rows_enabled(device=None):
    if _tex_rows:
        d = _dev_index(device)
        if d in _tex_rows:
            return _tex_rows[d]
    return os.environ.get("TH_ROWS_TEX", "1")[:1] != "0"


def mlp_is_fused(device=None):
    d = _dev_index(device)
    return _user_mode.get(d, 1) == 1 and not _range_fallback.get(d)


def set_tex_rows(on, device=None):
    _check(load_library().th_set_tex_rows(ctx(device), 1 if on else 0))
    _tex_rows[_dev_index(device)] = bool(on)


def set_mlp_mode(mode, device=None):
    _check(load_library().th_set_mlp_mode(ctx(device), int(mode)))
    d = _dev_index(device)
    _user_mode[d] = int(mode)
    _range_fallback.pop(d, None)


_fused_waves = {}


def set_fused_waves(waves, device=None):
    _check(load_library().th_set_fused_waves(ctx(device), int(waves)))
    _fused_waves[_dev_index(device)] = int(waves)


def fused_waves(device=None):
    dflt = 4 if os.environ.get("TH_FUSED_WAVES", "8")[:1] == "4" else 8
    if device is None and not torch.cuda.is_available():
        return dflt
    return _fused_waves.get(_dev_index(device), dflt)


def set_chunk_samples(n):
    _check(load_library().th_set_chunk_samples(int(n)))


PROF_PHASES = ("hull", "dparf", "gather", "mlp", "composite", "vit", "fold", "_7")


def profile_enable(on=True, device=None):
    _check(load_library().th_profile_enable(ctx(device), int(on)))


def profile_read(device=None):
    ms = (C.c_double * 8)()
    cnt = (C.c_int64 * 8)()
    _check(load_library().th_profile_read(ctx(device), ms, cnt))
    return {PROF_PHASES[i]: (ms[i], cnt[i]) for i in range(7)}


def clock_probe(out):
    assert out.dtype == torch.int64 and out.numel() >= 3 and out.is_cuda
    _check(load_library().th_clock_probe(ctx(out.device), _p(out), _stream()))


def fused_cycles(counters, device=None):
    if counters is not None:
        assert counters.dtype == torch.int64 and counters.numel() >= 64 and counters.is_cuda
# ... 18 lines not shown
```

transhuman_amd/networks/renderer/if_clight_renderer.py:

```python
import os
import sys

_REPO = os.path.dirname(os.path.dirname(os.path.dirname(os.path.dirname(os.path.abspath(__file__)))))
if _REPO not in sys.path:
    sys.path.insert(0, _REPO)
import pickle

import numpy as np
import torch

from transhuman_amd.config import get_cfg
from transhuman_amd import hip, synth


class Renderer:
    def __init__(self, net, vertex_can=None, pc2voxel_ind=None):
        cfg = get_cfg()
        self.net = net
        self.faces = None
        if vertex_can is None:
            with open("./data/smplx/smpl/SMPL_NEUTRAL.pkl", "rb") as f:
                data = pickle.load(f, encoding="latin1")
            vertex_can = np.asarray(data["v_template"])
            self.faces = data["f"]
        self.vertex_can = torch.as_tensor(np.asarray(vertex_can)).contiguous()
        self.CR = torch.tensor([-1.5, -1.5, -1.5, 1.5, 1.5, 1.5])
        voxel2pc = None
        if pc2voxel_ind is None:
            num_voxel = cfg.num_class
            path = f"./kmeans_dict/kmeans_dict_{num_voxel}.npy"
            pc2voxel_ind, voxel2pc = np.load(path, allow_pickle=True).item().values()
            pc2voxel_ind = np.asarray(pc2voxel_ind)
        self.pc2voxel_ind = torch.as_tensor(np.asarray(pc2voxel_ind)).type(torch.int64)
        if voxel2pc is not None:
            lists = [np.asarray(v, dtype=np.int64).reshape(-1) for v in voxel2pc.values()]
            self.csr_offsets = np.concatenate([[0], np.cumsum([len(v) for v in lists])]).astype(np.int64)
            self.csr_members = np.concatenate(lists).astype(np.int64)
        else:
            self.csr_offsets, self.csr_members = synth.csr_from_assign(self.pc2voxel_ind.numpy())
        self.num_clusters = len(self.csr_offsets) - 1
        self.voxel_PE_can = self._host_segment_mean(self.vertex_can)
        self._dev = {}

    def _host_segment_mean(self, x):
        out = [x[torch.as_tensor(self.csr_members[self.csr_offsets[c]:self.csr_offsets[c + 1]], dtype=torch.long)].mean(0)
               for c in range(self.num_clusters)]
        return torch.stack(out)

    def normalize_PE(self, PE, CR=None):
        assert len(PE.shape) == 3
        CR = self.CR if CR is None else CR
        mn, mx = CR[:3][None, None, :].to(PE.device), CR[3:][None, None, :].to(PE.device)
        return ((((PE - mn) / (mx - mn)) - 0.5) * 2).type(torch.float32)

    def voxelization(self, src):
        off, mem = self._csr(src.device)
        return hip.segment_mean(src, off, mem)

    def _csr(self, device):
        key = ("csr", str(device))
        if key not in self._dev:
            self._dev[key] = hip.csr_to_device(self.csr_offsets, self.csr_members, device)
        return self._dev[key]

    def _pe_norm(self, V, device):
        key = ("pe", V, str(device))
        if key not in self._dev:
            pe = self.voxel_PE_can.unsqueeze(0).repeat(V, 1, 1)
            self._dev[key] = self.normalize_PE(pe).to(device)
        return self._dev[key]

    def prepare_frame(self, batch, hull_thresh=None, fused_encoder_tail=True, compact_map=True, token_exchange=None,
                      pregather=None, defer_tokens=False, stem_exchange=None, crop_map=None, demand=None, stem_graph=False):
        cfg = get_cfg()
        assert cfg.time_steps == 1
        t = 0
        hip._sync_weights(self.net, "mlp")
        images = batch["input_imgs"][t]
        images = images.reshape(-1, *images.shape[2:])
        dev = images.device
        cams = hip.pack_cams(batch["input_R"][t].reshape(-1, 3, 3), batch["input_T"][t].reshape(-1, 3, 1),
                             batch["input_K"][t].reshape(-1, 3, 3))
        image_shape = batch["input_imgs"][t].shape[-2:]
        off, mem = self._csr(dev)
        viz = batch["input_vizmaps"][t][0] if cfg.rasterize else None
        enc = self.net.encoder
        fold_done = None
        if fused_encoder_tail and hasattr(enc, "trunk"):
            H, W = images.shape[2:]
            V = images.shape[0]
            trunk = (lambda im: enc.trunk(im, graph=True)) if stem_graph else enc.trunk
            lat = trunk(images) if stem_exchange is None else stem_exchange.latents(trunk, images)
            stem_flag = None if stem_exchange is None else stem_exchange.last_flag
            if stem_exchange is not None and hip.conv_fallback(dev) and not stem_exchange.last_mine:
                lat, stem_flag = enc.trunk(images), None
            cw, cb = enc.upsample_color.weight, enc.upsample_color.bias
            scale = hip.feat_scale(enc.feat_scale(H, W), image_shape, dev)
            thr = cfg_hull() if hull_thresh is None else hull_thresh
            if crop_map is None:
                crop_map = os.environ.get("TH_MAP_CROP") != "0"
            if compact_map == "interleaved":
                map_nhwc = hip.upsample_concat_nhwc(images, lat[0], lat[1], lat[2])
            elif compact_map and demand is not None:
                torch.cuda.current_stream(dev).wait_event(demand[1])
                map_nhwc = hip.upsample_concat_split(images, lat[0], lat[1], lat[2], demand=demand[0])
            elif compact_map and crop_map and thr >= 0:
                reach = float(thr) * 1.001 + 1e-6
                box = hip.map_box(batch["tar_smpl_vertice"][0], batch["input_smpl_vertice"][t][0], cams, scale, H, W, reach)
                map_nhwc = hip.upsample_concat_split(images, lat[0], lat[1], lat[2], box=box, reach=reach)
            elif compact_map:
                map_nhwc = hip.upsample_concat_split(images, lat[0], lat[1], lat[2])
            else:
                map_nhwc = hip.upsample_concat_nhwc(images, lat[0], lat[1], lat[2], cw, cb)
            if (isinstance(map_nhwc, hip.SplitMap) and hip.tex_rows_enabled(dev) and V <= 3 and V * H * W < (1 << 22)
                    and hip.mlp_is_fused(dev)):
                if pregather is not None:
                    cur = torch.cuda.current_stream(dev)
                    fs = self._dev.get(("fold_stream", str(dev)))
                    if fs is None:
                        fs = self._dev[("fold_stream", str(dev))] = torch.cuda.Stream(dev)
                    hip._sync_weights(self.net, "mlp")
                    fs.wait_stream(cur)
                    with torch.cuda.stream(fs):
                        fold = hip.map_fold(self.net, map_nhwc)
                        fold_done = torch.cuda.Event()
                        fold_done.record(fs)
                    fold.record_stream(cur)
                else:
                    hip.map_fold(self.net, map_nhwc)

            def group():
                return hip.paint_group_nhwc(map_nhwc, batch["input_smpl_vertice"][t][0], cams, scale, viz,
                                            enc.reduction_layer.weight, enc.reduction_layer.bias, off, mem,
                                            color_w=cw if compact_map else None, color_b=cb if compact_map else None)
            pix_scale = scale
        else:
            holder_map, holder_scale, pixel_map, pixel_scale = enc(images)
            V, _, H, W = pixel_map.shape

            def group():
                return hip.paint_group(holder_map, batch["input_smpl_vertice"][t][0], cams,
                                       hip.feat_scale(holder_scale, image_shape, dev), viz, off, mem)
            map_nhwc = hip.nchw_to_nhwc(pixel_map)
            pix_scale = hip.feat_scale(pixel_scale, image_shape, dev)

        def make_tokens():
            self.last_grouped = group()
            return self.net.ViT(self.last_grouped, self._pe_norm(V, dev), mask=None, graph=stem_graph)

        centres = hip.segment_mean(batch["tar_smpl_vertice_smplcoord"][0], off, mem)
        rot = hip.segment_mean_rot(batch["blend_mtx"][0], off, mem)
        mk_frame = lambda tok: hip.Frame(batch["tar_smpl_vertice"][0], batch["Rh"][0], batch["Th"][0], cams, pix_scale,
                                         map_nhwc, tok, centres, rot,
                                         hull_thresh=cfg_hull() if hull_thresh is None else hull_thresh,
                                         small_frame_rays=2400)
        if token_exchange is not None:
            frame = mk_frame(token_exchange(make_tokens, (V, self.num_clusters, get_cfg().embed_size), dev))
        elif defer_tokens:
            self.last_grouped = grouped = group()
            pe_norm = self._pe_norm(V, dev)
            frame = mk_frame(None)
            frame.finish_tokens = lambda: frame.set_tokens(self.net.ViT(grouped, pe_norm, mask=None, graph=stem_graph))
        elif pregather is None or os.environ.get("TH_PREGATHER") == "0":
            frame = mk_frame(make_tokens())
        else:
            pts_pg, slot_pg = pregather
            cur = torch.cuda.current_stream(dev)
            self.last_grouped = grouped = group()
            grouped_ready = torch.cuda.Event()
            grouped_ready.record(cur)
            frame = mk_frame(None)
            vs = self._dev.get(("vit_stream", str(dev)))
            if vs is None:
                vs = self._dev[("vit_stream", str(dev))] = torch.cuda.Stream(dev)
            with torch.cuda.stream(vs):
                vs.wait_event(grouped_ready)
                tokens = self.net.ViT(grouped, self._pe_norm(V, dev), mask=None, graph=stem_graph)
            hip.render_pregather(self.net, frame, pts_pg, slot_pg)
            grouped.record_stream(vs)
            tokens.record_stream(cur)
            cur.wait_stream(vs)
            frame.set_tokens(tokens)
        if fold_done is not None:
            torch.cuda.current_stream(dev).wait_event(fold_done)
        frame.rebuild = lambda: self.prepare_frame(batch, hull_thresh, fused_encoder_tail, compact_map, crop_map=crop_map)
        frame.stem_flag = stem_flag if (fused_encoder_tail and hasattr(enc, "trunk")) else None
        return frame

    def predemand(self, batch, pts, token_exchange=None, sharded=False):
        mode = os.environ.get("TH_MAP_DEMAND", "auto")
        if mode == "0" or (mode != "1" and not sharded) or not hasattr(self.net.encoder, "trunk"):
            return None
        t = 0
        imgs = batch["input_imgs"][t]
        V, H, W = int(np.prod(imgs.shape[:-3])), int(imgs.shape[-2]), int(imgs.shape[-1])
        dev = imgs.device
        if not (hip.tex_rows_enabled(dev) and hip.mlp_is_fused(dev)) or V > 3 or V * H * W >= (1 << 22):
            return None
# ... 262 lines not shown
```

Baseline: 19.13 million.

## Fold MLP first layer at low-res latent levels before upsampling

Applies the MLP's first linear layer to each encoder latent level at its native low resolution. The resulting 512-wide features are then bilinearly upsampled and summed, with the colour term added through a precomputed lift, so the map fold runs without first materialising the full-resolution upsampled map. Painting and pixel gathering read directly from the latent levels, and the full map is built lazily only when the texture-row path is off. This cuts the matmul work and the memory traffic of building and folding the full-resolution map. The cost is new kernels, a workspace per level, and a small numerical difference because the linear layer and the interpolation are applied in the opposite order.

```diff
diff --git a/include/transhuman_hip.h b/include/transhuman_hip.h
--- a/include/transhuman_hip.h
+++ b/include/transhuman_hip.h
@@ -123,6 +123,11 @@
                         const int32_t* csr_offsets,
                         const int32_t* csr_members, int n_clusters, float* tokens_out, void* workspace,
                         size_t workspace_bytes, th_stream stream);
+int th_paint_group_levels(th_ctx* ctx, const float* img, const float* lat0, const float* lat1, const float* lat2,
+                          const int32_t* dims_host, int V, int H, int W, const float* verts_world, int n_verts,
+                          const float* cams, const float* scale_xy, const uint8_t* vizmap, const th_linear* reduction,
+                          const th_linear* color_lift, const int32_t* csr_offsets, const int32_t* csr_members, int n_clusters,
+                          float* tokens_out, void* workspace, size_t workspace_bytes, th_stream stream);
 
 size_t th_conv_pack_bytes(int cout, int cin, int ks);
 int th_conv_pack(th_ctx* ctx, const float* w, int cout, int cin, int ks, void* packed, size_t packed_bytes,
@@ -165,6 +170,13 @@
 
 int th_map_fold(th_ctx* ctx, const float* map_split, int V, int H, int W, const int32_t* box, float* fold, th_stream stream);
 int th_map_fold_demand(th_ctx* ctx, const float* map_split, int V, int H, int W, const void* demand, float* fold, th_stream stream);
+size_t th_map_fold_levels_workspace_bytes(int V, const int32_t* dims_host);
+int th_map_fold_levels(th_ctx* ctx, const float* img, const float* lat0, const float* lat1, const float* lat2,
+                       const int32_t* dims_host, int V, int H, int W, const int32_t* box, float* map_split, float* fold,
+                       void* workspace, size_t workspace_bytes, th_stream stream);
+int th_map_fold_levels_demand(th_ctx* ctx, const float* img, const float* lat0, const float* lat1, const float* lat2,
+                              const int32_t* dims_host, int V, int H, int W, const void* demand, float* map_split, float* fold,
+                              void* workspace, size_t workspace_bytes, th_stream stream);
 
 size_t th_pixel_texlist_bytes(int V, int P);
 int th_pixel_texlist(th_ctx* ctx, const float* map_split, int V, int H, int W, const float* pts_world, const int32_t* sel,
diff --git a/transhuman_amd/csrc/k_encoder.hip b/transhuman_amd/csrc/k_encoder.hip
--- a/transhuman_amd/csrc/k_encoder.hip
+++ b/transhuman_amd/csrc/k_encoder.hip
@@ -13,6 +13,10 @@
     i1 = i0 + ((i0 < in - 1) ? 1 : 0);
     l1 = src - (float)i0;
     l0 = 1.0f - l1;
+}
+
+__device__ __forceinline__ float ups_blend(float v00, float v01, float v10, float v11, float lx0, float lx1, float ly0, float ly1) {
+    return ly0 * (lx0 * v00 + lx1 * v01) + ly1 * (lx0 * v10 + lx1 * v11);
 }
 
 __global__ __launch_bounds__(256) void upsample_concat_nhwc_kernel(UpsSrc s0, UpsSrc s1, UpsSrc s2,
@@ -61,7 +65,7 @@
         for (int c = wave; c < 64; c += 4) {
             const float* pl = base + (long long)c * s.h * s.w;
             float v00 = pl[y0 * s.w + x0], v01 = pl[y0 * s.w + x1], v10 = pl[y1 * s.w + x0], v11 = pl[y1 * s.w + x1];
-            tile[lane][c] = ly0 * (lx0 * v00 + lx1 * v01) + ly1 * (lx0 * v10 + lx1 * v11);
+            tile[lane][c] = ups_blend(v00, v01, v10, v11, lx0, lx1, ly0, ly1);
         }
     } else {
         int cin0 = (grp - 4) * 64;
@@ -91,6 +95,186 @@
     float* rgb4 = (!wc && split) ? out + (long long)V * H * W * 256 : nullptr;
     hipLaunchKernelGGL(upsample_concat_nhwc_kernel, dim3(th_cdiv(W, 64), H, V * NG), dim3(256), 0, s, s0, s1, s2, img, wc,
                        bc, H, W, NG, CO, out, rgb4, box, need);
+    TH_LAUNCH_CHECK();
+    return 0;
+}
+
+#define FU_RUN 16
+struct FoldLvl {
+    const float* p;
+    int h, w;
+};
+typedef float fu4 __attribute__((ext_vector_type(4)));
+#define FU_CORNERS(k) fu4 k##00 = {0.f, 0.f, 0.f, 0.f}, k##01 = k##00, k##10 = k##00, k##11 = k##00; int k##i0 = -1, k##i1 = -1
+__device__ __forceinline__ fu4 fu_level(fu4& a00, fu4& a01, fu4& a10, fu4& a11, int& ci0, int& ci1, const float* __restrict__ r0,
+                                        const float* __restrict__ r1, int x, int w, int W, float ly0, float ly1) {
+    int i0, i1;
+    float lx0, lx1;
+    ups_coord(x, w, W, i0, i1, lx0, lx1);
+    if (i0 != ci0 || i1 != ci1) {
+        if (i0 == ci1) { a00 = a01; a10 = a11; }
+        else {
+            a00 = *reinterpret_cast<const fu4*>(r0 + (long long)i0 * 512);
+            a10 = *reinterpret_cast<const fu4*>(r1 + (long long)i0 * 512);
+        }
+        if (i1 == i0) { a01 = a00; a11 = a10; }
+        else {
+            a01 = *reinterpret_cast<const fu4*>(r0 + (long long)i1 * 512);
+            a11 = *reinterpret_cast<const fu4*>(r1 + (long long)i1 * 512);
+        }
+        ci0 = i0; ci1 = i1;
+    }
+    fu4 e;
+#pragma unroll
+    for (int j = 0; j < 4; ++j) e[j] = ups_blend(a00[j], a01[j], a10[j], a11[j], lx0, lx1, ly0, ly1);
+    return e;
+}
+__global__ __launch_bounds__(256) void fold_upsample_kernel(FoldLvl s0, FoldLvl s1, FoldLvl s2, const float* __restrict__ img,
+                                                            const float* __restrict__ lc, int V, int H, int W,
+                                                            const int32_t* __restrict__ box, float* __restrict__ fold,
+                                                            float* __restrict__ rgb4) {
+    const int lane = threadIdx.x & 63, wave = __builtin_amdgcn_readfirstlane(threadIdx.x >> 6);
+    const int plane = wave & 1, y = blockIdx.y, v = blockIdx.z;
+    int x0 = 0, x1 = W - 1;
+    if (box != nullptr) {
+        if (y < box[4 * v + 1] || y > box[4 * v + 3]) return;
+        const int32_t* sp = box + 4 * V + ((long long)v * H + y) * 2;
+        x0 = max(sp[0], 0);
+        x1 = min(sp[1], W - 1);
+    }
+    const int xa = x0 + ((int)blockIdx.x * 2 + (wave >> 1)) * FU_RUN;
+    if (xa > x1) return;
+    const int xb = min(xa + FU_RUN - 1, x1);
+    const int ch = plane * 256 + 4 * lane;
+    int yl0, yl1;
+    float ly00, ly01, ly10, ly11, ly20, ly21;
+    ups_coord(y, s0.h, H, yl0, yl1, ly00, ly01);
+    const float* r00 = s0.p + (((long long)v * s0.h + yl0) * s0.w) * 512 + ch;
+    const float* r01 = s0.p + (((long long)v * s0.h + yl1) * s0.w) * 512 + ch;
+    ups_coord(y, s1.h, H, yl0, yl1, ly10, ly11);
+    const float* r10 = s1.p + (((long long)v * s1.h + yl0) * s1.w) * 512 + ch;
+    const float* r11 = s1.p + (((long long)v * s1.h + yl1) * s1.w) * 512 + ch;
+    ups_coord(y, s2.h, H, yl0, yl1, ly20, ly21);
+    const float* r20 = s2.p + (((long long)v * s2.h + yl0) * s2.w) * 512 + ch;
+    const float* r21 = s2.p + (((long long)v * s2.h + yl1) * s2.w) * 512 + ch;
+    const fu4 c0 = *reinterpret_cast<const fu4*>(lc + ch), c1 = *reinterpret_cast<const fu4*>(lc + 512 + ch),
+              c2 = *reinterpret_cast<const fu4*>(lc + 1024 + ch);
+    FU_CORNERS(ka);
+    FU_CORNERS(kb);
+    FU_CORNERS(kc);
+    const long long hw = (long long)H * W;
+    const float* ip = img + (long long)v * 3 * hw + (long long)y * W;
+    float* orow = fold + ((long long)plane * V * hw + (long long)v * hw + (long long)y * W) * 256 + 4 * lane;
+    for (int x = xa; x <= xb; ++x) {
+        const fu4 e0 = fu_level(ka00, ka01, ka10, ka11, kai0, kai1, r00, r01, x, s0.w, W, ly00, ly01);
+        const fu4 e1 = fu_level(kb00, kb01, kb10, kb11, kbi0, kbi1, r10, r11, x, s1.w, W, ly10, ly11);
+        const fu4 e2 = fu_level(kc00, kc01, kc10, kc11, kci0, kci1, r20, r21, x, s2.w, W, ly20, ly21);
+        const float r = ip[x], g = ip[hw + x], b = ip[2 * hw + x];
+        fu4 o;
+#pragma unroll
+        for (int j = 0; j < 4; ++j) o[j] = fmaf(b, c2[j], fmaf(g, c1[j], fmaf(r, c0[j], (e0[j] + e1[j]) + e2[j])));
+        *reinterpret_cast<fu4*>(orow + (long long)x * 256) = o;
+        if (plane == 0 && lane == 0)
+            *reinterpret_cast<float4*>(rgb4 + ((long long)v * hw + (long long)y * W + x) * 4) = make_float4(r, g, b, 0.f);
+    }
+}
+
+__global__ __launch_bounds__(256) void fold_upsample_list_kernel(FoldLvl s0, FoldLvl s1, FoldLvl s2, const float* __restrict__ img,
+                                                                 const float* __restrict__ lc, int V, int H, int W,
+                                                                 const int32_t* __restrict__ list, const unsigned* __restrict__ count,
+                                                                 float* __restrict__ fold, float* __restrict__ rgb4) {
+    const int lane = threadIdx.x & 63, wave = __builtin_amdgcn_readfirstlane(threadIdx.x >> 6);
+    const int plane = wave & 1, ch = plane * 256 + 4 * lane;
+    const int n = (int)*count, walkers = (int)gridDim.x * 2;
+    const fu4 c0 = *reinterpret_cast<const fu4*>(lc + ch), c1 = *reinterpret_cast<const fu4*>(lc + 512 + ch),
+              c2 = *reinterpret_cast<const fu4*>(lc + 1024 + ch);
+    const long long hw = (long long)H * W;
+    for (int e = (int)blockIdx.x * 2 + (wave >> 1); e < n; e += walkers) {
+        const int t = list[e];
+        const int v = t / (int)hw, rem = t - v * (int)hw, y = rem / W, x = rem - y * W;
+        int yl0, yl1;
+        float la, lb;
+        FU_CORNERS(ka);
+        FU_CORNERS(kb);
+        FU_CORNERS(kc);
+        ups_coord(y, s0.h, H, yl0, yl1, la, lb);
+        const fu4 e0 = fu_level(ka00, ka01, ka10, ka11, kai0, kai1, s0.p + (((long long)v * s0.h + yl0) * s0.w) * 512 + ch,
+                                s0.p + (((long long)v * s0.h + yl1) * s0.w) * 512 + ch, x, s0.w, W, la, lb);
+        ups_coord(y, s1.h, H, yl0, yl1, la, lb);
+        const fu4 e1 = fu_level(kb00, kb01, kb10, kb11, kbi0, kbi1, s1.p + (((long long)v * s1.h + yl0) * s1.w) * 512 + ch,
+                                s1.p + (((long long)v * s1.h + yl1) * s1.w) * 512 + ch, x, s1.w, W, la, lb);
+        ups_coord(y, s2.h, H, yl0, yl1, la, lb);
+        const fu4 e2 = fu_level(kc00, kc01, kc10, kc11, kci0, kci1, s2.p + (((long long)v * s2.h + yl0) * s2.w) * 512 + ch,
+                                s2.p + (((long long)v * s2.h + yl1) * s2.w) * 512 + ch, x, s2.w, W, la, lb);
+        const float* ip = img + (long long)v * 3 * hw + rem;
+        const float r = ip[0], g = ip[hw], b = ip[2 * hw];
+        fu4 o;
+#pragma unroll
+        for (int j = 0; j < 4; ++j) o[j] = fmaf(b, c2[j], fmaf(g, c1[j], fmaf(r, c0[j], (e0[j] + e1[j]) + e2[j])));
+        *reinterpret_cast<fu4*>(fold + ((long long)plane * V * hw + t) * 256 + 4 * lane) = o;
+        if (plane == 0 && lane == 0) *reinterpret_cast<float4*>(rgb4 + (long long)t * 4) = make_float4(r, g, b, 0.f);
+    }
+}
+
+int th_fold_upsample_launch(const float* img, const float* lvl0, const float* lvl1, const float* lvl2, const int* dims, int V, int H,
+                            int W, const float* lc, const int32_t* box, float* fold, float* rgb4, hipStream_t s,
+                            const unsigned* demand) {
+    TH_REQUIRE(H <= 65535 && V <= 65535, "image too tall for one launch");
+    FoldLvl s0{lvl0, dims[0], dims[1]}, s1{lvl1, dims[2], dims[3]}, s2{lvl2, dims[4], dims[5]};
+    if (demand != nullptr) {
+        const size_t NW = (size_t)V * H * W / 32;
+        hipLaunchKernelGGL(fold_upsample_list_kernel, dim3(2048), dim3(256), 0, s, s0, s1, s2, img, lc, V, H, W,
+                           reinterpret_cast<const int32_t*>(demand + 2 * NW + 16), demand + 2 * NW, fold, rgb4);
+        TH_LAUNCH_CHECK();
+        return 0;
+    }
+    hipLaunchKernelGGL(fold_upsample_kernel, dim3(th_cdiv(W, 2 * FU_RUN), H, V), dim3(256), 0, s, s0, s1, s2, img, lc, V, H, W, box,
+                       fold, rgb4);
+    TH_LAUNCH_CHECK();
+    return 0;
+}
+
+__global__ __launch_bounds__(256) void pixgather_levels_kernel(UpsSrc s0, UpsSrc s1, UpsSrc s2, const float* __restrict__ img, int V,
+                                                               int H, int W, const float* __restrict__ pts, const float* __restrict__ cams,
+                                                               const float* __restrict__ scale, float* __restrict__ out, int ldo) {
+    const int p = blockIdx.x / V, v = blockIdx.x - p * V, c = threadIdx.x;
+    float uu, vv;
+    th_project(cams + 21 * v, pts[3 * p], pts[3 * p + 1], pts[3 * p + 2], uu, vv);
+    const Bilin b = th_bilinear_setup(uu, vv, scale[0], scale[1], H, W);
+    const UpsSrc s = c < 64 ? s0 : (c < 128 ? s1 : s2);
+    const float* pl = s.p + ((long long)v * s.C + (c - s.c0)) * s.h * s.w;
+    const int tx[4] = {b.x0, b.x1, b.x0, b.x1}, ty[4] = {b.y0, b.y0, b.y1, b.y1};
+    float q[4];
+#pragma unroll
+    for (int k = 0; k < 4; ++k) {
+        int y0, y1, x0, x1;
+        float ly0, ly1, lx0, lx1;
+        ups_coord(ty[k], s.h, H, y0, y1, ly0, ly1);
+        ups_coord(tx[k], s.w, W, x0, x1, lx0, lx1);
+        q[k] = ups_blend(pl[y0 * s.w + x0], pl[y0 * s.w + x1], pl[y1 * s.w + x0], pl[y1 * s.w + x1], lx0, lx1, ly0, ly1);
+    }
+    float* orow = out + ((long long)p * V + v) * ldo;
+    orow[c] = fmaf(q[3], b.w11, fmaf(q[2], b.w10, fmaf(q[1], b.w01, q[0] * b.w00)));
+    if (256 + c < ldo) {
+        float r = 0.f;
+        if (c < 3) {
+            const float* ip = img + ((long long)v * 3 + c) * H * W;
+            r = fmaf(ip[b.i11], b.w11, fmaf(ip[b.i10], b.w10, fmaf(ip[b.i01], b.w01, ip[b.i00] * b.w00)));
+        }
+        orow[256 + c] = r;
+    }
+}
+
+int th_pixgather_levels_launch(const float* img, const float* lat0, const float* lat1, const float* lat2, const int* dims, int V,
+                               int H, int W, const float* pts_world, int P, const float* cams, const float* scale, float* out,
+                               int ldo, hipStream_t s) {
+    if (P <= 0) return 0;
+    TH_REQUIRE(ldo >= 260 && ldo <= 512, "rows hold the 260 channels of the compact map");
+    UpsSrc s0{lat0, 64, dims[0], dims[1], 0};
+    UpsSrc s1{lat1, 64, dims[2], dims[3], 64};
+    UpsSrc s2{lat2, 128, dims[4], dims[5], 128};
+    hipLaunchKernelGGL(pixgather_levels_kernel, dim3((unsigned)(P * V)), dim3(256), 0, s, s0, s1, s2, img, V, H, W, pts_world, cams,
+                       scale, out, ldo);
     TH_LAUNCH_CHECK();
     return 0;
 }
diff --git a/transhuman_amd/csrc/k_mlp_fused_host.hip b/transhuman_amd/csrc/k_mlp_fused_host.hip
--- a/transhuman_amd/csrc/k_mlp_fused_host.hip
+++ b/transhuman_amd/csrc/k_mlp_fused_host.hip
@@ -179,6 +179,13 @@
     }
 }
 
+__global__ void fold_lc_kernel(const float* __restrict__ a0, const float* __restrict__ xr, const float* __restrict__ r1,
+                               float* __restrict__ lc) {
+    const int n = blockIdx.x * 256 + threadIdx.x;
+    const float* row = n < 256 ? a0 + (long long)n * 260 : (n < 384 ? xr + (long long)(n - 256) * 260 : r1 + (long long)(n - 384) * 260);
+    for (int j = 0; j < 3; ++j) lc[j * 512 + n] = row[256 + j];
+}
+
 int th_fused_pack(const th_mlp_weights* w, const th_linear* folded, void* store, FusedParams* out, hipStream_t s) {
     char* tail = (char*)store + th_fused_pack_bytes() - 64 * 1024;
     PackCursor cur{(char*)store, (float*)tail, (int*)(tail + 40 * 1024)};
@@ -277,6 +284,13 @@
         out->vfA.inv_scale = out->vfD.inv_scale = ldexpf(1.f, -s_vf);
         out->compact_ready = folded != nullptr;
     }
+    out->fold_lc = nullptr;
+    if (folded) {
+        hipLaunchKernelGGL(fold_lc_kernel, dim3(2), dim3(256), 0, s, folded[0].w, XRc, folded[2].w, cur.bias);
+        TH_LAUNCH_CHECK();
+        out->fold_lc = cur.bias;
+        cur.bias += 3 * 512;
+    }
     float* tb = tw + 384 * 256;
     for (int which = 0; which < 2; ++which) {
         const th_linear& k = which == 0 ? w->key1 : w->key0;
@@ -368,6 +382,32 @@
     hipLaunchKernelGGL(map_fold_kernel<false>, dim3((unsigned)(V * H * tpr)), dim3(256), 2 * MF_TEX * STR272, s, p);
     TH_LAUNCH_CHECK();
     return 0;
+}
+
+size_t th_fold_levels_ws(int V, const int* dims) {
+    return th_align(((size_t)dims[0] * dims[1] + (size_t)dims[2] * dims[3] + (size_t)dims[4] * dims[5]) * V * 512 * sizeof(float));
+}
+
+int th_fold_levels_launch(const FusedParams& base, const float* img, const float* lat0, const float* lat1, const float* lat2,
+                          const int* dims, int V, int H, int W, const int32_t* box, void* ws, float* fold, float* rgb4,
+                          unsigned int* range, hipStream_t s, const unsigned* demand) {
+    TH_REQUIRE(base.compact_ready && base.fold_lc, "the map fold needs the colour-folded layers (th_mlp_weights.upsample_color)");
+    TH_REQUIRE(V >= 1 && H >= 1 && W >= 1 && img && lat0 && lat1 && lat2 && ws && fold && rgb4, "bad argument");
+    for (int i = 0; i < 6; ++i) TH_REQUIRE(dims[i] >= 1 && dims[i] <= 8192, "bad level size");
+    LevelFoldParams p;
+    p.ar0 = base.ar0c; p.rst = base.rstc;
+    p.lat0 = lat0; p.lat1 = lat1; p.lat2 = lat2;
+    p.h0 = dims[0]; p.w0 = dims[1]; p.h1 = dims[2]; p.w1 = dims[3]; p.h2 = dims[4]; p.w2 = dims[5];
+    const int n0 = th_cdiv(p.h0 * p.w0, MF_TEX), n1 = th_cdiv(p.h1 * p.w1, MF_TEX), n2 = th_cdiv(p.h2 * p.w2, MF_TEX);
+    p.wg1 = n0; p.wg2 = n0 + n1; p.wgn = n0 + n1 + n2;
+    p.out0 = (float*)ws;
+    p.out1 = p.out0 + (size_t)V * p.h0 * p.w0 * 512;
+    p.out2 = p.out1 + (size_t)V * p.h1 * p.w1 * 512;
+    p.box = box; p.V = V; p.H = H; p.W = W;
+    p.range = range;
+    hipLaunchKernelGGL(level_fold_kernel, dim3((unsigned)(V * p.wgn)), dim3(256), 2 * MF_TEX * LF_STR, s, p);
+    TH_LAUNCH_CHECK();
+    return th_fold_upsample_launch(img, p.out0, p.out1, p.out2, dims, V, H, W, base.fold_lc, box, fold, rgb4, s, demand);
 }
 
 int th_mlp_fused_forward(const FusedParams& base, const ThMlpPacked& heads, int V, int P, const float* stok,
diff --git a/transhuman_amd/csrc/k_mlp_fused_kernel.h b/transhuman_amd/csrc/k_mlp_fused_kernel.h
--- a/transhuman_amd/csrc/k_mlp_fused_kernel.h
+++ b/transhuman_amd/csrc/k_mlp_fused_kernel.h
@@ -1400,3 +1400,116 @@
     __syncthreads();
     }
 }
+
+#define LF_STR STR128
+struct LevelFoldParams {
+    FusedLayer ar0, rst;
+    const float* lat0;
+    const float* lat1;
+    const float* lat2;
+    int h0, w0, h1, w1, h2, w2;
+    int wg1, wg2, wgn;
+    float* out0;
+    float* out1;
+    float* out2;
+    const int32_t* box;
+    int V, H, W;
+    unsigned int* range;
+};
+__device__ __forceinline__ void level_span(int d0, int d1, int in, int out, int& i0, int& i1) {
+    const float scale = (out > 1) ? (float)(in - 1) / (float)(out - 1) : 0.f;
+    i0 = (int)(scale * (float)d0);
+    i1 = (int)(scale * (float)d1);
+    i1 = i1 + ((i1 < in - 1) ? 1 : 0);
+    i0 = min(max(i0, 0), in - 1);
+    i1 = min(max(i1, i0), in - 1);
+}
+__global__ __launch_bounds__(256, 1) void level_fold_kernel(LevelFoldParams P) {
+    extern __shared__ __attribute__((aligned(16))) char lds[];
+    char* hi_pl = lds;
+    char* lo_pl = lds + MF_TEX * LF_STR;
+    const int tid = threadIdx.x, lane = tid & 63, wave = tid >> 6;
+    const int v = (int)blockIdx.x / P.wgn;
+    int g = (int)blockIdx.x - v * P.wgn;
+    const int lvl = g >= P.wg2 ? 2 : (g >= P.wg1 ? 1 : 0);
+    g -= lvl == 2 ? P.wg2 : (lvl == 1 ? P.wg1 : 0);
+    const int C = lvl == 2 ? 128 : 64, h = lvl == 2 ? P.h2 : (lvl == 1 ? P.h1 : P.h0), w = lvl == 2 ? P.w2 : (lvl == 1 ? P.w1 : P.w0);
+    const float* lat = (lvl == 2 ? P.lat2 : (lvl == 1 ? P.lat1 : P.lat0)) + (long long)v * C * h * w;
+    float* out = (lvl == 2 ? P.out2 : (lvl == 1 ? P.out1 : P.out0)) + (long long)v * h * w * 512;
+    const int kb0 = lvl == 2 ? 8 : 4 * lvl, KB = C / 16;
+    int lx0 = 0, ly0 = 0, lx1 = w - 1, ly1 = h - 1;
+    if (P.box != nullptr) {
+        const int bx0 = P.box[4 * v], by0 = P.box[4 * v + 1], bx1 = P.box[4 * v + 2], by1 = P.box[4 * v + 3];
+        if (bx1 < bx0 || by1 < by0) return;
+        level_span(bx0, bx1, w, P.W, lx0, lx1);
+        level_span(by0, by1, h, P.H, ly0, ly1);
+    }
+    const int nx = lx1 - lx0 + 1, n = nx * (ly1 - ly0 + 1);
+    const int xs = g * MF_TEX;
+    if (xs >= n) return;
+    auto texel = [&](int i) __attribute__((always_inline)) -> int {
+        const int ty = i / nx;
+        return (ly0 + ty) * w + lx0 + (i - ty * nx);
+    };
+    {
+        unsigned rmax = 0u;
+        const unsigned seen_f = P.range ? P.range[TH_RANGE_F] : 0u;
+        const int ta = texel(min(xs + lane, n - 1)), tb = texel(min(xs + 64 + (lane & 31), n - 1));
+        const long long hw = (long long)h * w;
+        const int wv = __builtin_amdgcn_readfirstlane(wave);
+        for (int cp = wv; cp < C / 2; cp += 4) {
+            const float* p0 = lat + (long long)(2 * cp) * hw;
+            unsigned hh, ll;
+            split_pair(p0[ta], p0[hw + ta], hh, ll);
+            range_acc<false>(rmax, hh);
+            *reinterpret_cast<unsigned*>(hi_pl + lane * LF_STR + cp * 4) = hh;
+            *reinterpret_cast<unsigned*>(lo_pl + lane * LF_STR + cp * 4) = ll;
+            if (lane < 32) {
+                split_pair(p0[tb], p0[hw + tb], hh, ll);
+                range_acc<false>(rmax, hh);
+                *reinterpret_cast<unsigned*>(hi_pl + (64 + lane) * LF_STR + cp * 4) = hh;
+                *reinterpret_cast<unsigned*>(lo_pl + (64 + lane) * LF_STR + cp * 4) = ll;
+            }
+        }
+        range_commit(P.range, TH_RANGE_F, seen_f, rmax);
+    }
+    __syncthreads();
+    const int myrow = lane & 31;
+    uint4 wk2[FM_RING_D2][2][2];
+    f32x16 acc[2][MF_RT];
+    gemm_phase_core<MF_RT, 2, LF_STR, 32 * LF_STR, FM_RING_D2, true, 3, false>(hi_pl, lo_pl, wslice(P.ar0, wave, 2, kb0), KB, lane, acc, wk2);
+    {
+        const float sc = P.ar0.inv_scale;
+#pragma unroll
+        for (int r = 0; r < MF_RT; ++r) {
+            const int i = xs + r * 32 + myrow;
+            if (i < n) {
+                float* o = out + (long long)texel(i) * 512 + wave * 64 + 4 * (lane >> 5);
+#pragma unroll
+                for (int c = 0; c < 2; ++c)
+#pragma unroll
+                    for (int q = 0; q < 4; ++q)
+                        *reinterpret_cast<float4*>(o + c * 32 + 8 * q) =
+                            make_float4(acc[c][r][4 * q] * sc, acc[c][r][4 * q + 1] * sc, acc[c][r][4 * q + 2] * sc, acc[c][r][4 * q + 3] * sc);
+            }
+        }
+    }
+    gemm_phase_core<MF_RT, 2, LF_STR, 32 * LF_STR, FM_RING_D2, true, 3, false>(hi_pl, lo_pl, wslice(P.rst, wave, 2, kb0), KB, lane, acc, wk2);
+    {
+        const float s0 = P.rst.inv_scale, s1 = P.rst.inv_scale2;
+#pragma unroll
+        for (int r = 0; r < MF_RT; ++r) {
+            const int i = xs + r * 32 + myrow;
+            if (i < n) {
+                float* o = out + (long long)texel(i) * 512 + 256 + wave * 32 + 4 * (lane >> 5);
+#pragma unroll
+                for (int q = 0; q < 4; ++q) {
+                    *reinterpret_cast<float4*>(o + 8 * q) =
+                        make_float4(acc[0][r][4 * q] * s0, acc[0][r][4 * q + 1] * s0, acc[0][r][4 * q + 2] * s0, acc[0][r][4 * q + 3] * s0);
+                    *reinterpret_cast<float4*>(o + 128 + 8 * q) =
+                        make_float4(acc[1][r][4 * q] * s1, acc[1][r][4 * q + 1] * s1, acc[1][r][4 * q + 2] * s1, acc[1][r][4 * q + 3] * s1);
+                }
+            }
+        }
+    }
+}
diff --git a/transhuman_amd/csrc/th_api.hip b/transhuman_amd/csrc/th_api.hip
--- a/transhuman_amd/csrc/th_api.hip
+++ b/transhuman_amd/csrc/th_api.hip
@@ -94,6 +94,8 @@
     if (c->mlp_store) (void)hipFree(c->mlp_store);
     if (c->vit_store) (void)hipFree(c->vit_store);
     if (c->fused_store) (void)hipFree(c->fused_store);
+    if (c->level_ws) (void)hipFree(c->level_ws);
+    if (c->level_ws_ev) (void)hipEventDestroy(c->level_ws_ev);
     if (c->host_pinned) (void)hipHostFree(c->host_pinned);
     if (c->range_dev) (void)hipFree(c->range_dev);
     if (c->range_host) (void)hipHostFree(c->range_host);
@@ -474,11 +476,12 @@
            th_align((size_t)(out_f * 260 + out_f) * 4);
 }
 
-int th_paint_group_nhwc(th_ctx* c, const float* map_nhwc, int V, int H, int W, int C, const float* verts, int nv,
-                        const float* cams, const float* scale, const uint8_t* viz, const th_linear* reduction,
-                        const th_linear* color_lift, const int32_t* off, const int32_t* mem, int nc, float* tokens,
-                        void* ws, size_t ws_bytes, th_stream stream) {
-    TH_REQUIRE(c && map_nhwc && verts && cams && scale && reduction && off && mem && tokens && ws, "null argument");
+struct PaintLevels { const float *img, *lat0, *lat1, *lat2; const int32_t* dims; };
+static int paint_group_rows(th_ctx* c, const float* map_nhwc, const PaintLevels* lv, int V, int H, int W, int C, const float* verts,
+                            int nv, const float* cams, const float* scale, const uint8_t* viz, const th_linear* reduction,
+                            const th_linear* color_lift, const int32_t* off, const int32_t* mem, int nc, float* tokens,
+                            void* ws, size_t ws_bytes, th_stream stream) {
+    TH_REQUIRE(c && (map_nhwc || lv) && verts && cams && scale && reduction && off && mem && tokens && ws, "null argument");
     const bool compact = C == TH_MAP_COMPACT || C == TH_MAP_SPLIT;
     TH_REQUIRE(reduction->in_f == (compact ? TH_MAP_FULL : C), "reduction layer must take the (full) map's channel count");
     TH_REQUIRE(!compact || (color_lift && color_lift->w && lin_ok(*color_lift, 128, 3)),
@@ -494,7 +497,8 @@
     void* pk = ar.take<char>(ThPacked::bytes(out_f, CR));
     float* fold = ar.take<float>((size_t)out_f * 260 + out_f);
     TH_REQUIRE(fold != nullptr, "workspace carve failed");
-    TH_TRY(th_pixgather_launch(map_nhwc, V, C, H, W, verts, nullptr, nullptr, nv, cams, scale, g, CR, TH_ROWS_F32, s));
+    if (lv) TH_TRY(th_pixgather_levels_launch(lv->img, lv->lat0, lv->lat1, lv->lat2, lv->dims, V, H, W, verts, nv, cams, scale, g, CR, s));
+    else TH_TRY(th_pixgather_launch(map_nhwc, V, C, H, W, verts, nullptr, nullptr, nv, cams, scale, g, CR, TH_ROWS_F32, s));
     ThPacked P;
     th_linear red = *reduction;
     if (compact) {
@@ -505,6 +509,25 @@
     TH_TRY(th_pack_linear(red, pk, &P, s));
     TH_TRY(th_gemm(g, CR, (int)rows, P, TH_ACT_NONE, r, out_f, s));
     return th_segmean_masked_launch(r, V, out_f, viz, nv, off, mem, nc, tokens, s);
+}
+
+int th_paint_group_nhwc(th_ctx* c, const float* map_nhwc, int V, int H, int W, int C, const float* verts, int nv,
+                        const float* cams, const float* scale, const uint8_t* viz, const th_linear* reduction,
+                        const th_linear* color_lift, const int32_t* off, const int32_t* mem, int nc, float* tokens,
+                        void* ws, size_t ws_bytes, th_stream stream) {
+    TH_REQUIRE(map_nhwc, "null argument");
+    return paint_group_rows(c, map_nhwc, nullptr, V, H, W, C, verts, nv, cams, scale, viz, reduction, color_lift, off, mem, nc, tokens,
+                            ws, ws_bytes, stream);
+}
+
+int th_paint_group_levels(th_ctx* c, const float* img, const float* lat0, const float* lat1, const float* lat2,
+                          const int32_t* dims_host, int V, int H, int W, const float* verts, int nv, const float* cams,
+                          const float* scale, const uint8_t* viz, const th_linear* reduction, const th_linear* color_lift,
+                          const int32_t* off, const int32_t* mem, int nc, float* tokens, void* ws, size_t ws_bytes, th_stream stream) {
+    TH_REQUIRE(img && lat0 && lat1 && lat2 && dims_host, "null argument");
+    const PaintLevels lv{img, lat0, lat1, lat2, dims_host};
+    return paint_group_rows(c, nullptr, &lv, V, H, W, TH_MAP_SPLIT, verts, nv, cams, scale, viz, reduction, color_lift, off, mem, nc,
+                            tokens, ws, ws_bytes, stream);
 }
 
 int th_bn_act_eval(th_ctx* c, const float* x, const float* residual, int N, int C, int HW, const float* gamma, const float* beta,
@@ -612,15 +635,61 @@
                                TH_ROWS_SPLIT, (hipStream_t)stream, nullptr);
 }
 
+static void level_fold_forget(th_ctx* c, const void* fold) {
+    for (auto& p : c->level_folds) if (p == fold) p = nullptr;
+}
+static bool level_fold_known(const th_ctx* c, const void* fold) {
+    if (fold == nullptr) return false;
+    for (auto p : c->level_folds) if (p == fold) return true;
+    return false;
+}
+
 int th_map_fold(th_ctx* c, const float* map_split, int V, int H, int W, const int32_t* box, float* fold, th_stream stream) {
     TH_REQUIRE(c && map_split && fold, "null argument");
+    level_fold_forget(c, fold);
     TH_REQUIRE(c->fused_ready && c->fused.compact_ready, "th_map_fold needs the MLP weights incl. upsample_color (th_set_mlp_weights)");
     ProfScope sc(prof_of(c), TH_PROF_FOLD, (hipStream_t)stream);
     return th_map_fold_launch(c->fused, map_split, V, H, W, box, fold, c->range_dev, (hipStream_t)stream);
 }
 
+size_t th_map_fold_levels_workspace_bytes(int V, const int32_t* dims_host) {
+    return dims_host && V > 0 ? th_fold_levels_ws(V, dims_host) : 0;
+}
+
+int th_map_fold_levels(th_ctx* c, const float* img, const float* lat0, const float* lat1, const float* lat2, const int32_t* dims_host,
+                       int V, int H, int W, const int32_t* box, float* map_split, float* fold, void* ws, size_t ws_bytes,
+                       th_stream stream) {
+    TH_REQUIRE(c && img && lat0 && lat1 && lat2 && dims_host && map_split && fold && ws, "null argument");
+    TH_REQUIRE(c->fused_ready && c->fused.compact_ready, "th_map_fold_levels needs the MLP weights incl. upsample_color (th_set_mlp_weights)");
+    TH_REQUIRE(ws_bytes >= th_fold_levels_ws(V, dims_host), "workspace too small (th_map_fold_levels_workspace_bytes)");
+    ProfScope sc(prof_of(c), TH_PROF_FOLD, (hipStream_t)stream);
+    if (!level_fold_known(c, fold)) {
+        c->level_folds[c->level_fold_next] = fold;
+        c->level_fold_next = (c->level_fold_next + 1) % 16;
+    }
+    return th_fold_levels_launch(c->fused, img, lat0, lat1, lat2, dims_host, V, H, W, box, ws, fold, map_split + (size_t)V * H * W * 256,
+                                 c->range_dev, (hipStream_t)stream);
+}
+
+int th_map_fold_levels_demand(th_ctx* c, const float* img, const float* lat0, const float* lat1, const float* lat2,
+                              const int32_t* dims_host, int V, int H, int W, const void* demand, float* map_split, float* fold,
+                              void* ws, size_t ws_bytes, th_stream stream) {
+    TH_REQUIRE(c && img && lat0 && lat1 && lat2 && dims_host && map_split && fold && ws && demand, "null argument");
+    TH_REQUIRE(c->fused_ready && c->fused.compact_ready, "th_map_fold_levels needs the MLP weights incl. upsample_color (th_set_mlp_weights)");
+    TH_REQUIRE(ws_bytes >= th_fold_levels_ws(V, dims_host), "workspace too small (th_map_fold_levels_workspace_bytes)");
+    TH_REQUIRE(W % 64 == 0, "demand-driven map: the image width must be a multiple of 64");
+    ProfScope sc(prof_of(c), TH_PROF_FOLD, (hipStream_t)stream);
+    if (!level_fold_known(c, fold)) {
+        c->level_folds[c->level_fold_next] = fold;
+        c->level_fold_next = (c->level_fold_next + 1) % 16;
+    }
+    return th_fold_levels_launch(c->fused, img, lat0, lat1, lat2, dims_host, V, H, W, nullptr, ws, fold, map_split + (size_t)V * H * W * 256,
+                                 c->range_dev, (hipStream_t)stream, reinterpret_cast<const unsigned*>(demand));
+}
+
 int th_map_fold_demand(th_ctx* c, const float* map_split, int V, int H, int W, const void* demand, float* fold, th_stream stream) {
     TH_REQUIRE(c && map_split && fold && demand, "null argument");
+    level_fold_forget(c, fold);
     TH_REQUIRE(c->fused_ready && c->fused.compact_ready, "th_map_fold needs the MLP weights incl. upsample_color (th_set_mlp_weights)");
     ProfScope sc(prof_of(c), TH_PROF_FOLD, (hipStream_t)stream);
     return th_map_fold_launch(c->fused, map_split, V, H, W, nullptr, fold, c->range_dev, (hipStream_t)stream,
@@ -1028,8 +1097,26 @@
                                           : (unmasked || f->hull_thresh < 0.f || f->hull_thresh > f->map_source->reach))) {
         const th_map_source* ms = f->map_source;
         TH_REQUIRE(f->map_channels == TH_MAP_SPLIT && ms->img && ms->lat0 && ms->lat1 && ms->lat2, "map_source: split map only");
+        if (prepass == 3 && tex && level_fold_known(c, f->map_fold)) {
+            c->prepass[slot].npre = 0;
+            return 0;
+        }
         TH_TRY(th_upsample_concat_launch(ms->img, ms->lat0, ms->lat1, ms->lat2, ms->dims, V, f->H, f->W, nullptr, nullptr,
                                          const_cast<float*>(f->pixel_map_nhwc), s, 1, nullptr));
+        if (tex && level_fold_known(c, f->map_fold)) {
+            const size_t need = th_fold_levels_ws(V, ms->dims);
+            if (!c->level_ws_ev) TH_HIP(hipEventCreateWithFlags(&c->level_ws_ev, hipEventDisableTiming));
+            else TH_HIP(hipStreamWaitEvent(s, c->level_ws_ev, 0));
+            if (c->level_ws_bytes < need) {
+                if (c->level_ws) { TH_HIP(hipDeviceSynchronize()); TH_HIP(hipFree(c->level_ws)); c->level_ws = nullptr; c->level_ws_bytes = 0; }
+                TH_HIP(hipMalloc(&c->level_ws, need));
+                c->level_ws_bytes = need;
+            }
+            TH_TRY(th_fold_levels_launch(c->fused, ms->img, ms->lat0, ms->lat1, ms->lat2, ms->dims, V, f->H, f->W, nullptr, c->level_ws,
+                                         const_cast<float*>(f->map_fold),
+                                         const_cast<float*>(f->pixel_map_nhwc) + (size_t)V * f->H * f->W * 256, c->range_dev, s));
+            TH_HIP(hipEventRecord(c->level_ws_ev, s));
+        } else
         if (tex) TH_TRY(th_map_fold_launch(c->fused, f->pixel_map_nhwc, V, f->H, f->W, nullptr, const_cast<float*>(f->map_fold),
                                            c->range_dev, s));
         if (tk) tk->map_done = f->pixel_map_nhwc;
diff --git a/transhuman_amd/csrc/th_internal.h b/transhuman_amd/csrc/th_internal.h
--- a/transhuman_amd/csrc/th_internal.h
+++ b/transhuman_amd/csrc/th_internal.h
@@ -242,6 +242,7 @@
     unsigned int* range;
     long long* dbg;
     long long* cycles_buf;
+    const float* fold_lc;
 };
 enum { TH_RANGE_F = 0, TH_RANGE_S = 1, TH_RANGE_P = 2, TH_RANGE_N = 3, TH_RANGE_INTER = 4, TH_RANGE_F4 = 5, TH_RANGE_CONV = 6,
        TH_RANGE_VIT = 7 };
@@ -260,6 +261,16 @@
 }
 int th_map_fold_launch(const FusedParams& base, const float* map_split, int V, int H, int W, const int32_t* box, float* fold,
                        unsigned int* range, hipStream_t s, const unsigned* demand = nullptr );
+size_t th_fold_levels_ws(int V, const int* dims);
+int th_fold_levels_launch(const FusedParams& base, const float* img, const float* lat0, const float* lat1, const float* lat2,
+                          const int* dims, int V, int H, int W, const int32_t* box, void* ws, float* fold, float* rgb4,
+                          unsigned int* range, hipStream_t s, const unsigned* demand = nullptr );
+int th_fold_upsample_launch(const float* img, const float* lvl0, const float* lvl1, const float* lvl2, const int* dims, int V, int H,
+                            int W, const float* lc, const int32_t* box, float* fold, float* rgb4, hipStream_t s,
+                            const unsigned* demand = nullptr);
+int th_pixgather_levels_launch(const float* img, const float* lat0, const float* lat1, const float* lat2, const int* dims, int V,
+                               int H, int W, const float* pts_world, int P, const float* cams, const float* scale, float* out,
+                               int ldo, hipStream_t s);
 size_t th_pixtex_bytes(int V, long long P);
 int th_pixtex_launch(int V, int H, int W, const ThPointSrc* ps, const int32_t* sel, int P, const float* cams,
                      const float* scale, void* out, hipStream_t s);
@@ -273,6 +284,11 @@
     int vit_mode = 1;
     int tok_gather = 1;
     int tex_rows = 1;
+    const void* level_folds[16] = {};
+    int level_fold_next = 0;
+    void* level_ws = nullptr;
+    size_t level_ws_bytes = 0;
+    hipEvent_t level_ws_ev = nullptr;
     int device = 0;
     void* mlp_store = nullptr;
     void* vit_store = nullptr;
diff --git a/transhuman_amd/hip.py b/transhuman_amd/hip.py
--- a/transhuman_amd/hip.py
+++ b/transhuman_amd/hip.py
@@ -101,6 +101,16 @@
                                                   C.POINTER(C.c_int32), C.c_int, C.c_int, C.c_int, C.c_void_p, C.c_void_p,
                                                   C.c_void_p, C.c_void_p]),
     "th_map_fold_demand": (C.c_int, [C.c_void_p, C.c_void_p, C.c_int, C.c_int, C.c_int, C.c_void_p, C.c_void_p, C.c_void_p]),
+    "th_map_fold_levels_workspace_bytes": (C.c_size_t, [C.c_int, C.POINTER(C.c_int32)]),
+    "th_map_fold_levels": (C.c_int, [C.c_void_p, C.c_void_p, C.c_void_p, C.c_void_p, C.c_void_p, C.POINTER(C.c_int32), C.c_int,
+                                     C.c_int, C.c_int, C.c_void_p, C.c_void_p, C.c_void_p, C.c_void_p, C.c_size_t, C.c_void_p]),
+    "th_map_fold_levels_demand": (C.c_int, [C.c_void_p, C.c_void_p, C.c_void_p, C.c_void_p, C.c_void_p, C.POINTER(C.c_int32),
+                                            C.c_int, C.c_int, C.c_int, C.c_void_p, C.c_void_p, C.c_void_p, C.c_void_p, C.c_size_t,
+                                            C.c_void_p]),
+    "th_paint_group_levels": (C.c_int, [C.c_void_p, C.c_void_p, C.c_void_p, C.c_void_p, C.c_void_p, C.POINTER(C.c_int32),
+                                        C.c_int, C.c_int, C.c_int, C.c_void_p, C.c_int, C.c_void_p, C.c_void_p, C.c_void_p,
+                                        C.POINTER(ThLinear), C.POINTER(ThLinear), C.c_void_p, C.c_void_p, C.c_int, C.c_void_p,
+                                        C.c_void_p, C.c_size_t, C.c_void_p]),
     "th_render_predemand": (C.c_int, [C.c_void_p, C.POINTER(ThFrame), C.POINTER(ThPoints), C.c_void_p, C.c_size_t, C.c_void_p,
                                       C.c_int, C.c_void_p, C.c_size_t, C.c_void_p]),
     "th_map_box": (C.c_int, [C.c_void_p, C.c_void_p, C.c_int, C.c_void_p, C.c_int, C.c_void_p, C.c_int, C.c_void_p,
@@ -563,6 +573,22 @@
         self.device = buf.device
         self.source = source
         self.fold = None
+        self.levels = None
+
+    def _materialise(self):
+        if self.levels is None:
+            return
+        (img, l0, l1, l2, dims), self.levels = self.levels, None
+        lib = load_library()
+        if self.demand is not None:
+            _check(lib.th_upsample_concat_split_demand(ctx(img.device), _p(img), _p(l0), _p(l1), _p(l2), dims, self.V, self.H, self.W,
+                                                       self.buf.data_ptr(), None, _p(self.demand), _stream()))
+        elif self.box is None:
+            _check(lib.th_upsample_concat_split(ctx(img.device), _p(img), _p(l0), _p(l1), _p(l2), dims, self.V, self.H, self.W,
+                                                self.buf.data_ptr(), _stream()))
+        else:
+            _check(lib.th_upsample_concat_split_box(ctx(img.device), _p(img), _p(l0), _p(l1), _p(l2), dims, self.V, self.H, self.W,
+                                                    self.buf.data_ptr(), _p(self.box), _stream()))
 
     @property
     def box(self):
@@ -573,10 +599,12 @@
         return self.source[1][5] if self.source is not None and len(self.source[1]) > 5 else None
 
     def data_ptr(self):
+        self._materialise()
         return self.buf.data_ptr()
 
     @property
     def latents(self):
+        self._materialise()
         return self.buf[: self.V * self.H * self.W * 256].view(self.V, self.H, self.W, 256)
 
     @property
@@ -601,6 +629,40 @@
     _check(load_library().th_map_fold(ctx(split_map.device), _p(split_map), V, H, W, _p(split_map.box), _p(fold), _stream()))
     split_map.fold = fold
     return fold
+
+
+def fold_levels(net, images, lat0, lat1, lat2, box=None, reach=0.0, demand=None):
+    lib = load_library()
+    _sync_weights(net, "mlp")
+    img, l0, l1, l2 = _f32(images), _f32(lat0), _f32(lat1), _f32(lat2)
+    V, _, H, W = img.shape
+    assert l0.shape[1] == 64 and l1.shape[1] == 64 and l2.shape[1] == 128
+    dims = (C.c_int32 * 6)(l0.shape[2], l0.shape[3], l1.shape[2], l1.shape[3], l2.shape[2], l2.shape[3])
+    buf = torch.empty(V * H * W * 260, dtype=torch.float32, device=img.device)
+    if demand is not None:
+        m = SplitMap(buf, V, H, W, source=(ThMapSource(None, float(reach), _p(img), _p(l0), _p(l1), _p(l2), dims, _p(demand)),
+                                           (None, img, l0, l1, l2, demand)))
+        m.levels = (img, l0, l1, l2, dims)
+        fold = torch.empty((2, V, H, W, 256), dtype=torch.float32, device=img.device)
+        ws = _ws(lib.th_map_fold_levels_workspace_bytes(V, dims), img.device)
+        _check(lib.th_map_fold_levels_demand(ctx(img.device), _p(img), _p(l0), _p(l1), _p(l2), dims, V, H, W, _p(demand),
+                                             buf.data_ptr(), _p(fold), _p(ws), ws.numel(), _stream()))
+        m.fold = fold
+        return m
+    if box is not None:
+        assert box.dtype == torch.int32 and tuple(box.shape) == (V, 4) and box.is_contiguous()
+        _box_checked(box, H)
+        src = ThMapSource(_p(box), float(reach), _p(img), _p(l0), _p(l1), _p(l2), dims, None)
+        m = SplitMap(buf, V, H, W, source=(src, (box, img, l0, l1, l2)))
+    else:
+        m = SplitMap(buf, V, H, W)
+    m.levels = (img, l0, l1, l2, dims)
+    fold = torch.empty((2, V, H, W, 256), dtype=torch.float32, device=img.device)
+    ws = _ws(lib.th_map_fold_levels_workspace_bytes(V, dims), img.device)
+    _check(lib.th_map_fold_levels(ctx(img.device), _p(img), _p(l0), _p(l1), _p(l2), dims, V, H, W, _p(box), buf.data_ptr(),
+                                  _p(fold), _p(ws), ws.numel(), _stream()))
+    m.fold = fold
+    return m
 
 
 def map_box(verts_a, verts_b, cams, scale_xy, H, W, reach):
@@ -677,6 +739,13 @@
     lift, keep2 = _linear(color_w, color_b) if color_w is not None else (None, None)
     tokens = torch.empty((V, nc, lin.out_f), dtype=torch.float32, device=v.device)
     ws = _ws(lib.th_paint_group_nhwc_workspace_bytes(V, v.shape[0], Cc, lin.out_f), v.device)
+    if isinstance(map_nhwc, SplitMap) and map_nhwc.levels is not None:
+        img, l0, l1, l2, dims = map_nhwc.levels
+        assert lift is not None
+        _check(lib.th_paint_group_levels(ctx(v.device), _p(img), _p(l0), _p(l1), _p(l2), dims, V, H, W, _p(v), v.shape[0],
+                                         _p(cams), _p(scale_xy), _p(viz), C.byref(lin), C.byref(lift), _p(off), _p(mem), nc,
+                                         _p(tokens), _p(ws), ws.numel(), _stream()))
+        return tokens
     _check(lib.th_paint_group_nhwc(ctx(v.device), _p(map_nhwc), V, H, W, Cc, _p(v), v.shape[0], _p(cams), _p(scale_xy),
                                    _p(viz), C.byref(lin), C.byref(lift) if lift is not None else None, _p(off), _p(mem),
                                    nc, _p(tokens), _p(ws), ws.numel(), _stream()))
@@ -1155,7 +1224,7 @@
             "pixel map must be the full (384) or the compact (260 interleaved / SplitMap) channels-last map"
         src = getattr(pixel_map_nhwc, "source", None)
         self.c = ThFrame(_p(self.verts), self.verts.shape[0], _p(self.Rh), _p(self.Th), _p(self.cams), _p(self.scale),
-                         _p(self.map), V, H, W, Cc, _p(self.tokens), _p(self.centres), _p(self.rot),
+                         _p(self.map.buf if isinstance(self.map, SplitMap) else self.map), V, H, W, Cc, _p(self.tokens), _p(self.centres), _p(self.rot),
                          self.centres.shape[0], hull_thresh, small_frame_rays,
                          C.cast(C.pointer(src[0]), C.c_void_p).value if src is not None else None,
                          _p(getattr(pixel_map_nhwc, "fold", None)))
@@ -1263,6 +1332,12 @@
                                             _stream()))
 
 
+def _frame_latents(frame, dev):
+    m = frame.map
+    if isinstance(m, SplitMap) and m.levels is not None and not (tex_rows_enabled(dev) and mlp_is_fused(dev)):
+        m._materialise()
+
+
 def render_pregather(net, frame, points, slot=0, early=False, pool_slot=None):
     if not getattr(points, "_prepass_pending", False):
         return
@@ -1273,6 +1348,7 @@
     cnt = _prepass_counts(ws, dev)
     if cnt is None:
         return
+    _frame_latents(frame, dev)
     pool = _shade_pool(frame.c, cnt[2], True, dev, pool_slot)
     points._pregathered = True
     fn = lib.th_render_pregather_early if early else lib.th_render_pregather
@@ -1306,6 +1382,7 @@
         ws = _cached_ws(need, dev)
         _check(lib.th_render_prepass_drop(ctx(dev), _p(ws)))
     points._pregathered = False
+    _frame_latents(frame, dev)
     pool = _shade_pool(fc, n_bound, pre, dev, pool_slot)
     stats = (C.c_int64 * 4)()
     _check(lib.th_render_rays(ctx(dev), C.byref(fc), C.byref(points.c), _p(rgb), _p(acc), _p(dep), int(white_bkgd),
@@ -1323,6 +1400,7 @@
             fc = ThFrame.from_buffer_copy(frame.c)
             fc.small_frame_rays = keep_sfr
         _check(lib.th_render_prepass_drop(ctx(dev), _p(ws)))
+        _frame_latents(frame, dev)
         pool = _shade_pool(fc, st["valid_samples"], False, dev, pool_slot)
         _check(lib.th_render_rays(ctx(dev), C.byref(fc), C.byref(points.c), _p(rgb), _p(acc), _p(dep),
                                   int(white_bkgd), _p(ws), ws.numel(), _p(pool), pool.numel(), stats, _stream()))
@@ -1342,6 +1420,7 @@
     ws = _cached_ws(lib.th_sigma_grid_workspace_bytes(C.byref(frame.c), P), p.device)
     stats = (C.c_int64 * 4)()
     for _ in range(3):
+        _frame_latents(frame, p.device)
         pool = _shade_pool(frame.c, P, False, p.device)
         _check(lib.th_eval_sigma_grid(ctx(p.device), C.byref(frame.c), _p(p), P, _p(out), _p(ws), ws.numel(), _p(pool),
                                       pool.numel(), stats, _stream()))
diff --git a/transhuman_amd/networks/renderer/if_clight_renderer.py b/transhuman_amd/networks/renderer/if_clight_renderer.py
--- a/transhuman_amd/networks/renderer/if_clight_renderer.py
+++ b/transhuman_amd/networks/renderer/if_clight_renderer.py
@@ -99,7 +99,33 @@
             thr = cfg_hull() if hull_thresh is None else hull_thresh
             if crop_map is None:
                 crop_map = os.environ.get("TH_MAP_CROP") != "0"
-            if compact_map == "interleaved":
+            tex = (hip.tex_rows_enabled(dev) and V <= 3 and V * H * W < (1 << 22) and hip.mlp_is_fused(dev))
+            levels = (tex and compact_map is True and os.environ.get("TH_FOLD_LEVELS") != "0")
+            map_nhwc = None
+            if levels and demand is not None:
+                torch.cuda.current_stream(dev).wait_event(demand[1])
+                map_nhwc = hip.fold_levels(self.net, images, lat[0], lat[1], lat[2], demand=demand[0])
+            elif levels:
+                box, reach = None, 0.0
+                if crop_map and thr >= 0:
+                    reach = float(thr) * 1.001 + 1e-6
+                    box = hip.map_box(batch["tar_smpl_vertice"][0], batch["input_smpl_vertice"][t][0], cams, scale, H, W, reach)
+                if pregather is not None:
+                    cur = torch.cuda.current_stream(dev)
+                    fs = self._dev.get(("fold_stream", str(dev)))
+                    if fs is None:
+                        fs = self._dev[("fold_stream", str(dev))] = torch.cuda.Stream(dev)
+                    hip._sync_weights(self.net, "mlp")
+                    fs.wait_stream(cur)
+                    with torch.cuda.stream(fs):
+                        map_nhwc = hip.fold_levels(self.net, images, lat[0], lat[1], lat[2], box=box, reach=reach)
+                        fold_done = torch.cuda.Event()
+                        fold_done.record(fs)
+                    map_nhwc.fold.record_stream(cur)
+                    map_nhwc.buf.record_stream(cur)
+                else:
+                    map_nhwc = hip.fold_levels(self.net, images, lat[0], lat[1], lat[2], box=box, reach=reach)
+            elif compact_map == "interleaved":
                 map_nhwc = hip.upsample_concat_nhwc(images, lat[0], lat[1], lat[2])
             elif compact_map and demand is not None:
                 torch.cuda.current_stream(dev).wait_event(demand[1])
@@ -112,8 +138,7 @@
                 map_nhwc = hip.upsample_concat_split(images, lat[0], lat[1], lat[2])
             else:
                 map_nhwc = hip.upsample_concat_nhwc(images, lat[0], lat[1], lat[2], cw, cb)
-            if (isinstance(map_nhwc, hip.SplitMap) and hip.tex_rows_enabled(dev) and V <= 3 and V * H * W < (1 << 22)
-                    and hip.mlp_is_fused(dev)):
+            if isinstance(map_nhwc, hip.SplitMap) and tex and not levels:
                 if pregather is not None:
                     cur = torch.cuda.current_stream(dev)
                     fs = self._dev.get(("fold_stream", str(dev)))
```

Result: no change. 19.05 million (-0.4%).
